# ETH3D/badslam

Hardware: NVIDIA H100
Metric: surfel_keyframe_residuals_per_second_per_BA_iteration (higher is better)
Workload: dtype f32

## Files before the change

badslam_b200/_lib.py:

```python
from __future__ import annotations

import ctypes as C
import os

HERE = os.path.dirname(os.path.abspath(__file__))
LIB_PATH = os.path.join(HERE, "libbadba_b200.so")

ABI_VERSION = 10

POSE_VARIANT_AUTO, POSE_VARIANT_256_PRE, POSE_VARIANT_512_PRE, POSE_VARIANT_256, POSE_VARIANT_512, POSE_VARIANT_1024 = range(6)

OK, ERR_INVALID_ARGUMENT, ERR_CUDA, ERR_STATE, ERR_UNSUPPORTED, ERR_NO_DEVICE = range(6)
STATUS_NAMES = {0: "BBA_OK", 1: "BBA_ERR_INVALID_ARGUMENT", 2: "BBA_ERR_CUDA", 3: "BBA_ERR_STATE",
                4: "BBA_ERR_UNSUPPORTED", 5: "BBA_ERR_NO_DEVICE"}


class Config(C.Structure):
    _fields_ = [("depth_width", C.c_int), ("depth_height", C.c_int), ("color_width", C.c_int), ("color_height", C.c_int),
                ("depth_intrinsics", C.c_float * 4), ("color_intrinsics", C.c_float * 4),
                ("raw_to_float_depth", C.c_float), ("baseline_fx", C.c_float),
                ("sparse_surfel_cell_size", C.c_int), ("max_surfel_count", C.c_uint32), ("max_keyframes", C.c_int),
                ("use_depth_residuals", C.c_int), ("use_descriptor_residuals", C.c_int),
                ("device", C.c_int), ("rank", C.c_int), ("world_size", C.c_int),
                ("min_observation_count_while_bootstrapping_1", C.c_int), ("min_observation_count_while_bootstrapping_2", C.c_int),
                ("min_observation_count", C.c_int), ("surfel_merge_dist_factor", C.c_float)]


PROGRESS_FN = C.CFUNCTYPE(C.c_int, C.c_void_p, C.c_int)


class BAOptions(C.Structure):
    _fields_ = [("optimize_depth_intrinsics", C.c_int), ("optimize_color_intrinsics", C.c_int),
                ("do_surfel_updates", C.c_int), ("optimize_poses", C.c_int), ("optimize_geometry", C.c_int),
                ("min_iterations", C.c_int), ("max_iterations", C.c_int), ("use_pcg", C.c_int),
                ("active_keyframe_window_start", C.c_int), ("active_keyframe_window_end", C.c_int),
                ("increase_ba_iteration_count", C.c_int), ("time_limit_seconds", C.c_double),
                ("pcg_max_inner_iterations", C.c_int), ("pcg_max_keyframes", C.c_int), ("pcg_gauge_keyframe", C.c_int),
                ("progress_function", PROGRESS_FN), ("progress_user", C.c_void_p)]


class PcgProbe(C.Structure):
    _fields_ = [("r", C.c_void_p), ("M", C.c_void_p), ("p", C.c_void_p), ("g", C.c_void_p), ("delta", C.c_void_p),
                ("alpha_n", C.c_double), ("alpha_d", C.c_double),
                ("r_step2", C.c_void_p), ("delta_step2", C.c_void_p), ("z", C.c_void_p), ("beta_n", C.c_double),
                ("p_step3", C.c_void_p), ("g_step3", C.c_void_p), ("alpha_d_step3", C.c_double)]


class BAResult(C.Structure):
    _fields_ = [("iterations_done", C.c_int), ("converged", C.c_int),
                ("depth_residual_count", C.c_uint64), ("descriptor_residual_count", C.c_uint64), ("cost", C.c_double),
                ("pose_iterations_total", C.c_int),
                ("ms_surfel_activation", C.c_float), ("ms_geometry_optimization", C.c_float),
                ("ms_pose_optimization", C.c_float), ("ms_intrinsics_optimization", C.c_float),
                ("kernel_launches", C.c_uint64),
                ("pcg_inner_iterations_total", C.c_int), ("pcg_last_r_norm", C.c_float), ("ms_pcg", C.c_float),
                ("surfels_deleted", C.c_uint32), ("surfels_size", C.c_uint32),
                ("surfels_created", C.c_uint32), ("surfels_merged", C.c_uint32)]


class PreprocessOptions(C.Structure):
    _fields_ = [("bilateral_filter_sigma_xy", C.c_float), ("bilateral_filter_sigma_inv_depth", C.c_float),
                ("bilateral_filter_radius_factor", C.c_float), ("max_depth", C.c_float)]


class RawFrameOptions(C.Structure):
    _fields_ = [("base", PreprocessOptions), ("median_filter_and_densify_iterations", C.c_int),
                ("pyramid_level_for_depth", C.c_int), ("pyramid_level_for_color", C.c_int)]


class OdometryOptions(C.Structure):
    _fields_ = [("num_scales", C.c_int), ("use_pyramid_level_0", C.c_int), ("use_gradmag", C.c_int),
                ("test_different_initial_estimates", C.c_int), ("max_iterations_per_scale", C.c_int)]


class OdometryResult(C.Structure):
    _fields_ = [("iterations", C.c_int * 8), ("chose_initial", C.c_int * 8), ("residual_count", C.c_uint32),
                ("residual_sum", C.c_float), ("passes", C.c_uint32), ("kernel_launches", C.c_uint32)]


class MotionModelRecord(C.Structure):
    _fields_ = [("count", C.c_int), ("base_kf_tr_frame", (C.c_float * 7) * 3), ("frame_tr_base_kf", (C.c_float * 7) * 3)]


class PoseConstraint(C.Structure):
    _fields_ = [("keyframe_a", C.c_int), ("keyframe_b", C.c_int), ("a_T_b", C.c_float * 7), ("information", C.c_float * 21)]


class PoseGraphOptions(C.Structure):
    _fields_ = [("gauge_keyframe", C.c_int), ("max_iterations", C.c_int), ("use_odometry_chain", C.c_int),
                ("odometry_information", C.c_float * 21)]


class PoseGraphResult(C.Structure):
    _fields_ = [("iterations", C.c_int), ("converged", C.c_int), ("linear_iterations", C.c_int), ("held_keyframes", C.c_int),
                ("initial_cost", C.c_double), ("final_cost", C.c_double)]


class PeerHandle(C.Structure):
    _fields_ = [("surfels_ipc", C.c_ubyte * 64), ("surfels_offset", C.c_uint64), ("active_ipc", C.c_ubyte * 64),
                ("active_offset", C.c_uint64), ("pitch_bytes", C.c_uint64), ("surfels_size", C.c_uint32), ("rank", C.c_int32)]


class PoseCoeffs(C.Structure):
    _fields_ = [("H", C.c_float * 21), ("b", C.c_float * 6),
                ("n_pair", C.c_uint64), ("n_inimg", C.c_uint64), ("n_depthok", C.c_uint64),
                ("n_assoc", C.c_uint64), ("n_photo", C.c_uint64),
                ("cost_depth", C.c_double), ("cost_desc1", C.c_double), ("cost_desc2", C.c_double)]


class FrameBuffers(C.Structure):
    _fields_ = [("depth", C.c_void_p), ("depth_pitch", C.c_size_t), ("normals", C.c_void_p), ("normals_pitch", C.c_size_t),
                ("color_rgba", C.c_void_p), ("color_pitch", C.c_size_t)]


class OdometryEntry(C.Structure):
    _fields_ = [("base_keyframe_id", C.c_int), ("base_frame", C.c_int), ("tracked_frame", C.c_int),
                ("base_T_frame_initial_1", C.c_float * 7), ("base_T_frame_initial_2", C.c_float * 7)]


ODOMETRY_CHUNK_ENTRIES = 64


class Profile(C.Structure):
    _fields_ = [("pose_launches", C.c_uint64), ("pose_ms", C.c_double), ("kf_evals", C.c_uint64),
                ("n_pair", C.c_uint64), ("n_inimg", C.c_uint64), ("n_depthok", C.c_uint64),
                ("n_assoc", C.c_uint64), ("n_photo", C.c_uint64),
                ("geometry_launches", C.c_uint64), ("activation_normals_ms", C.c_double),
                ("position_descriptor_ms", C.c_double)]


COLLECTIVE_FN = C.CFUNCTYPE(None, C.c_void_p, C.c_int, C.c_void_p, C.c_size_t, C.c_void_p)
COLLECTIVE_ALLGATHER, COLLECTIVE_ALLREDUCE_SUM = 0, 1

_P = C.c_void_p
_F7 = C.POINTER(C.c_float)
SYMBOLS = {
    "bba_abi_version": (C.c_int, []),
    "bba_create": (C.c_int, [C.POINTER(Config), C.POINTER(_P)]),
    "bba_destroy": (None, [_P]),
    "bba_last_error": (C.c_char_p, [_P]),
    "bba_set_surfels": (C.c_int, [_P, _P, C.c_size_t, C.c_uint32]),
    "bba_set_active_flags": (C.c_int, [_P, _P]),
    "bba_set_surfels_host": (C.c_int, [_P, _P, C.c_size_t, C.c_uint32, _P]),
    "bba_get_surfels_host": (C.c_int, [_P, _P, C.c_size_t, C.c_int, _P]),
    "bba_get_active_flags_host": (C.c_int, [_P, _P, _P]),
    "bba_get_surfels_device": (C.c_int, [_P, C.POINTER(_P), C.POINTER(C.c_size_t), C.POINTER(C.c_uint32)]),
    "bba_add_keyframe": (C.c_int, [_P, _P, C.c_size_t, _P, C.c_size_t, _P, C.c_size_t, _P, C.c_size_t, _F7,
                                   C.c_float, C.c_float, _P, C.POINTER(C.c_int)]),
    "bba_add_keyframe_host": (C.c_int, [_P, _P, _P, _P, _P, _F7, C.c_float, C.c_float, _P, C.POINTER(C.c_int)]),
    "bba_keyframe_count": (C.c_int, [_P]),
    "bba_set_keyframe_pose": (C.c_int, [_P, C.c_int, _F7]),
    "bba_get_keyframe_pose": (C.c_int, [_P, C.c_int, _F7]),
    "bba_set_keyframe_activation": (C.c_int, [_P, C.c_int, C.c_int]),
    "bba_get_keyframe_activation": (C.c_int, [_P, C.c_int, C.POINTER(C.c_int)]),
    "bba_set_keyframe_states": (C.c_int, [_P, C.c_int, _P, _P]),
    "bba_get_keyframe_states": (C.c_int, [_P, C.c_int, _P, _P]),
    "bba_get_covisibility": (C.c_int, [_P, C.c_int, _P]),
    "bba_set_keyframe_pose_priors": (C.c_int, [_P, C.c_int, _P, _P, _P]),
    "bba_clear_keyframe_pose_priors": (C.c_int, [_P, C.c_int, _P]),
    "bba_get_keyframe_pose_prior": (C.c_int, [_P, C.c_int, _P, _P, C.POINTER(C.c_int)]),
    "bba_add_keyframe_pose_constraints": (C.c_int, [_P, C.c_int, _P, _P]),
    "bba_remove_keyframe_pose_constraints": (C.c_int, [_P, C.c_int, _P]),
    "bba_get_keyframe_pose_constraints": (C.c_int, [_P, C.c_int, _P, _P, C.POINTER(C.c_int)]),
    "bba_set_intrinsics": (C.c_int, [_P, _F7, _F7, C.c_float]),
    "bba_get_intrinsics": (C.c_int, [_P, _F7, _F7, C.POINTER(C.c_float)]),
    "bba_host_se3_exp": (None, [_P, _P]),
    "bba_host_se3_log": (None, [_P, _P]),
    "bba_host_se3_compose": (None, [_P, _P, _P]),
    "bba_host_se3_inverse": (None, [_P, _P]),
    "bba_host_pose_update_converged": (C.c_int, [_P]),
    "bba_host_solve_ldlt": (C.c_int, [C.c_int, _P, _P, _P]),
    "bba_host_pose_prior_terms": (None, [_P, _P, _P, _P, _P, C.POINTER(C.c_double)]),
    "bba_host_pose_constraint_terms": (None, [_P, _P, _P, _P, _P, _P, C.POINTER(C.c_double)]),
    "bba_host_frusta_intersect": (C.c_int, [_P, C.c_int, C.c_int, _P, C.c_float, C.c_float, _P, C.c_float, C.c_float]),
    "bba_host_motion_model_clear": (None, [C.POINTER(MotionModelRecord), _P, _P]),
    "bba_host_motion_model_predict": (C.c_int, [C.POINTER(MotionModelRecord), C.c_int, _P, _P]),
    "bba_host_motion_model_push": (None, [C.POINTER(MotionModelRecord), _P]),
    "bba_host_motion_model_rebase": (None, [C.POINTER(MotionModelRecord)]),
    "bba_host_deform_trajectory": (C.c_int, [C.c_int, _P, _P, _P, C.c_int, C.c_int, _P]),
    "bba_set_residual_types": (C.c_int, [_P, C.c_int, C.c_int]),
    "bba_get_residual_types": (C.c_int, [_P, C.POINTER(C.c_int), C.POINTER(C.c_int)]),
    "bba_set_cfactor_host": (C.c_int, [_P, _P, _P]),
    "bba_get_cfactor_host": (C.c_int, [_P, _P, _P]),
    "bba_cfactor_size": (C.c_int, [_P, C.POINTER(C.c_int), C.POINTER(C.c_int)]),
    "bba_accumulate_pose_coeffs": (C.c_int, [_P, C.c_int, _F7, C.POINTER(PoseCoeffs), _P]),
    "bba_debug_pose_coeffs_batch": (C.c_int, [_P, C.c_int, _P, _P, C.c_int, C.c_int, _P, _P, _P, _P, _P]),
    "bba_debug_set_pose_group": (C.c_int, [_P, C.c_int]),
    "bba_estimate_frame_pose": (C.c_int, [_P, C.c_int, _F7, _F7, C.POINTER(C.c_int), C.POINTER(C.c_int), _P]),
    "bba_estimate_frame_pose_for_frame": (C.c_int, [_P, _P, C.c_size_t, _P, C.c_size_t, _P, C.c_size_t, _F7, _F7,
                                                    C.POINTER(C.c_int), C.POINTER(C.c_int), _P]),
    "bba_estimate_frame_poses_for_frames": (C.c_int, [_P, C.c_int, C.POINTER(FrameBuffers), C.c_int, _P, _P, _P, _P, _P,
                                                      C.POINTER(PoseCoeffs), _P]),
    "bba_track_frame_pairwise": (C.c_int, [_P, C.POINTER(OdometryOptions), C.c_int, _P, C.c_size_t, _P, C.c_size_t, _P, C.c_size_t,
                                           _F7, _F7, _F7, C.POINTER(OdometryResult), _P]),
    "bba_track_frames_pairwise": (C.c_int, [_P, C.POINTER(OdometryOptions), C.c_int, C.POINTER(FrameBuffers), C.c_int,
                                            C.POINTER(OdometryEntry), _P, C.POINTER(OdometryResult), C.POINTER(C.c_uint32), _P]),
    "bba_track_frame_pairwise_to_frame": (C.c_int, [_P, C.POINTER(OdometryOptions), _P, C.c_size_t, _P, C.c_size_t, _P, C.c_size_t,
                                                    _P, C.c_size_t, _P, C.c_size_t, _P, C.c_size_t, _F7, _F7, _F7,
                                                    C.POINTER(OdometryResult), _P]),
    "bba_odometry_get_level": (C.c_int, [_P, C.c_int, C.c_int, _P, _P, _P, C.POINTER(C.c_int), C.POINTER(C.c_int), _P]),
    "bba_odometry_debug_coeffs": (C.c_int, [_P, C.c_int, C.c_int, _F7, _F7, _P, _P, C.POINTER(C.c_uint32), C.POINTER(C.c_float),
                                            _P, _P, _P]),
    "bba_update_surfel_activation": (C.c_int, [_P, _P]),
    "bba_optimize_geometry_iteration": (C.c_int, [_P, _P]),
    "bba_deform_surfels": (C.c_int, [_P, C.c_int, _P, C.POINTER(C.c_uint32), C.POINTER(C.c_uint32), _P]),
    "bba_optimize_pose_graph": (C.c_int, [_P, C.POINTER(PoseGraphOptions), C.POINTER(PoseGraphResult), _P]),
    "bba_optimize_intrinsics": (C.c_int, [_P, C.c_int, C.c_int, _P]),
    "bba_debug_intrinsics_coeffs": (C.c_int, [_P, C.c_int, C.c_int, _P, _P, _P]),
    "bba_perform_end_tasks": (C.c_int, [_P, C.c_int, C.POINTER(C.c_uint32), C.POINTER(C.c_uint32), _P]),
    "bba_surfels_size": (C.c_uint32, [_P]),
    "bba_get_ba_iteration_counts": (C.c_int, [_P, C.POINTER(C.c_int), C.POINTER(C.c_int)]),
    "bba_set_ba_iteration_counts": (C.c_int, [_P, C.c_int, C.c_int]),
    "bba_create_surfels_for_keyframe": (C.c_int, [_P, C.c_int, C.c_int, C.POINTER(C.c_uint32), _P]),
    "bba_merge_surfels_for_keyframe": (C.c_int, [_P, C.c_int, C.POINTER(C.c_uint32), _P]),
    "bba_compact_surfels": (C.c_int, [_P, C.c_uint32, C.c_int, C.POINTER(C.c_uint32), _P]),
    "bba_preprocess_frame": (C.c_int, [_P, C.POINTER(PreprocessOptions), _P, C.c_size_t, _P, C.c_size_t, _P, C.c_size_t,
                                       _P, C.c_size_t, _P, C.c_size_t, _P, C.c_size_t, C.POINTER(C.c_float), C.POINTER(C.c_float), _P]),
    "bba_preprocess_raw_frame": (C.c_int, [_P, C.POINTER(RawFrameOptions), _P, C.c_size_t, C.c_int, C.c_int, _P, C.c_size_t, C.c_int,
                                           C.c_int, _P, C.c_size_t, _P, C.c_size_t, _P, C.c_size_t, _P, C.c_size_t,
                                           C.POINTER(C.c_float), C.POINTER(C.c_float), _P]),
    "bba_pcg_debug": (C.c_int, [_P, C.POINTER(BAOptions), C.c_int, C.c_int, C.POINTER(C.c_uint32), C.POINTER(PcgProbe), _P]),
    "bba_bundle_adjust": (C.c_int, [_P, C.POINTER(BAOptions), C.POINTER(BAResult), _P]),
    "bba_peer_export": (C.c_int, [_P, _P]),
    "bba_peer_import": (C.c_int, [_P, _P, C.c_int]),
    "bba_peer_count": (C.c_int, [_P]),
    "bba_peer_unmap": (C.c_int, [_P]),
    "bba_mark_replica_rewritten": (C.c_int, [_P]),
    "bba_set_collective": (C.c_int, [_P, COLLECTIVE_FN, _P]),
    "bba_local_group_create": (C.c_int, [C.POINTER(_P), C.c_int, C.c_int, C.POINTER(_P)]),
    "bba_local_group_reset": (C.c_int, [_P]),
    "bba_local_group_poison": (C.c_int, [_P]),
    "bba_local_group_destroy": (None, [_P]),
    "bba_debug_collective": (C.c_int, [_P, C.c_int, _P, C.c_size_t, _P]),
    "bba_shard_surfel_owner": (C.c_int, [C.c_uint32, C.c_int]),
    "bba_shard_surfel_local_index": (C.c_uint32, [C.c_uint32, C.c_int]),
    "bba_shard_slice_length": (C.c_uint32, [C.c_uint32, C.c_int]),
    "bba_shard_keyframe_owner": (C.c_int, [C.c_int, C.c_int]),
    "bba_balance_keyframes": (None, [_P, C.c_int, C.c_int, _P]),
    "bba_kernel_launch_count": (C.c_uint64, [_P]),
    "bba_update_keyframe_host": (C.c_int, [_P, C.c_int, _P, _P, _P, _P, _P]),
    "bba_set_deterministic": (C.c_int, [_P, C.c_int]),
    "bba_get_deterministic": (C.c_int, [_P, C.POINTER(C.c_int)]),
    "bba_debug_exact_sum": (C.c_int, [_P, _P, C.c_uint64, C.POINTER(C.c_double), _P]),
    "bba_host_exact_sum": (None, [_P, C.c_size_t, C.POINTER(C.c_double)]),
    "bba_set_profiling": (C.c_int, [_P, C.c_int]),
    "bba_get_profile": (C.c_int, [_P, C.POINTER(Profile), C.c_int]),
}

_lib = None


def load():
    global _lib
    if _lib is not None:
        return _lib
    if not os.path.exists(LIB_PATH):
        raise ImportError(f"{LIB_PATH} is missing: build it with `python -m badslam_b200.build` "
                          "(there is no CPU / eager fallback)")
    lib = C.CDLL(LIB_PATH)
    for name, (restype, argtypes) in SYMBOLS.items():
        fn = getattr(lib, name)
        fn.restype = restype
        fn.argtypes = argtypes
    if lib.bba_abi_version() != ABI_VERSION:
        raise ImportError(f"libbadba_b200.so ABI version {lib.bba_abi_version()}, this binding expects {ABI_VERSION}")
    _lib = lib
    return lib


class BadBAError(RuntimeError):
    def __init__(self, status, message):
        super().__init__(f"{STATUS_NAMES.get(status, status)}: {message}")
        self.status = status
```

badslam_b200/csrc/bundle_adjust.cu:

```cuda
#include <chrono>
#include <cmath>
#include <cstring>
#include <limits>

#include "handle.hpp"

namespace bba {
namespace {

void DetermineCovisibleActiveKeyframes(bba_handle h) {
  for (Keyframe& kf : h->keyframes) {
    if (kf.activation != BBA_KF_ACTIVE) continue;
    for (int o : kf.covis) {
      Keyframe& other = h->keyframes[o];
      if (other.activation == BBA_KF_INACTIVE) other.activation = BBA_KF_COVISIBLE_ACTIVE;
    }
  }
}

bba_status ReserveTileEpochs(bba_handle h) {
  const uint32_t need = (h->surfels_size + 31u) / 32u;
  BBA_CUDA(h, h->geo.d_tile_epoch.Reserve(need, std::max<uint32_t>((h->cfg.max_surfel_count + 31u) / 32u, need) + 1));
  return BBA_OK;
}
// ... 556 lines not shown
             h->pcg.d_vec[4], h->pcg.d_scalars, an, bn, h->sm_count, s);
  return BBA_OK;
}

bba_status PcgStep3(bba_handle h, const PcgLayout& L, int an, int bn, cudaStream_t s) {
  BBA_CUDA(h, cudaMemsetAsync(h->pcg.d_scalars + 1, 0, sizeof(double), s));
  BBA_LAUNCH(h, h->launches, LaunchPcgStep3, L.unknown_count, L.a_index, static_cast<int>(h->keyframes.size()), h->pcg.d_vec[3],
             h->pcg.d_vec[4], h->pcg.d_scalars, an, bn, h->sm_count, s);
  return BBA_OK;
}

bba_status PcgApplyDelta(bba_handle h, const PcgLayout& L, int gauge, cudaStream_t s, int* num_converged) {
  const int K = static_cast<int>(h->keyframes.size());
  const uint32_t N = h->surfels_size, P = static_cast<uint32_t>(h->cf_w) * h->cf_h;
  const float* pcg_delta = h->pcg.d_vec[2];
  size_t n_host = 0;
  const size_t pose_floats = L.opt_poses ? 6 * static_cast<size_t>(K - 1) : 0;
  if (pose_floats) BBA_CUDA(h, cudaMemcpyAsync(h->pcg.h_delta, pcg_delta, sizeof(float) * pose_floats, cudaMemcpyDeviceToHost, s));
  n_host = pose_floats;
  float* h_di = h->pcg.h_delta + n_host;
  if (L.opt_depth_intr) {
    BBA_CUDA(h, cudaMemcpyAsync(h_di, pcg_delta + L.depth_start, sizeof(float) * 5, cudaMemcpyDeviceToHost, s));
    n_host += 5;
  }
  float* h_ci = h->pcg.h_delta + n_host;
  if (L.opt_color_intr) BBA_CUDA(h, cudaMemcpyAsync(h_ci, pcg_delta + L.color_start, sizeof(float) * 4, cudaMemcpyDeviceToHost, s));
  if (L.opt_geometry && N > 0) {
    BBA_LAUNCH(h, h->launches, LaunchPcgUpdateSurfels, h->surfels, SurfelPitch(h), N, L.use_desc, L.surfel_start, pcg_delta, s);
    h->xchg.replicated_pass_pending = true;
  }
  if (L.opt_depth_intr) BBA_LAUNCH(h, h->launches, LaunchPcgUpdateCfactor, h->d_cfactor, P, pcg_delta + L.depth_start + 5, s);
  BBA_CUDA(h, cudaStreamSynchronize(s));
  if (L.opt_poses) {
    for (int k = 0; k < K; ++k) {
      if (k == gauge) {
        ++*num_converged;
        continue;
      }
      const float* d6 = h->pcg.h_delta + 6 * static_cast<size_t>(k < gauge ? k : k - 1);
      const Pose delta = bba::Exp(d6);
      h->keyframes[k].pose = bba::Compose(h->keyframes[k].pose, delta);
      float lg[6];
      bba::Log(delta, lg);
      if (bba::IsScale1PoseEstimationConverged(lg)) ++*num_converged;
    }
  }
  if (L.opt_depth_intr) {
    const double old_fx_inv = 1. / h->depth_K[0], old_fy_inv = 1. / h->depth_K[1];
    const double old_cx_inv = -(h->depth_K[2] - 0.5) * old_fx_inv, old_cy_inv = -(h->depth_K[3] - 0.5) * old_fy_inv;
    const double new_fx = 1. / (old_fx_inv + h_di[0]);
    const double new_fy = 1. / (old_fy_inv + h_di[1]);
    const double new_cx = -(new_fx * (old_cx_inv + h_di[2])) + 0.5;
    const double new_cy = -(new_fy * (old_cy_inv + h_di[3])) + 0.5;
    h->depth_K[0] = static_cast<float>(new_fx);
    h->depth_K[1] = static_cast<float>(new_fy);
    h->depth_K[2] = static_cast<float>(new_cx);
    h->depth_K[3] = static_cast<float>(new_cy);
    h->depth_a += h_di[4];
  }
  if (L.opt_color_intr)
    for (int c = 0; c < 4; ++c) h->color_K[c] = static_cast<float>(h->color_K[c] + h_ci[c]);
  return Publish(h, s, L.opt_depth_intr);
}

bba_status BundleAdjustPCG(bba_handle h, const bba_ba_options* o, bba_ba_result* res, cudaStream_t s) {
  const int K = static_cast<int>(h->keyframes.size());
  const int world = h->cfg.world_size;
  if (bba_status st = CheckCollective(h)) return st;
  if (world > 1 && o->pcg_gauge_keyframe < 0)
    return Fail(h, BBA_ERR_INVALID_ARGUMENT, "use_pcg with more than one rank needs pcg_gauge_keyframe >= 0 (the reference draws rand() % K)");
  if (K == 0) return Fail(h, BBA_ERR_STATE, "use_pcg: no keyframes");
  const int max_inner = o->pcg_max_inner_iterations > 0 ? o->pcg_max_inner_iterations : 30;
  const int max_keyframes = o->pcg_max_keyframes > 0 ? o->pcg_max_keyframes : 2500;
  if (K > max_keyframes) return Fail(h, BBA_ERR_INVALID_ARGUMENT, "use_pcg: more keyframes than pcg_max_keyframes");
  if (o->pcg_gauge_keyframe >= K) return Fail(h, BBA_ERR_INVALID_ARGUMENT, "pcg_gauge_keyframe out of range");
  PcgLayout L;
  if (bba_status st = MakePcgLayout(h, o, &L)) return st;
  const bool opt_poses = L.opt_poses, opt_geometry = L.opt_geometry;
  const uint64_t launches_before = h->launches;
  const auto t_start = std::chrono::steady_clock::now();
  if (bba_status st = BeginBundleAdjust(h, o, res, s)) return st;
  std::vector<int> keyframes_with_new_surfels;

  for (int iteration = 0; iteration < o->max_iterations; ++iteration) {
    if (o->progress_function && !o->progress_function(o->progress_user, iteration)) break;
    ++res->iterations_done;
    if (bba_status st = CreateInLoopSurfels(h, o, h->ba_iteration_count, s, res, &keyframes_with_new_surfels)) return st;
    const uint32_t N = h->surfels_size;
    if (N > 0) BBA_CUDA(h, cudaMemsetAsync(h->active, bba::kSurfelActiveFlag, N, s));
    if (bba_status st = UploadKeyframes(h, s)) return st;
    BBA_CUDA(h, cudaEventRecord(h->ev[0], s));
    if (opt_geometry && N > 0) {
      bba::GeometryArgs g;
      if (bba_status st = BuildGeometryArgs(h, &g, s, GeoOrder::kCaller)) return st;
      BBA_LAUNCH(h, h->launches, LaunchActivationAndNormals, g, h->sm_count, false, true, s);
      if (bba_status st = ExchangeGeometry(h, s)) return st;
    }
    BBA_CUDA(h, cudaEventRecord(h->ev[1], s));

    if (bba_status st = MakePcgLayout(h, o, &L)) return st;
    const uint32_t unknown_count = L.unknown_count;
    const int gauge = o->pcg_gauge_keyframe >= 0 ? o->pcg_gauge_keyframe : (rand() % K);

    int num_converged = 0;
    if (unknown_count > 0) {
      const bba::PcgArgs a = MakePcgArgs(h, L, gauge);
      int an = 0, bn = 2;
      if (bba_status st = PcgInit(h, L, a, an, s)) return st;
      float prev_r_norm = std::numeric_limits<float>::infinity();
      int without_improvement = 0;
      for (int step = 0; step < max_inner; ++step) {
        if (step > 0) std::swap(an, bn);
        if (bba_status st = PcgStep1(h, L, a, s)) return st;
        if (bba_status st = PcgStep2(h, L, an, bn, s)) return st;
        BBA_CUDA(h, cudaMemcpyAsync(h->pcg.h_scalars, h->pcg.d_scalars, sizeof(double) * 4, cudaMemcpyDeviceToHost, s));
        BBA_CUDA(h, cudaStreamSynchronize(s));
        ++res->pcg_inner_iterations_total;
        const float r_norm = std::sqrt(static_cast<float>(h->pcg.h_scalars[bn]));
        res->pcg_last_r_norm = r_norm;
        if (static_cast<double>(r_norm) < static_cast<double>(prev_r_norm) - 1e-3) {
          without_improvement = 0;
        } else if (++without_improvement >= 3) {
          break;
        }
        prev_r_norm = r_norm;
        if (step < max_inner - 1) {
          if (bba_status st = PcgStep3(h, L, an, bn, s)) return st;
        }
      }
      BBA_CUDA(h, cudaEventRecord(h->ev[2], s));
      if (bba_status st = PcgApplyDelta(h, L, gauge, s, &num_converged)) return st;
      if (o->do_surfel_updates && !keyframes_with_new_surfels.empty()) {
        uint32_t merged = 0;
        if (bba_status st = MergeAndCompact(h, keyframes_with_new_surfels, s, &merged)) return st;
        res->surfels_merged += merged;
      }
    } else {
      BBA_CUDA(h, cudaEventRecord(h->ev[2], s));
      BBA_CUDA(h, cudaStreamSynchronize(s));
      num_converged = opt_poses ? 1 : 0;
    }
    cudaEventElapsedTime(&res->ms_geometry_optimization, h->ev[0], h->ev[1]);
    cudaEventElapsedTime(&res->ms_pcg, h->ev[1], h->ev[2]);
    if (StopIterating(o, iteration, num_converged, K, t_start, res)) break;
  }
  if (!o->increase_ba_iteration_count && o->do_surfel_updates && !keyframes_with_new_surfels.empty()) {
    uint32_t merged = 0;
    if (bba_status st = MergeAndCompact(h, keyframes_with_new_surfels, s, &merged)) return st;
    res->surfels_merged += merged;
  }
  return EndBundleAdjust(h, o, launches_before, res, s);
}

bba_status GeometryPass(bba_handle h, bool activation, cudaStream_t s) {
  if (!h) return BBA_ERR_INVALID_ARGUMENT;
  if (bba_status st = CheckSurfels(h)) return st;
  if (h->surfels_size == 0) return BBA_OK;
  if (bba_status st = UploadKeyframes(h, s)) return st;
  bba::GeometryArgs g;
  if (bba_status st = BuildGeometryArgs(h, &g, s, GeoOrder::kSpatial)) return st;
  if (bba_status st = CheckCollective(h)) return st;
  BBA_LAUNCH(h, h->launches, LaunchActivationAndNormals, g, h->sm_count, activation, !activation, s);
  if (!activation) BBA_LAUNCH(h, h->launches, LaunchPositionAndDescriptor, g, h->sm_count, s);
  if (bba_status st = ExchangeGeometry(h, s)) return st;
  return MarkStaging(h, s);
}

void QuatToMatrix64(const float q[4], double R[9]) {
  const double n = std::sqrt(static_cast<double>(q[0]) * q[0] + static_cast<double>(q[1]) * q[1] + static_cast<double>(q[2]) * q[2] +
                             static_cast<double>(q[3]) * q[3]);
  const double x = q[0] / n, y = q[1] / n, z = q[2] / n, w = q[3] / n;
  R[0] = 1 - 2 * (y * y + z * z); R[1] = 2 * (x * y - z * w); R[2] = 2 * (x * z + y * w);
  R[3] = 2 * (x * y + z * w); R[4] = 1 - 2 * (x * x + z * z); R[5] = 2 * (y * z - x * w);
  R[6] = 2 * (x * z - y * w); R[7] = 2 * (y * z + x * w); R[8] = 1 - 2 * (x * x + y * y);
}

KfChange KeyframeChange(const Pose& global_T_frame, const float original[7]) {
  KfChange c{};
  float inv[7];
  PoseToArray(Inverse(global_T_frame), inv);
  c.unmoved = std::memcmp(inv, original, sizeof(inv)) == 0;
  double Rc[9], Ro[9];
  QuatToMatrix64(global_T_frame.q, Rc);
  QuatToMatrix64(original, Ro);
  for (int r = 0; r < 3; ++r) {
    for (int col = 0; col < 3; ++col)
      c.D[4 * r + col] = static_cast<float>(Rc[3 * r] * Ro[col] + Rc[3 * r + 1] * Ro[3 + col] + Rc[3 * r + 2] * Ro[6 + col]);
    c.D[4 * r + 3] = static_cast<float>(Rc[3 * r] * original[4] + Rc[3 * r + 1] * original[5] + Rc[3 * r + 2] * original[6] +
                                        global_T_frame.t[r]);
    c.centre[r] = static_cast<float>(-(Ro[r] * original[4] + Ro[3 + r] * original[5] + Ro[6 + r] * original[6]));
  }
  if (c.unmoved)
    for (int i = 0; i < 12; ++i) c.D[i] = (i % 5 == 0) ? 1.f : 0.f;
  return c;
}

bba_status DeformSurfels(bba_handle h, int count, const float* original, uint32_t* moved, uint32_t* unobserved, cudaStream_t s) {
  if (!h) return BBA_ERR_INVALID_ARGUMENT;
  const std::string fn = "bba_deform_surfels: ";
  if (count < 0 || count > static_cast<int>(h->keyframes.size())) return Fail(h, BBA_ERR_INVALID_ARGUMENT, fn + "bad count");
  if (count > 0 && !original) return Fail(h, BBA_ERR_INVALID_ARGUMENT, fn + "null argument");
  for (int k = 0; k < count; ++k) {
    const float* p = original + 7 * static_cast<size_t>(k);
    for (int j = 0; j < 7; ++j)
      if (!std::isfinite(p[j])) return Fail(h, BBA_ERR_INVALID_ARGUMENT, fn + "non-finite pose");
    if (p[0] * p[0] + p[1] * p[1] + p[2] * p[2] + p[3] * p[3] < 1e-12f) return Fail(h, BBA_ERR_INVALID_ARGUMENT, fn + "zero quaternion");
  }
  if (moved) *moved = 0;
  if (unobserved) *unobserved = 0;
  if (count == 0 || h->surfels_size == 0) return BBA_OK;
  if (bba_status st = CheckSurfels(h)) return st;
  if (bba_status st = CheckCollective(h)) return st;
  auto& d = h->deform;
  BBA_CUDA(h, d.h_kfs.Reserve(count, h->cfg.max_keyframes));
  BBA_CUDA(h, d.d_kfs.Reserve(count, h->cfg.max_keyframes));
  BBA_CUDA(h, d.h_changes.Reserve(count, h->cfg.max_keyframes));
  BBA_CUDA(h, d.d_changes.Reserve(count, h->cfg.max_keyframes));
  BBA_CUDA(h, d.d_counts.Reserve(2));
  BBA_CUDA(h, d.h_counts.Reserve(2));
  if (bba_status st = MakeAllKeyframeList(h)) return st;
  if (bba_status st = WaitStaging(h)) return st;
  for (int k = 0; k < count; ++k) {
    const Keyframe& kf = h->keyframes[k];
    const float* p = original + 7 * static_cast<size_t>(k);
    FillKfDevice(kf, kf.pose, d.h_kfs + k);
    ToMatrix3x4(PoseFromArray(p), d.h_kfs[k].T);
    d.h_changes[k] = KeyframeChange(kf.pose, p);
  }
  BBA_CUDA(h, cudaMemcpyAsync(d.d_kfs, d.h_kfs, sizeof(KfDevice) * count, cudaMemcpyHostToDevice, s));
  BBA_CUDA(h, cudaMemcpyAsync(d.d_changes, d.h_changes, sizeof(KfChange) * count, cudaMemcpyHostToDevice, s));
  if (bba_status st = MarkStaging(h, s)) return st;
  BBA_CUDA(h, cudaMemsetAsync(d.d_counts, 0, sizeof(unsigned int) * 2, s));
  bba::DeformArgs a;
  if (bba_status st = BuildGeometryArgs(h, &a.geo, s, GeoOrder::kSpatial)) return st;
  a.geo.kfs = d.d_kfs;
  a.geo.kf_list = h->geo.d_all_list;
  a.geo.kf_count = count;
  a.changes = d.d_changes;
  a.counts = d.d_counts;
  BBA_LAUNCH(h, h->launches, LaunchDeformSurfels, a, h->sm_count, s);
  if (bba_status st = ExchangeGeometry(h, s)) return st;
  h->pose.order_stale = true;
  if (!moved && !unobserved) return BBA_OK;
  BBA_CUDA(h, cudaMemcpyAsync(d.h_counts, d.d_counts, sizeof(unsigned int) * 2, cudaMemcpyDeviceToHost, s));
  BBA_CUDA(h, cudaStreamSynchronize(s));
  uint32_t counts[2] = {d.h_counts[0], d.h_counts[1]};
  if (h->cfg.world_size > 1)
    for (uint32_t& c : counts)
      if (bba_status st = SumOverRanks(h, c, s, &c)) return st;
  if (moved) *moved = counts[0];
  if (unobserved) *unobserved = counts[1];
  return BBA_OK;
}

struct PoseGraphSizes {
  size_t terms, ints, doubles;
};
PoseGraphSizes PoseGraphCapacity(size_t K, size_t C) {
  const size_t terms = 2 * K + C, entries = 3 * K + 2 * C, nnz = 3 * K + 2 * C;
  const size_t block_doubles = sizeof(PoseGraphTermBlocks) / sizeof(double);
  return {terms, K + 2 * (K + 1) + 2 * entries + nnz, terms * block_doubles + 36 * nnz + 42 * K + PoseGraphWorkDoubles(K)};
}

bba_status ReservePoseGraph(bba_handle h, size_t constraints) {
  const size_t M = static_cast<size_t>(h->cfg.max_keyframes);
  const PoseGraphSizes need = PoseGraphCapacity(M, constraints), alloc = PoseGraphCapacity(M, 2 * constraints);
  auto& g = h->graph;
  BBA_CUDA(h, g.h_terms.Reserve(need.terms, alloc.terms));
  BBA_CUDA(h, g.d_terms.Reserve(need.terms, alloc.terms));
  BBA_CUDA(h, g.h_ints.Reserve(need.ints, alloc.ints));
  BBA_CUDA(h, g.d_ints.Reserve(need.ints, alloc.ints));
  BBA_CUDA(h, g.d_doubles.Reserve(need.doubles, alloc.doubles));
  BBA_CUDA(h, g.h_poses.Reserve(7 * M));
  BBA_CUDA(h, g.d_poses.Reserve(14 * M));
  BBA_CUDA(h, g.d_state.Reserve(1));
  BBA_CUDA(h, g.h_state.Reserve(1));
  return BBA_OK;
}

int FindRoot(std::vector<int>& parent, int k) {
  while (parent[k] != k) k = parent[k] = parent[parent[k]];
  return k;
}

bba_status OptimizePoseGraph(bba_handle h, const bba_pose_graph_options* o, bba_pose_graph_result* result, cudaStream_t s) {
  if (!h) return BBA_ERR_INVALID_ARGUMENT;
  const std::string fn = "bba_optimize_pose_graph: ";
  if (!o) return Fail(h, BBA_ERR_INVALID_ARGUMENT, fn + "null options");
  const int K = static_cast<int>(h->keyframes.size());
  const int gauge = o->gauge_keyframe;
  if (gauge < -1 || gauge >= K) return Fail(h, BBA_ERR_INVALID_ARGUMENT, fn + "gauge_keyframe out of range");
  if (o->use_odometry_chain) {
    for (int j = 0; j < 21; ++j)
      if (!std::isfinite(o->odometry_information[j])) return Fail(h, BBA_ERR_INVALID_ARGUMENT, fn + "non-finite odometry_information");
    if (!InformationPsd(o->odometry_information))
      return Fail(h, BBA_ERR_INVALID_ARGUMENT, fn + "odometry_information is not positive semi-definite");
  }
  bba_pose_graph_result r{};
  if (result) *result = r;
  if (K < 2 && h->pose_prior_count == 0) return BBA_OK;
  const std::vector<PoseConstraint>& cons = h->pose_constraints;
  if (bba_status st = ReservePoseGraph(h, cons.size())) return st;
  auto& g = h->graph;
  const bool chain = o->use_odometry_chain != 0;
  const int max_iterations = o->max_iterations > 0 ? o->max_iterations : 20;

  float* poses = g.h_poses;
  for (int k = 0; k < K; ++k) PoseToArray(h->keyframes[k].pose, poses + 7 * k);
  std::vector<int> prior_term(K, -1);
  int T = 0;
  auto add = [&](int a, int b, const float* z, const float* info) {
    PoseGraphTerm& t = g.h_terms[T++];
    t.a = a;
    t.b = b;
    std::memcpy(t.z, z, sizeof(t.z));
    std::memcpy(t.info, info, sizeof(t.info));
// ... 7 lines not shown
  const int first_constraint = T;
  for (const PoseConstraint& c : cons) add(c.c.keyframe_a, c.c.keyframe_b, c.c.a_T_b, c.c.information);
  const int first_chain = T;
  if (chain)
    for (int k = 0; k + 1 < K; ++k) {
      double qa[4], ta[3], qb[4], tb[3], q[4], t[3];
      LoadPoseD(poses + 7 * k, qa, ta);
      LoadPoseD(poses + 7 * (k + 1), qb, tb);
      Se3BetweenD(qa, ta, qb, tb, q, t);
      float z[7];
      for (int j = 0; j < 4; ++j) z[j] = static_cast<float>(q[j]);
      for (int j = 0; j < 3; ++j) z[4 + j] = static_cast<float>(t[j]);
      add(k, k + 1, z, o->odometry_information);
    }

  std::vector<int> parent(K), lowest(K, -1);
  std::vector<char> touched(K, 0), anchored(K, 0);
  for (int k = 0; k < K; ++k) parent[k] = k;
  for (int i = first_constraint; i < T; ++i) {
    const PoseGraphTerm& t = g.h_terms[i];
    touched[t.a] = touched[t.b] = 1;
    const int ra = FindRoot(parent, t.a), rb = FindRoot(parent, t.b);
    if (ra != rb) parent[std::max(ra, rb)] = std::min(ra, rb);
  }
  for (int k = 0; k < K; ++k) {
    const int root = FindRoot(parent, k);
    if (lowest[root] < 0) lowest[root] = k;
    if (prior_term[k] >= 0) touched[k] = 1;
    if (prior_term[k] >= 0 || k == gauge) anchored[root] = 1;
  }
  int* held = g.h_ints;
  int held_count = 0;
  for (int k = 0; k < K; ++k) {
    const int root = FindRoot(parent, k);
    held[k] = (k == gauge || !touched[k] || (!anchored[root] && lowest[root] == k)) ? 1 : 0;
    held_count += held[k];
  }

  std::vector<int> off, adj;
  ConstraintAdjacency(h, K, &off, &adj);
  int* row_off = held + K;
  int entries = 0, nnz = 0;
  for (int k = 0; k < K; ++k) {
    row_off[k] = entries;
    const int binary = (off[k + 1] - off[k]) + (chain ? (k > 0) + (k + 1 < K) : 0);
    entries += (prior_term[k] >= 0) + binary;
    nnz += 1 + binary;
  }
  row_off[K] = entries;
  int* row_terms = row_off + K + 1;
  int* csr_off = row_terms + 2 * entries;
  int* csr_col = csr_off + K + 1;
  int e = 0, c = 0;
  auto entry = [&](int term, int side, int col) {
    row_terms[2 * e] = term;
    row_terms[2 * e + 1] = side;
    ++e;
    if (col >= 0) csr_col[c++] = col;
  };
  for (int k = 0; k < K; ++k) {
    csr_off[k] = c;
    csr_col[c++] = k;
    if (prior_term[k] >= 0) entry(prior_term[k], 0, -1);
    for (int j = off[k]; j < off[k + 1]; ++j) {
      const bba_pose_constraint& pc = cons[adj[j]].c;
      const bool is_a = pc.keyframe_a == k;
      entry(first_constraint + adj[j], is_a ? 0 : 1, is_a ? pc.keyframe_b : pc.keyframe_a);
    }
    if (chain && k > 0) entry(first_chain + k - 1, 1, k - 1);
    if (chain && k + 1 < K) entry(first_chain + k, 0, k + 1);
  }
  csr_off[K] = c;
  const size_t ints = static_cast<size_t>(csr_col + nnz - held);

  const size_t M = static_cast<size_t>(h->cfg.max_keyframes);
  if (T) BBA_CUDA(h, cudaMemcpyAsync(g.d_terms, g.h_terms, sizeof(PoseGraphTerm) * T, cudaMemcpyHostToDevice, s));
  BBA_CUDA(h, cudaMemcpyAsync(g.d_ints, g.h_ints, sizeof(int) * ints, cudaMemcpyHostToDevice, s));
  BBA_CUDA(h, cudaMemcpyAsync(g.d_poses, poses, sizeof(float) * 7 * K, cudaMemcpyHostToDevice, s));
  BBA_CUDA(h, cudaMemcpyAsync(g.d_poses + 7 * M, poses, sizeof(float) * 7 * K, cudaMemcpyHostToDevice, s));
  BBA_CUDA(h, cudaMemsetAsync(g.d_state, 0, sizeof(PoseGraphState), s));
  PoseGraphArgs a{};
  a.K = K;
  a.term_count = T;
  a.terms = g.d_terms;
  a.blocks = reinterpret_cast<PoseGraphTermBlocks*>(g.d_doubles.get());
  a.poses = g.d_poses;
  a.prev = g.d_poses + 7 * M;
  const int* d_ints = g.d_ints;
  a.held = d_ints;
  a.row_off = d_ints + (row_off - held);
  a.row_terms = d_ints + (row_terms - held);
  a.csr_off = d_ints + (csr_off - held);
  a.csr_col = d_ints + (csr_col - held);
  double* d = g.d_doubles.get() + static_cast<size_t>(T) * (sizeof(PoseGraphTermBlocks) / sizeof(double));
  a.csr_val = d;
  a.rhs = a.csr_val + 36 * static_cast<size_t>(nnz);
  a.tri = a.rhs + 6 * static_cast<size_t>(K);
  a.work = a.tri + 36 * static_cast<size_t>(K);
  a.state = g.d_state;
  a.max_iterations = max_iterations;
  a.max_linear = 6 * (K - held_count);
  for (int round = 0; round <= max_iterations; ++round) {
    a.round = round;
    BBA_LAUNCH(h, h->launches, LaunchPoseGraphRound, a, s);
  }
  BBA_CUDA(h, cudaMemcpyAsync(g.h_state, g.d_state, sizeof(PoseGraphState), cudaMemcpyDeviceToHost, s));
  BBA_CUDA(h, cudaMemcpyAsync(poses, g.d_poses, sizeof(float) * 7 * K, cudaMemcpyDeviceToHost, s));
  BBA_CUDA(h, cudaStreamSynchronize(s));
  for (int k = 0; k < K; ++k)
    if (!held[k]) h->keyframes[k].pose = PoseFromArray(poses + 7 * k);
  const PoseGraphState& st = *g.h_state.get();
  r.iterations = st.iterations;
  r.converged = st.converged;
  r.linear_iterations = st.linear_iterations;
  r.held_keyframes = held_count;
  r.initial_cost = st.initial_cost;
  r.final_cost = st.cost;
  if (result) *result = r;
  return Publish(h, s, false);
}

}
}

using namespace bba;

extern "C" {

bba_status bba_update_surfel_activation(bba_handle h, void* stream) {
  return GeometryPass(h, true, static_cast<cudaStream_t>(stream));
}

bba_status bba_optimize_geometry_iteration(bba_handle h, void* stream) {
  return GeometryPass(h, false, static_cast<cudaStream_t>(stream));
}

bba_status bba_deform_surfels(bba_handle h, int count, const float* original_keyframe_T_global, uint32_t* moved, uint32_t* unobserved,
                              void* stream) {
  return DeformSurfels(h, count, original_keyframe_T_global, moved, unobserved, static_cast<cudaStream_t>(stream));
}

bba_status bba_optimize_pose_graph(bba_handle h, const bba_pose_graph_options* options, bba_pose_graph_result* result, void* stream) {
  return OptimizePoseGraph(h, options, result, static_cast<cudaStream_t>(stream));
}

bba_status bba_optimize_intrinsics(bba_handle h, int optimize_depth, int optimize_color, void* stream) {
  if (!h) return BBA_ERR_INVALID_ARGUMENT;
  if (!optimize_depth && !optimize_color) return Fail(h, BBA_ERR_INVALID_ARGUMENT, "nothing to optimise");
  if (bba_status st = CheckSurfels(h)) return st;
  if (bba_status st = CheckCollective(h)) return st;
  return OptimizeIntrinsics(h, optimize_depth != 0, optimize_color != 0, static_cast<cudaStream_t>(stream));
}

bba_status bba_debug_intrinsics_coeffs(bba_handle h, int optimize_depth, int optimize_color, double* sums, float* cells, void* stream) {
  if (!h) return BBA_ERR_INVALID_ARGUMENT;
  if (!sums || !cells) return Fail(h, BBA_ERR_INVALID_ARGUMENT, "bba_debug_intrinsics_coeffs: null argument");
  if (!optimize_depth && !optimize_color) return Fail(h, BBA_ERR_INVALID_ARGUMENT, "nothing to optimise");
  if (bba_status st = CheckSurfels(h)) return st;
  if (bba_status st = CheckCollective(h)) return st;
  const size_t P = static_cast<size_t>(h->cf_w) * h->cf_h;
  std::memset(sums, 0, sizeof(double) * bba::kIntrinsicsSums);
  std::memset(cells, 0, sizeof(float) * 8 * P);
  if (h->surfels_size == 0 || h->keyframes.empty()) return BBA_OK;
  cudaStream_t s = static_cast<cudaStream_t>(stream);
  IntrinsicsEquations eq;
  if (bba_status st = AccumulateIntrinsics(h, optimize_depth != 0, optimize_color != 0, s, &eq)) return st;
  BBA_CUDA(h, cudaMemcpyAsync(sums, h->geo.d_intr_sums, sizeof(double) * bba::kIntrinsicsSums, cudaMemcpyDeviceToHost, s));
  BBA_CUDA(h, cudaMemcpyAsync(cells, eq.cell_B, sizeof(float) * 8 * P, cudaMemcpyDeviceToHost, s));
  BBA_CUDA(h, cudaStreamSynchronize(s));
  return BBA_OK;
}

}

namespace bba {
namespace {

bba_status BundleAdjust(bba_handle h, const bba_ba_options* o, bba_ba_result* res, void* stream) {
  std::memset(res, 0, sizeof(*res));
  if (bba_status st = CheckSurfels(h)) return st;
  if (o->use_pcg && h->deterministic)
    return Fail(h, BBA_ERR_UNSUPPORTED, "bba_bundle_adjust: use_pcg is not available in the deterministic mode (bba_set_deterministic)");
  if (o->use_pcg) return BundleAdjustPCG(h, o, res, static_cast<cudaStream_t>(stream));
  const bool opt_depth_intr = o->optimize_depth_intrinsics && h->cfg.use_depth_residuals;
  const bool opt_color_intr = o->optimize_color_intrinsics && h->cfg.use_descriptor_residuals;
  if (bba_status st = CheckCollective(h)) return st;
  cudaStream_t s = static_cast<cudaStream_t>(stream);
  const int K = static_cast<int>(h->keyframes.size());
  const uint64_t launches_before = h->launches;
  const auto t_start = std::chrono::steady_clock::now();

  h->pose.order_stale = true;
  const int fixed_ba_iteration_count = h->ba_iteration_count;
  if (bba_status st = BeginBundleAdjust(h, o, res, s)) return st;
  std::vector<int> keyframes_with_new_surfels;

  const bool fixed_window = o->active_keyframe_window_start > 0 || o->active_keyframe_window_end > 0;
  const bool whole_window = !(o->active_keyframe_window_start != 0 || o->active_keyframe_window_end != K - 1);

  BBA_CUDA(h, cudaMemsetAsync(h->active, 0, h->surfels_size, s));

  for (int iteration = 0; iteration < o->max_iterations; ++iteration) {
    if (o->progress_function && !o->progress_function(o->progress_user, iteration)) break;
    ++res->iterations_done;
    if (fixed_window) {
      for (int k = 0; k < K; ++k)
        h->keyframes[k].activation =
            (k >= o->active_keyframe_window_start && k <= o->active_keyframe_window_end) ? BBA_KF_ACTIVE : BBA_KF_INACTIVE;
      DetermineCovisibleActiveKeyframes(h);
    }

    BBA_TRACE("iteration start");
    const uint32_t old_surfels_size = h->surfels_size;
    if (bba_status st = CreateInLoopSurfels(h, o, fixed_ba_iteration_count, s, res, &keyframes_with_new_surfels)) return st;
    if (!keyframes_with_new_surfels.empty()) h->pose.order_stale = true;

    BBA_TRACE("creation done");
    if (bba_status st = UploadKeyframes(h, s)) return st;
    BBA_TRACE("keyframes uploaded");
    const bool has_new = o->optimize_geometry && h->surfels_size > old_surfels_size;
    bba::GeometryArgs g;
    if (bba_status st = BuildGeometryArgs(h, &g, s, has_new ? GeoOrder::kCaller : GeoOrder::kByPairs)) return st;

    BBA_TRACE("after creation + upload");
    BBA_CUDA(h, cudaEventRecord(h->ev[0], s));
    if (has_new)
      BBA_CUDA(h, cudaMemsetAsync(h->active + old_surfels_size, bba::kSurfelActiveFlag, h->surfels_size - old_surfels_size, s));
    if (!whole_window) BBA_CUDA(h, cudaMemsetAsync(h->active, bba::kSurfelActiveFlag, old_surfels_size, s));
    if (h->surfels_size > 0) {
      if (whole_window && has_new) {
        bba::GeometryArgs g_old = g, g_new = g;
        g_old.end = LocalCountBelow(old_surfels_size, h->cfg.rank, h->cfg.world_size);
        g_new.begin = g_old.end;
        BBA_LAUNCH(h, h->launches, LaunchActivationAndNormals, g_old, h->sm_count, true, true, s);
        BBA_LAUNCH(h, h->launches, LaunchActivationAndNormals, g_new, h->sm_count, false, true, s);
      } else if (whole_window) {
        BBA_LAUNCH(h, h->launches, LaunchActivationAndNormals, g, h->sm_count, true, o->optimize_geometry != 0, s);
      } else if (o->optimize_geometry) {
        BBA_LAUNCH(h, h->launches, LaunchActivationAndNormals, g, h->sm_count, false, true, s);
      }
    }
    BBA_CUDA(h, cudaEventRecord(h->ev[1], s));
    if (o->optimize_geometry && h->surfels_size > 0) BBA_LAUNCH(h, h->launches, LaunchPositionAndDescriptor, g, h->sm_count, s);
    if (bba_status st = ExchangeGeometry(h, s)) return st;
    BBA_CUDA(h, cudaEventRecord(h->ev[2], s));
    if (bba_status st = MarkStaging(h, s)) return st;

    BBA_TRACE("after geometry");
    if (o->do_surfel_updates && !keyframes_with_new_surfels.empty()) {
      uint32_t merged = 0;
      if (bba_status st = MergeAndCompact(h, keyframes_with_new_surfels, s, &merged)) return st;
      res->surfels_merged += merged;
      h->pose.order_stale = true;
    }

    BBA_TRACE("before pose step");
    int num_converged = 0;
    if (o->optimize_poses) {
      std::vector<int> ids;
      std::vector<Pose> init;
      for (int k = 0; k < K; ++k) {
        if (h->keyframes[k].activation == BBA_KF_INACTIVE) {
          ++num_converged;
          continue;
        }
        ids.push_back(k);
        init.push_back(h->keyframes[k].pose);
      }
      if (bba_status st = RunPoseStep(h, ids, init, 30, s)) return st;
      res->depth_residual_count = 0;
      res->descriptor_residual_count = 0;
      res->cost = 0;
      for (int k : ids) {
        Keyframe& kf = h->keyframes[k];
        const Pose est = PoseFromArray(h->pose.h_pose_est + 7 * k);
        float lg[6];
        bba::Log(bba::Compose(bba::Inverse(kf.pose), est), lg);
        const bool moved = !bba::IsScale1PoseEstimationConverged(lg);
        kf.pose = est;
        if (moved) {
          kf.activation = BBA_KF_ACTIVE;
        } else {
          kf.activation = BBA_KF_INACTIVE;
          ++num_converged;
        }
        res->pose_iterations_total += h->pose.h_iterations[k];
        const double* fs = h->pose.h_first_stats + 8 * k;
        res->depth_residual_count += static_cast<uint64_t>(fs[0] + 0.5);
        res->descriptor_residual_count += 2 * static_cast<uint64_t>(fs[1] + 0.5);
        res->cost += fs[2] + fs[3];
      }
    } else {
      BBA_CUDA(h, cudaStreamSynchronize(s));
    }
    if (bba_status st = Publish(h, s, false)) return st;
    BBA_CUDA(h, cudaEventRecord(h->ev[3], s));
    if (opt_depth_intr || opt_color_intr) {
      if (bba_status st = OptimizeIntrinsics(h, opt_depth_intr, opt_color_intr, s)) return st;
      BBA_CUDA(h, cudaEventRecord(h->ev[4], s));
      BBA_CUDA(h, cudaEventSynchronize(h->ev[4]));
      cudaEventElapsedTime(&res->ms_intrinsics_optimization, h->ev[3], h->ev[4]);
    }
    BBA_CUDA(h, cudaEventSynchronize(h->ev[3]));
    cudaEventElapsedTime(&res->ms_surfel_activation, h->ev[0], h->ev[1]);
    cudaEventElapsedTime(&res->ms_geometry_optimization, h->ev[1], h->ev[2]);
    cudaEventElapsedTime(&res->ms_pose_optimization, h->ev[2], h->ev[3]);
    if (h->profiling) {
      h->profile.activation_normals_ms += res->ms_surfel_activation;
      h->profile.position_descriptor_ms += res->ms_geometry_optimization;
      h->profile.geometry_launches += (o->optimize_geometry ? 2 : 1);
    }

    if (StopIterating(o, iteration, num_converged, K, t_start, res)) break;
    DetermineCovisibleActiveKeyframes(h);
    if (bba_status st = Publish(h, s, false)) return st;
  }
  BBA_TRACE("iterations done");
  return EndBundleAdjust(h, o, launches_before, res, s);
}

}
}

extern "C" bba_status bba_bundle_adjust(bba_handle h, const bba_ba_options* o, bba_ba_result* res, void* stream) {
  if (!h || !o || !res) return BBA_ERR_INVALID_ARGUMENT;
  const bba_status st = bba::BundleAdjust(h, o, res, static_cast<cudaStream_t>(stream));
  bba::Publish(h, static_cast<cudaStream_t>(stream), false);
  return st;
}

extern "C" {

bba_status bba_perform_end_tasks(bba_handle h, int do_surfel_updates, uint32_t* deleted, uint32_t* surfels_size, void* stream) {
  if (!h) return BBA_ERR_INVALID_ARGUMENT;
  if (bba_status st = CheckSurfels(h)) return st;
  uint32_t d = 0;
  if (bba_status st = PerformEndTasks(h, static_cast<cudaStream_t>(stream), &d, do_surfel_updates != 0)) return st;
  if (deleted) *deleted = d;
  if (surfels_size) *surfels_size = h->surfels_size;
  return BBA_OK;
}

bba_status bba_create_surfels_for_keyframe(bba_handle h, int id, int filter_new_surfels, uint32_t* created, void* stream) {
  CHECK_KF(h, id);
  if (bba_status st = CheckSurfels(h)) return st;
  uint32_t c = 0;
  if (bba_status st = CreateSurfelsForKeyframe(h, id, filter_new_surfels != 0, static_cast<cudaStream_t>(stream), &c)) return st;
  if (created) *created = c;
  return BBA_OK;
}

bba_status bba_merge_surfels_for_keyframe(bba_handle h, int id, uint32_t* deleted, void* stream) {
  CHECK_KF(h, id);
  if (bba_status st = CheckSurfels(h)) return st;
  uint32_t d = 0;
  if (bba_status st = MergeSurfelsForKeyframe(h, id, static_cast<cudaStream_t>(stream), &d)) return st;
  if (deleted) *deleted = d;
  return BBA_OK;
}

bba_status bba_compact_surfels(bba_handle h, uint32_t free_count, int with_active_flags, uint32_t* surfels_size, void* stream) {
  if (!h) return BBA_ERR_INVALID_ARGUMENT;
  if (bba_status st = CheckSurfels(h)) return st;
  if (free_count > h->surfels_size) return Fail(h, BBA_ERR_INVALID_ARGUMENT, "free_count exceeds surfels_size");
  if (bba_status st = CompactSurfels(h, free_count, with_active_flags != 0, static_cast<cudaStream_t>(stream))) return st;
  if (surfels_size) *surfels_size = h->surfels_size;
  return BBA_OK;
}

bba_status bba_pcg_debug(bba_handle h, const bba_ba_options* o, int step, int apply, uint32_t* unknown_count, bba_pcg_probe* out,
                         void* stream) {
  if (!h || !o || !unknown_count || step < 0) return BBA_ERR_INVALID_ARGUMENT;
  if (bba_status st = CheckSurfels(h)) return st;
  const int K = static_cast<int>(h->keyframes.size());
  if (K == 0) return Fail(h, BBA_ERR_STATE, "no keyframes");
  if (o->pcg_gauge_keyframe < 0 || o->pcg_gauge_keyframe >= K) return Fail(h, BBA_ERR_INVALID_ARGUMENT, "pcg_gauge_keyframe out of range");
  if (h->cfg.world_size > 1) return Fail(h, BBA_ERR_UNSUPPORTED, "bba_pcg_debug runs on one rank");
  if (h->deterministic) return Fail(h, BBA_ERR_UNSUPPORTED, "bba_pcg_debug: the PCG solver is not available in the deterministic mode");
  cudaStream_t s = static_cast<cudaStream_t>(stream);
  PcgLayout L;
  if (bba_status st = MakePcgLayout(h, o, &L)) return st;
  *unknown_count = L.unknown_count;
  if (!out || L.unknown_count == 0) return BBA_OK;
  const uint32_t U = L.unknown_count;
  auto copy = [&](float* dst, const float* src) -> bba_status {
    if (dst) BBA_CUDA(h, cudaMemcpyAsync(dst, src, sizeof(float) * U, cudaMemcpyDeviceToHost, s));
    return BBA_OK;
  };
  auto scalars = [&](int slot, double* dst) -> bba_status {
    BBA_CUDA(h, cudaMemcpyAsync(h->pcg.h_scalars, h->pcg.d_scalars, sizeof(double) * 4, cudaMemcpyDeviceToHost, s));
    BBA_CUDA(h, cudaStreamSynchronize(s));
    *dst = h->pcg.h_scalars[slot];
    return BBA_OK;
  };
  if (bba_status st = UploadKeyframes(h, s)) return st;
  const bba::PcgArgs a = MakePcgArgs(h, L, o->pcg_gauge_keyframe);
  int an = 0, bn = 2;
  if (bba_status st = PcgInit(h, L, a, an, s)) return st;
  for (int k = 0;; ++k) {
    if (k > 0) std::swap(an, bn);
    if (bba_status st = PcgStep1(h, L, a, s)) return st;
    if (k == step) break;
    if (bba_status st = PcgStep2(h, L, an, bn, s)) return st;
    if (bba_status st = PcgStep3(h, L, an, bn, s)) return st;
  }
  float *r = h->pcg.d_vec[0], *M = h->pcg.d_vec[1], *delta = h->pcg.d_vec[2], *g = h->pcg.d_vec[3], *p = h->pcg.d_vec[4];
  bba_status st = BBA_OK;
  if ((st = copy(out->r, r)) || (st = copy(out->M, M)) || (st = copy(out->p, p)) || (st = copy(out->g, g)) || (st = copy(out->delta, delta)) ||
      (st = scalars(an, &out->alpha_n)) || (st = scalars(1, &out->alpha_d)))
    return st;
  if ((st = PcgStep2(h, L, an, bn, s)) || (st = copy(out->r_step2, r)) || (st = copy(out->delta_step2, delta)) || (st = copy(out->z, g)) ||
      (st = scalars(bn, &out->beta_n)))
    return st;
  if ((st = PcgStep3(h, L, an, bn, s)) || (st = copy(out->p_step3, p)) || (st = copy(out->g_step3, g)) || (st = scalars(1, &out->alpha_d_step3)))
    return st;
  if (apply) {
    int num_converged = 0;
    if ((st = PcgApplyDelta(h, L, o->pcg_gauge_keyframe, s, &num_converged))) return st;
  }
  BBA_CUDA(h, cudaStreamSynchronize(s));
  return MarkStaging(h, s);
}

}
```

badslam_b200/csrc/handle.hpp:

```cpp
#pragma once

#include <cuda_runtime.h>

#include <algorithm>
#include <atomic>
#include <condition_variable>
#include <cstdio>
#include <cstdlib>
#include <map>
#include <memory>
#include <mutex>
#include <string>
#include <thread>
#include <vector>

#include "../../include/badba.h"
#include "host_math.hpp"
#include "kernels.cuh"
#include "odometry.cuh"

namespace bba {

template <class R, auto Free>
struct Owned {
// ... 50 lines not shown
    p_.r = p;
    pitch_ = pitch;
    return cudaSuccess;
  }
  template <class T = uint8_t> T* get() const { return static_cast<T*>(p_.r); }
  size_t pitch() const { return pitch_; }
  explicit operator bool() const { return p_.r != nullptr; }

 private:
  Owned<void*, cudaFree> p_;
  size_t pitch_ = 0;
};

using Event = Owned<cudaEvent_t, cudaEventDestroy>;

struct Texture {
  Owned<cudaArray_t, cudaFreeArray> array;
  Owned<cudaTextureObject_t, cudaDestroyTextureObject> tex;
};

struct Keyframe {
  const uint16_t* depth = nullptr;
  const uint16_t* normals = nullptr;
  const uint16_t* radius = nullptr;
  size_t depth_pitch = 0, normals_pitch = 0, radius_pitch = 0;
  cudaTextureObject_t tex = 0;
  const uint8_t* rgba = nullptr;
  size_t rgba_pitch = 0;
  PitchedBuffer owned[3];
  PitchedBuffer owned_rgba;
  Texture luma;
  int last_active_in_ba_iteration = -1;
  int last_covis_in_ba_iteration = -1;
  Pose pose;
  int activation = BBA_KF_ACTIVE;
  float min_depth = 0.f, max_depth = 0.f;
  Frustum frustum;
  std::vector<int> covis;
};

struct KeyframeView {
  const uint16_t* depth = nullptr;
  const uint16_t* normals = nullptr;
  size_t depth_pitch = 0, normals_pitch = 0;
  cudaTextureObject_t tex = 0;
  Pose pose;
  float min_depth = 0.f, max_depth = 0.f;
  int activation = BBA_KF_ACTIVE;
  PosePrior prior{};
};

struct PoseConstraint {
  int id;
  bba_pose_constraint c;
  float info_a[21];
};

struct CameraView {
  float depth_K[4] = {}, color_K[4] = {};
  float depth_a = 0.f;
  int use_depth = 1, use_desc = 1;
  int deterministic = 0;
};

struct LumaStaging {
  PitchedBuffer plane;
  int planes = 0;
  PinnedBuffer<LumaSource> table_upload;
  DeviceBuffer<LumaSource> table;
  Event free;
};

}

struct bba_context {
  bba_config cfg;
  float depth_K[4], color_K[4];
  float depth_a = 0.f;
  int cf_w = 0, cf_h = 0;
  int sm_count = 132;
  std::mutex error_mu;
  std::map<std::thread::id, std::string> errors;

  float* surfels = nullptr;
  size_t surfel_pitch_bytes = 0;
  uint32_t surfels_size = 0;
  uint8_t* active = nullptr;
  bba::DeviceBuffer<float> owned_surfels;
  size_t owned_surfel_pitch = 0;
  bba::DeviceBuffer<uint8_t> owned_active;

  bba::DeviceBuffer<float> d_cfactor;
  std::vector<bba::Keyframe> keyframes;
  bba::DeviceBuffer<bba::KfDevice> d_kfs;
  std::vector<bba::PosePrior> pose_priors;
  int pose_prior_count = 0;
  std::vector<bba::PoseConstraint> pose_constraints;
  int next_pose_constraint_id = 0;

  struct Staging {
    bba::PinnedBuffer<bba::KfDevice> h_kfs;
    bba::Event event;
    bool pending = false;
    bba::LumaStaging luma;
    bba::PitchedBuffer color;
  } staging;

  std::vector<bba::Texture> frame_luma;

  struct PoseStep {
    bba::DeviceBuffer<bba::KfDevice> d_work_records;
    bba::DeviceBuffer<float> d_pose_est;
    bba::DeviceBuffer<double> d_acc;
    bba::DeviceBuffer<bba::ExactSum> d_exact;
    bba::DeviceBuffer<unsigned long long> d_stage_counts;
    bba::DeviceBuffer<int> d_work[2];
    bba::DeviceBuffer<int> d_count;
    bba::DeviceBuffer<int> d_iterations;
    bba::DeviceBuffer<int> d_converged;
    bba::DeviceBuffer<double> d_first_stats;
    bba::DeviceBuffer<unsigned long long> d_totals;
    bba::DeviceBuffer<unsigned int> d_queue;
    bba::MappedBuffer<int> flag;
    volatile int* h_flag = nullptr;
    int* d_flag = nullptr;
    bba::PinnedBuffer<float> h_pose_est;
    bba::PinnedBuffer<int> h_work;
    bba::PinnedBuffer<int> h_iterations;
    bba::PinnedBuffer<int> h_converged;
    bba::PinnedBuffer<double> h_first_stats;
    bba::PinnedBuffer<unsigned long long> h_totals;
    bba::PinnedBuffer<int> h_term_offsets;
    bba::DeviceBuffer<int> d_term_offsets;
    bba::PinnedBuffer<bba::PoseTerm> h_terms;
    bba::DeviceBuffer<bba::PoseTerm> d_terms;
    struct Order {
      bba::DeviceBuffer<uint32_t> words;
      bba::DeviceBuffer<unsigned char> temp;
      bba::DeviceBuffer<float> stream;
      bba::DeviceBuffer<float> boxes;
      bba::SpatialOrderBuffers view{};
      uint32_t capacity = 0;
    } order;
    uint32_t order_n = 0;
    bool order_stale = true;
    int group = 0;
  } pose;

  struct Geometry {
    bba::DeviceBuffer<int> d_list;
    bba::PinnedBuffer<int> h_list;
    bba::DeviceBuffer<unsigned int> d_queue;
    bba::DeviceBuffer<unsigned int> d_tile_epoch;
    const uint32_t* perm = nullptr;
    bba::DeviceBuffer<float> d_intr;
    bba::DeviceBuffer<double> d_intr_sums;
    bba::DeviceBuffer<bba::ExactSum> d_intr_exact;
    bba::DeviceBuffer<int> d_all_list;
    bba::PinnedBuffer<double> h_intr_sums;
    bba::PinnedBuffer<float> h_intr_x1;
  } geo;

  struct Deform {
    bba::PinnedBuffer<bba::KfDevice> h_kfs;
    bba::DeviceBuffer<bba::KfDevice> d_kfs;
    bba::PinnedBuffer<bba::KfChange> h_changes;
    bba::DeviceBuffer<bba::KfChange> d_changes;
    bba::DeviceBuffer<unsigned int> d_counts;
    bba::PinnedBuffer<unsigned int> h_counts;
  } deform;

  struct PoseGraph {
    bba::PinnedBuffer<bba::PoseGraphTerm> h_terms;
    bba::DeviceBuffer<bba::PoseGraphTerm> d_terms;
    bba::PinnedBuffer<int> h_ints;
    bba::DeviceBuffer<int> d_ints;
    bba::PinnedBuffer<float> h_poses;
    bba::DeviceBuffer<float> d_poses;
    bba::DeviceBuffer<double> d_doubles;
    bba::DeviceBuffer<bba::PoseGraphState> d_state;
    bba::PinnedBuffer<bba::PoseGraphState> h_state;
  } graph;

  struct Lifecycle {
    bba::DeviceBuffer<unsigned int> d_sup;
    bba::DeviceBuffer<unsigned int> d_cell_bits;
    bba::DeviceBuffer<unsigned int> d_flags;
    bba::DeviceBuffer<unsigned int> d_scan_out;
    bba::DeviceBuffer<unsigned int> d_scan_sums;
    bba::DeviceBuffer<bba::CovisEntry> d_covis;
    bba::PinnedBuffer<bba::CovisEntry> h_covis;
    bba::DeviceBuffer<bba::KfRadius> d_kf_radius;
    bba::PinnedBuffer<bba::KfRadius> h_kf_radius;
    bba::DeviceBuffer<unsigned int> d_deleted_count;
    bba::PinnedBuffer<unsigned int> h_count;
  } life;
  int last_ba_iteration_count = -1;

  struct Pcg {
    bba::DeviceBuffer<float> d_vec[5];
    bba::DeviceBuffer<double> d_scalars;
    bba::PinnedBuffer<double> h_scalars;
    bba::PinnedBuffer<float> h_delta;
    bba::PinnedBuffer<bba::PcgPoseBlock> h_pose_blocks;
    bba::DeviceBuffer<bba::PcgPoseBlock> d_pose_blocks;
    bba::PinnedBuffer<bba::PcgPoseTerm> h_pose_terms;
    bba::DeviceBuffer<bba::PcgPoseTerm> d_pose_terms;
    int pose_blocks = 0;
  } pcg;

  struct Exchange {
    bba_collective_fn collective = nullptr;
    void* collective_user = nullptr;
    bba_local_group group = nullptr;
    std::string exchange_error;
    bba::DeviceBuffer<float> d_exchange;
    bba::DeviceBuffer<float> d_pose_pack;
    bba::PinnedBuffer<float> h_pose_pack;
    bba::DeviceBuffer<int> d_local_ids;
    bba::DeviceBuffer<float> d_count_xchg;
    bba::PinnedBuffer<float> h_count_xchg;
    bba::DeviceBuffer<float> d_barrier;
    bba::PeerSet peers{};
    void* peer_bases[2 * bba::kMaxPeers] = {};
    int peer_base_count = 0;
    bool replicated_pass_pending = false;
  } xchg;

  struct Pyramid {
    bba::PitchedBuffer gradmag;
    bba::Texture gradmag_tex;
    bba::PitchedBuffer depth[bba::odom::kMaxScales], normals[bba::odom::kMaxScales], color[bba::odom::kMaxScales];
    bba::Texture color_tex[bba::odom::kMaxScales];
    bba::odom::Image image[bba::odom::kMaxScales] = {};
  };
  struct Odometry {
    int num_scales = 0;
    int last_num_scales = 0;
    int last_first_scale = 0;
    std::vector<std::unique_ptr<Pyramid>> pool;
    int w[bba::odom::kMaxScales] = {}, h[bba::odom::kMaxScales] = {};
    bba::odom::LevelCamera cam[bba::odom::kMaxScales] = {};
    bba::odom::Image last_level[2][bba::odom::kMaxScales] = {};
    bba::odom::TrackEntry last_entry{};
    bba::PinnedBuffer<bba::odom::PyramidImage> h_images;
    bba::DeviceBuffer<bba::odom::PyramidImage> d_images;
    bba::PinnedBuffer<bba::odom::TrackEntry> h_entries;
    bba::DeviceBuffer<bba::odom::TrackEntry> d_entries;
    bba::DeviceBuffer<double> d_acc;
    bba::DeviceBuffer<double> d_partials;
    bba::DeviceBuffer<unsigned int> d_control;
    bba::DeviceBuffer<bba::odom::TrackResult> d_result;
    bba::PinnedBuffer<bba::odom::TrackResult> h_result;
  } odo;

  struct Preprocess {
    bba::DeviceBuffer<float> d_min_max;
    bba::PinnedBuffer<float> h_min_max;
  } pre;

  struct FrontEnd {
    std::mutex mu;
    std::condition_variable slot_free;
    bba::CameraView cams;
    std::vector<bba::KeyframeView> kfs;
    std::vector<bba::PoseConstraint> constraints;
    bba::DeviceBuffer<float> cfactor[2];
    bba::Event published[2];
    bba::Event readers_done[2];
    int current = 0;
    int readers[2] = {0, 0};
    std::mutex call;
    bba::LumaStaging luma;
    std::vector<bba::Texture> frames;
  } fe;

  std::atomic<uint64_t> launches{0};
  std::atomic<uint64_t> front_end_launches{0};
  int ba_iteration_count = 0;
  std::vector<float> kf_cost;

  bool deterministic = false;

  int profiling = 0;
  bba_profile profile;
  bba::Event prof_ev[64];
  bba::Event ev[6];
};

namespace bba {

bba_status Fail(bba_handle h, bba_status s, const std::string& msg);
void SetError(bba_handle h, const std::string& msg);

class FrontEndScope {
 public:
  FrontEndScope() { ++depth_; }
  ~FrontEndScope() { --depth_; }
  FrontEndScope(const FrontEndScope&) = delete;
  FrontEndScope& operator=(const FrontEndScope&) = delete;
  static bool active() { return depth_ > 0; }

 private:
  static thread_local int depth_;
};

// ... 98 lines not shown
```

badslam_b200/csrc/kernels.cu:

```cuda
#include "persistent.cuh"

#include <cuda.h>

#include <algorithm>

namespace bba {


__device__ __forceinline__ uint32_t SmemAddr(const void* p) { return static_cast<uint32_t>(__cvta_generic_to_shared(p)); }

__device__ __forceinline__ void MbarInit(uint64_t* bar, uint32_t count) {
  asm volatile("mbarrier.init.shared::cta.b64 [%0], %1;" ::"r"(SmemAddr(bar)), "r"(count));
}
__device__ __forceinline__ void FenceBarrierInit() { asm volatile("fence.mbarrier_init.release.cluster;" ::: "memory"); }
__device__ __forceinline__ void MbarArriveExpectTx(uint64_t* bar, uint32_t bytes) {
  asm volatile("mbarrier.arrive.expect_tx.shared::cta.b64 _, [%0], %1;" ::"r"(SmemAddr(bar)), "r"(bytes) : "memory");
}
__device__ __forceinline__ void MbarArrive(uint32_t bar) {
  asm volatile("mbarrier.arrive.shared::cta.b64 _, [%0];" ::"r"(bar) : "memory");
}
__device__ __forceinline__ void MbarWait(uint32_t bar, uint32_t parity) {
  asm volatile(
      "{\n"
      ".reg .pred p;\n"
// ... 396 lines not shown
      }
    }
  }
  if (PRE) {
    acquire_slot(batch_seq);
    if (lane == 0) batch_hdr[warp][batch_seq & 1] = make_int4(0, 0, 0, -1);
    commit_slot(batch_seq);
  }
}

__global__ void __launch_bounds__(128) PackWorkRecordsKernel(const KfDevice* __restrict__ kfs, const int* __restrict__ work_list,
                                                             const int* __restrict__ work_count, KfDevice* __restrict__ records) {
  const int n = __ldg(work_count);
  constexpr int kWords = sizeof(KfDevice) / 16;
  for (int i = blockIdx.x * blockDim.x + threadIdx.x; i < n * kWords; i += gridDim.x * blockDim.x) {
    const int rec = i / kWords, w = i - rec * kWords;
    const int kf = __ldg(work_list + rec);
    uint4 v = __ldg(reinterpret_cast<const uint4*>(kfs + kf) + w);
    if (w == kWords - 1) v.y = static_cast<unsigned int>(kf);
    reinterpret_cast<uint4*>(records + rec)[w] = v;
  }
}

static constexpr size_t PoseSmemBytes(int tile, bool pre, int group) {
  return static_cast<size_t>(2) * (pre ? kPoseStagedRowsPre : kPoseStagedRows) * tile * sizeof(float) + (pre ? kPoseRingBytes : 0) +
         static_cast<size_t>(2) * group * sizeof(KfDevice);
}

template <int TILE, bool PRE>
static cudaError_t SetPoseSmemLimit() {
  const int smem = static_cast<int>(PoseSmemBytes(TILE, PRE, kPoseMaxGroup));
  for (const void* k : {reinterpret_cast<const void*>(PoseAccumulateKernel<TILE, false, PRE, false>),
                        reinterpret_cast<const void*>(PoseAccumulateKernel<TILE, true, PRE, false>),
                        reinterpret_cast<const void*>(PoseAccumulateKernel<TILE, false, PRE, true>),
                        reinterpret_cast<const void*>(PoseAccumulateKernel<TILE, true, PRE, true>)})
    if (const cudaError_t e = cudaFuncSetAttribute(k, cudaFuncAttributeMaxDynamicSharedMemorySize, smem)) return e;
  return cudaSuccess;
}

cudaError_t SetPoseAccumulateSmemLimits() {
  for (cudaError_t e : {SetPoseSmemLimit<256, true>(), SetPoseSmemLimit<512, true>(), SetPoseSmemLimit<256, false>(),
                        SetPoseSmemLimit<512, false>(), SetPoseSmemLimit<1024, false>()})
    if (e != cudaSuccess) return e;
  return cudaSuccess;
}

template <int TILE, bool STATS, bool PRE>
static void LaunchPoseAccumulateT(const PoseAccumulateArgs& args, int sm_count, cudaStream_t stream) {
  const size_t smem = PoseSmemBytes(TILE, PRE, args.group);
  const dim3 grid(kPoseMinCtas * sm_count), block(PRE ? kPoseWsThreads : kPoseThreads);
  if (args.exact) PoseAccumulateKernel<TILE, STATS, PRE, true><<<grid, block, smem, stream>>>(args);
  else PoseAccumulateKernel<TILE, STATS, PRE, false><<<grid, block, smem, stream>>>(args);
}

template <bool STATS>
static void LaunchPoseAccumulateS(const PoseAccumulateArgs& args, int sm_count, int variant, cudaStream_t stream) {
  if (variant == kPoseVariantAuto) {
    const uint64_t slots = static_cast<uint64_t>(kPoseMinCtas * sm_count) * 4;
    if (args.stream != nullptr) variant = args.n >= slots * 512 ? kPoseVariant512Pre : kPoseVariant256Pre;
    else variant = args.n >= slots * 1024 ? kPoseVariant1024 : args.n >= slots * 512 ? kPoseVariant512 : kPoseVariant256;
  }
  switch (variant) {
    case kPoseVariant256Pre: LaunchPoseAccumulateT<256, STATS, true>(args, sm_count, stream); break;
    case kPoseVariant512Pre: LaunchPoseAccumulateT<512, STATS, true>(args, sm_count, stream); break;
    case kPoseVariant256: LaunchPoseAccumulateT<256, STATS, false>(args, sm_count, stream); break;
    case kPoseVariant512: LaunchPoseAccumulateT<512, STATS, false>(args, sm_count, stream); break;
    case kPoseVariant1024: LaunchPoseAccumulateT<1024, STATS, false>(args, sm_count, stream); break;
  }
}

LaunchResult LaunchPoseAccumulate(const PoseAccumulateArgs& args, int sm_count, bool with_stats, int max_work, cudaStream_t stream,
                                  int variant) {
  if (args.n == 0 || max_work <= 0) return {};
  PackWorkRecordsKernel<<<(max_work * 6 + 127) / 128, 128, 0, stream>>>(args.kfs, args.work_list, args.work_count, args.work_records);
  PoseAccumulateArgs a = args;
  if (a.group == 0) a.group = a.stream && a.stream_sorted ? 32 : 8;
  if (with_stats) LaunchPoseAccumulateS<true>(a, sm_count, variant, stream);
  else LaunchPoseAccumulateS<false>(a, sm_count, variant, stream);
  return {2};
}


constexpr int kGeoThreads = 256;
constexpr int kGeoGroup = 32;

__device__ __forceinline__ void StageGroupRecords(const KfDevice* __restrict__ kfs, const int* __restrict__ kf_list, int count,
                                                  KfDevice* dst, int lane) {
  constexpr int kWords = sizeof(KfDevice) / 16;
  __syncwarp();
  const int my_kf = lane < count ? __ldg(kf_list + lane) : 0;
#pragma unroll
  for (int w = 0; w < (kGeoGroup * kWords + 31) / 32; ++w) {
    const int idx = w * 32 + lane, rec = idx / kWords, part = idx - rec * kWords;
    const int kf = __shfl_sync(0xffffffffu, my_kf, rec & 31);
    if (rec < count) {
      uint4 v = __ldg(reinterpret_cast<const uint4*>(kfs + kf) + part);
      reinterpret_cast<uint4*>(dst + rec)[part] = v;
    }
  }
  __syncwarp();
}

__device__ __forceinline__ void WarpBox(const Vec3& p, bool in, float (&lo)[3], float (&hi)[3]) {
  const float c[3] = {p.x, p.y, p.z};
#pragma unroll
  for (int ax = 0; ax < 3; ++ax) {
    const bool f = in && isfinite(c[ax]);
    lo[ax] = FromOrderedBits(__reduce_min_sync(0xffffffffu, f ? OrderedBits(c[ax]) : 0xffffffffu));
    hi[ax] = FromOrderedBits(__reduce_max_sync(0xffffffffu, f ? OrderedBits(c[ax]) : 0u));
  }
}

static_assert(kGeoGroup <= 32, "one lane per keyframe of a group");
template <bool ACTIVE_ONLY>
__device__ __forceinline__ unsigned VisibleKeyframes(const CameraParams& cam, const KfDevice* recs, int n_kf, const float (&lo)[3],
                                                     const float (&hi)[3], int lane) {
  bool visible = false;
  if (lane < n_kf) {
    KfRegs K;
    LoadKfShared(recs + lane, &K);
    visible = (!ACTIVE_ONLY || K.activation == 0) && !BoxOutsideViewLane(cam, K.T, lo, hi);
  }
  return __ballot_sync(0xffffffffu, visible);
}

__device__ __forceinline__ int PopLowest(unsigned* m) {
  if (*m == 0u) return -1;
  const int j = __ffs(*m) - 1;
  *m &= *m - 1u;
  return j;
}

__device__ __forceinline__ void StoreSurfelRow(const GeometryArgs& a, int row, uint32_t i, float v) {
  StoreReplicas(a.surfels, a.peers.surfels, a.peers.count, static_cast<size_t>(row) * a.pitch + i, v);
}

__device__ __forceinline__ bool GeoStreamPosition(const GeometryArgs& a, uint32_t tile, uint32_t sub, int lane, uint32_t* s) {
  const uint32_t li = a.begin + (tile << a.tile_shift) + sub * 32 + lane;
  *s = SurfelShardToGlobal(li, a.shard_rank, a.shard_world);
  return li < a.end && *s < a.n;
}
__device__ __forceinline__ uint32_t GeoResultIndex(const GeometryArgs& a, uint32_t s) { return a.perm ? __ldg(a.perm + s) : s; }
template <int N>
__device__ __forceinline__ void LoadParkedSums(const GeometryArgs& a, uint32_t s, float (&v)[N]) {
#pragma unroll
  for (int r = 0; r < N; ++r) v[r] = __ldcg(a.surfels + (kRowAccum0 + r) * static_cast<size_t>(a.pitch) + s);
}
template <int N>
__device__ __forceinline__ void StoreParkedSums(const GeometryArgs& a, uint32_t s, const float (&v)[N]) {
#pragma unroll
  for (int r = 0; r < N; ++r) __stcg(a.surfels + (kRowAccum0 + r) * static_cast<size_t>(a.pitch) + s, v[r]);
}

template <bool DETERMINE, bool NORMALS>
__global__ void __launch_bounds__(kGeoThreads) ActivationNormalsKernel(const __grid_constant__ GeometryArgs a) {
  extern __shared__ __align__(16) unsigned char geo_smem[];
  KfDevice* s_kfs = reinterpret_cast<KfDevice*>(geo_smem);
  const uint32_t tile_len = 1u << a.tile_shift;
  const uint32_t n_tiles = (a.end - a.begin + tile_len - 1) >> a.tile_shift;
  const uint32_t n_groups = (a.kf_count + kGeoGroup - 1) / kGeoGroup;
  const uint32_t n_items = n_groups * n_tiles;
  const size_t P = a.pitch, F = a.stream_pitch;
  const int lane = threadIdx.x & 31;
  uint32_t group, tile;
  while (ClaimItem(a.queue, n_tiles, n_items, a.tile_epoch, &group, &tile)) {
    const bool first = group == 0, last = group + 1 == n_groups;
    const int j_begin = group * kGeoGroup, j_end = min(a.kf_count, static_cast<int>(group + 1) * kGeoGroup);
    const int n_kf = j_end - j_begin;
    KfDevice* recs = s_kfs + (threadIdx.x >> 5) * kGeoGroup;
    StageGroupRecords(a.kfs, a.kf_list + j_begin, n_kf, recs, lane);
    for (uint32_t sub = 0; sub < tile_len / 32; ++sub) {
      uint32_t s;
      const bool in_range = GeoStreamPosition(a, tile, sub, lane, &s);
      const uint32_t flags = in_range ? __float_as_uint(a.stream[(kGeoStreamRows - 1) * F + s]) : 0u;
      const bool live = in_range && (DETERMINE || (flags & kSurfelActiveFlag));
      if (__ballot_sync(0xffffffffu, live) == 0) continue;
      bool act = !DETERMINE;
      float s0 = 0.f, s1 = 0.f, s2 = 0.f, s3 = 0.f;
      if (!first && live) {
        if (NORMALS) {
          s0 = __ldcg(a.surfels + (kRowAccum0 + 0) * P + s);
          s1 = __ldcg(a.surfels + (kRowAccum0 + 1) * P + s);
          s2 = __ldcg(a.surfels + (kRowAccum0 + 2) * P + s);
          s3 = __ldcg(a.surfels + (kRowAccum0 + 3) * P + s);
        }
        if (DETERMINE) act = __ldcg(a.surfels + (kRowAccum0 + 4) * P + s) != 0.f;
      }
      const bool walk = live && (NORMALS || !act);
      if (__ballot_sync(0xffffffffu, walk) != 0) {
        Vec3 gp = V3(0.f, 0.f, 0.f), nrm = V3(0.f, 0.f, 1.f);
        if (walk) {
          gp = V3(a.stream[0 * F + s], a.stream[1 * F + s], a.stream[2 * F + s]);
          nrm = UnpackNormal(__float_as_uint(a.stream[3 * F + s]));
        }
        float lo[3], hi[3];
        WarpBox(gp, walk, lo, hi);
        unsigned vis = VisibleKeyframes<!NORMALS>(a.cam, recs, n_kf, lo, hi, lane);
        auto accumulate = [&](const KfRegs& K, const PixelLoads& l, Assoc& r) {
          if (Associate(a.cam, K.T, nrm, l, &r) != 3) return;
          if (K.activation == 0) act = true;
          if (NORMALS) {
            const Vec3 ln = U16ToImageSpaceNormal(r.kf_normal);
            s0 += K.T[0] * ln.x + K.T[4] * ln.y + K.T[8] * ln.z;
            s1 += K.T[1] * ln.x + K.T[5] * ln.y + K.T[9] * ln.z;
            s2 += K.T[2] * ln.x + K.T[6] * ln.y + K.T[10] * ln.z;
            s3 += 1.f;
          }
        };
        for (int j = PopLowest(&vis); j >= 0; j = PopLowest(&vis)) {
          KfRegs K;
          LoadKfShared(recs + j, &K);
          Assoc r;
          if (walk && (NORMALS || !act) && ProjectIntoImage(a.cam, K.T, gp, &r))
            accumulate(K, LoadPixel(a.cam, K.depth, K.depth_pitch, K.normals, K.normals_pitch, r), r);
          if (!NORMALS && __all_sync(0xffffffffu, !walk || act)) break;
        }
      }
      if (!live) continue;
      if (!last) {
        if (NORMALS) {
          __stcg(a.surfels + (kRowAccum0 + 0) * P + s, s0);
          __stcg(a.surfels + (kRowAccum0 + 1) * P + s, s1);
          __stcg(a.surfels + (kRowAccum0 + 2) * P + s, s2);
          __stcg(a.surfels + (kRowAccum0 + 3) * P + s, s3);
        }
        if (DETERMINE) __stcg(a.surfels + (kRowAccum0 + 4) * P + s, act ? 1.f : 0.f);
      } else {
        const uint32_t i = GeoResultIndex(a, s);
        if (DETERMINE) StoreReplicas(a.active, a.peers.active, a.peers.count, i, act ? kSurfelActiveFlag : static_cast<uint8_t>(flags & ~kSurfelActiveFlag));
        if (NORMALS && act && s3 >= 1.f) {
          const float inv = 1.f / s3;
          StoreSurfelRow(a, kRowNormal, i, __uint_as_float(PackNormal(V3(inv * s0, inv * s1, inv * s2))));
        }
      }
    }
    RetireItem(a.tile_epoch, group, tile);
  }
}

template <bool USE_DEPTH, bool USE_DESC>
__global__ void __launch_bounds__(kGeoThreads, 3) PositionDescriptorKernel(const __grid_constant__ GeometryArgs a) {
  extern __shared__ __align__(16) unsigned char geo_smem[];
  KfDevice* s_kfs = reinterpret_cast<KfDevice*>(geo_smem);
  const uint32_t tile_len = 1u << a.tile_shift;
  const uint32_t n_tiles = (a.end - a.begin + tile_len - 1) >> a.tile_shift;
  const uint32_t n_groups = (a.kf_count + kGeoGroup - 1) / kGeoGroup;
  const uint32_t n_items = n_groups * n_tiles;
  const size_t P = a.pitch, F = a.stream_pitch;
  const int lane = threadIdx.x & 31;
  uint32_t group, tile;
  while (ClaimItem(a.queue, n_tiles, n_items, a.tile_epoch, &group, &tile)) {
    const bool first = group == 0, last = group + 1 == n_groups;
    const int j_begin = group * kGeoGroup, j_end = min(a.kf_count, static_cast<int>(group + 1) * kGeoGroup);
    KfDevice* recs = s_kfs + (threadIdx.x >> 5) * kGeoGroup;
    StageGroupRecords(a.kfs, a.kf_list + j_begin, j_end - j_begin, recs, lane);
    for (uint32_t sub = 0; sub < tile_len / 32; ++sub) {
      const uint32_t li = a.begin + (tile << a.tile_shift) + sub * 32 + lane;
      const uint32_t s = SurfelShardToGlobal(li, a.shard_rank, a.shard_world);
      const bool live = li < a.end && s < a.n && (__float_as_uint(a.stream[(kGeoStreamRows - 1) * F + s]) & kSurfelActiveFlag);
      if (__ballot_sync(0xffffffffu, live) == 0) continue;
      Vec3 gp = V3(0.f, 0.f, 0.f), nrm = V3(0.f, 0.f, 1.f);
      float radius_sq = 0.f, d1 = 0.f, d2 = 0.f;
      if (live) {
        gp = V3(a.stream[0 * F + s], a.stream[1 * F + s], a.stream[2 * F + s]);
        nrm = UnpackNormal(__float_as_uint(a.stream[3 * F + s]));
        if (USE_DESC) {
          radius_sq = a.stream[4 * F + s];
          d1 = a.stream[5 * F + s];
          d2 = a.stream[6 * F + s];
        }
      }
      float H00 = 0.f, H01 = 0.f, H02 = 0.f, H11 = 0.f, H22 = 0.f, b0 = 0.f, b1 = 0.f, b2 = 0.f;
      const float H12 = 0.f;
      if (!first && live) {
        H00 = __ldcg(a.surfels + (kRowAccum0 + 0) * P + s);
        b0 = __ldcg(a.surfels + (kRowAccum0 + 6) * P + s);
        if (USE_DESC) {
          H01 = __ldcg(a.surfels + (kRowAccum0 + 1) * P + s);
          H02 = __ldcg(a.surfels + (kRowAccum0 + 2) * P + s);
          H11 = __ldcg(a.surfels + (kRowAccum0 + 3) * P + s);
          H22 = __ldcg(a.surfels + (kRowAccum0 + 5) * P + s);
          b1 = __ldcg(a.surfels + (kRowAccum0 + 7) * P + s);
          b2 = __ldcg(a.surfels + (kRowAccum0 + 8) * P + s);
        }
      }
      float lo[3], hi[3];
      WarpBox(gp, live, lo, hi);
      unsigned vis = VisibleKeyframes<false>(a.cam, recs, j_end - j_begin, lo, hi, lane);
      auto accumulate = [&](const Assoc& r, const DescEval& e, bool photo) {
        if (USE_DEPTH) {
          float inv_stddev;
          Vec3 up;
          const float raw = DepthResidual(a.cam, r, &inv_stddev, &up);
          const float jac = -inv_stddev;
          const float w = DepthWeight(raw);
          if (USE_DESC) {
            H00 += w * jac * jac;
            b0 += w * raw * jac;
          } else {
            const float wj = w * jac;
            H00 += wj * jac;
            b0 += wj * raw;
          }
        }
        if (USE_DESC && photo) {
          const float term1 = -a.cam.cfx * (r.ln.x * r.lp.z - r.ln.z * r.lp.x);
          const float term2 = -a.cam.cfy * (r.ln.y * r.lp.z - r.ln.z * r.lp.y);
          const float term3 = 1.f / (r.lp.z * r.lp.z);
          const float j1 = -(e.gx1 * term1 + e.gy1 * term2) * term3;
          const float j2 = -(e.gx2 * term1 + e.gy2 * term2) * term3;
          constexpr float jd = -1.f;
          const float w1 = DescWeight(e.r1), wr1 = w1 * e.r1;
          const float w2 = DescWeight(e.r2), wr2 = w2 * e.r2;
          H00 += w1 * j1 * j1 + w2 * j2 * j2;
          H01 += w1 * j1 * jd;
          H11 += w1 * jd * jd;
          b0 += wr1 * j1 + wr2 * j2;
          b1 += wr1 * jd;
          H02 += w2 * j2 * jd;
          H22 += w2 * jd * jd;
          b2 += wr2 * jd;
        }
      };
      for (int j = PopLowest(&vis); j >= 0; j = PopLowest(&vis)) {
        KfRegs K;
        LoadKfShared(recs + j, &K);
        K.tex = UniformTexture(K.tex);
        Assoc r;
        if (!live || !ProjectIntoImage(a.cam, K.T, gp, &r)) continue;
        PixelLoads l;
        DescEval e;
        bool photo = false;
        if (EvalPair(a.cam, K, gp, nrm, radius_sq, d1, d2, USE_DESC, &r, &l, &e, &photo) == 3) accumulate(r, e, photo);
      }

      if (!live) continue;
      if (!last) {
        __stcg(a.surfels + (kRowAccum0 + 0) * P + s, H00);
        __stcg(a.surfels + (kRowAccum0 + 6) * P + s, b0);
        if (USE_DESC) {
          __stcg(a.surfels + (kRowAccum0 + 1) * P + s, H01);
          __stcg(a.surfels + (kRowAccum0 + 2) * P + s, H02);
          __stcg(a.surfels + (kRowAccum0 + 3) * P + s, H11);
          __stcg(a.surfels + (kRowAccum0 + 5) * P + s, H22);
          __stcg(a.surfels + (kRowAccum0 + 7) * P + s, b1);
          __stcg(a.surfels + (kRowAccum0 + 8) * P + s, b2);
        }
        continue;
      }
      const uint32_t i = a.perm ? __ldg(a.perm + s) : s;
      if (!USE_DESC) {
        if (H00 > 1e-6f) {
          const float t = -1.f * b0 / H00;
          StoreSurfelRow(a, kRowX, i, gp.x + t * nrm.x);
          StoreSurfelRow(a, kRowY, i, gp.y + t * nrm.y);
          StoreSurfelRow(a, kRowZ, i, gp.z + t * nrm.z);
        }
      } else {
        constexpr float kEpsilon = 1e-6f;
        const float L00 = sqrtf(H00 + kEpsilon);
        const float L01 = H01 / L00;
        const float L11 = sqrtf((H11 + kEpsilon) - L01 * L01);
        const float L02 = H02 / L00;
        const float L12 = (H12 - L02 * L01) / L11;
        const float L22 = sqrtf((H22 + kEpsilon) - L02 * L02 - L12 * L12);
        const float y0 = b0 / L00;
        const float y1 = (b1 - L01 * y0) / L11;
        const float y2 = (b2 - L02 * y0 - L12 * y1) / L22;
        const float x2 = y2 / L22;
        const float x1 = (y1 - L12 * x2) / L11;
        const float x0 = (y0 - L02 * x2 - L01 * x1) / L00;
        if (x0 != 0) {
          StoreSurfelRow(a, kRowX, i, gp.x - x0 * nrm.x);
          StoreSurfelRow(a, kRowY, i, gp.y - x0 * nrm.y);
          StoreSurfelRow(a, kRowZ, i, gp.z - x0 * nrm.z);
        }
        if (x1 != 0) StoreSurfelRow(a, kRowD1, i, fmaxf(-180.f, fminf(180.f, d1 - x1)));
        if (x2 != 0) StoreSurfelRow(a, kRowD2, i, fmaxf(-180.f, fminf(180.f, d2 - x2)));
      }
    }
    RetireItem(a.tile_epoch, group, tile);
  }
}

constexpr int kDeformSums = 8;
__global__ void __launch_bounds__(kGeoThreads) DeformSurfelsKernel(const __grid_constant__ DeformArgs d) {
  extern __shared__ __align__(16) unsigned char geo_smem[];
  const GeometryArgs& a = d.geo;
  KfDevice* s_kfs = reinterpret_cast<KfDevice*>(geo_smem);
  const uint32_t tile_len = 1u << a.tile_shift;
  const uint32_t n_tiles = (a.end - a.begin + tile_len - 1) >> a.tile_shift;
  const uint32_t n_groups = (a.kf_count + kGeoGroup - 1) / kGeoGroup;
  const uint32_t n_items = n_groups * n_tiles;
  const size_t F = a.stream_pitch;
  const int lane = threadIdx.x & 31;
  auto vote = [&](const KfChange* __restrict__ c, const Vec3& p, const Vec3& n, float (&v)[kDeformSums]) {
    const float* D = c->D;
    const Vec3 q = Transform(D, p);
    v[0] += q.x - p.x;
    v[1] += q.y - p.y;
    v[2] += q.z - p.z;
    const Vec3 rn = Rotate(D, n);
    v[3] += rn.x;
    v[4] += rn.y;
    v[5] += rn.z;
    v[6] += 1.f;
    if (!__ldg(&c->unmoved)) v[7] += 1.f;
  };
  uint32_t group, tile;
  while (ClaimItem(a.queue, n_tiles, n_items, a.tile_epoch, &group, &tile)) {
    const bool first = group == 0, last = group + 1 == n_groups;
    const int j_begin = group * kGeoGroup, j_end = min(a.kf_count, static_cast<int>(group + 1) * kGeoGroup);
    const int n_kf = j_end - j_begin;
    KfDevice* recs = s_kfs + (threadIdx.x >> 5) * kGeoGroup;
    StageGroupRecords(a.kfs, a.kf_list + j_begin, n_kf, recs, lane);
    for (uint32_t sub = 0; sub < tile_len / 32; ++sub) {
      uint32_t s;
      const bool in_range = GeoStreamPosition(a, tile, sub, lane, &s);
      Vec3 gp = V3(0.f, 0.f, 0.f), nrm = V3(0.f, 0.f, 1.f);
      if (in_range) gp = V3(a.stream[0 * F + s], a.stream[1 * F + s], a.stream[2 * F + s]);
      const bool live = in_range && !isnan(gp.x);
      if (__ballot_sync(0xffffffffu, live) == 0) continue;
      if (live) nrm = UnpackNormal(__float_as_uint(a.stream[3 * F + s]));
      float v[kDeformSums] = {};
      if (!first && live) LoadParkedSums(a, s, v);
      float lo[3], hi[3];
      WarpBox(gp, live, lo, hi);
      unsigned vis = VisibleKeyframes<false>(a.cam, recs, n_kf, lo, hi, lane);
      for (int j = PopLowest(&vis); j >= 0; j = PopLowest(&vis)) {
        KfRegs K;
        LoadKfShared(recs + j, &K);
        Assoc r;
        if (live && ProjectIntoImage(a.cam, K.T, gp, &r) &&
            Associate(a.cam, K.T, nrm, LoadPixel(a.cam, K.depth, K.depth_pitch, K.normals, K.normals_pitch, r), &r) == 3)
          vote(d.changes + j_begin + j, gp, nrm, v);
      }
      if (live && !last) StoreParkedSums(a, s, v);
      bool unobserved = false, moved = false;
      if (live && last) {
        unobserved = v[6] == 0.f;
        if (unobserved) {
          int best = 0;
          float best_d = INFINITY;
          for (int k = 0; k < a.kf_count; ++k) {
            const Vec3 e = gp - V3(__ldg(&d.changes[k].centre[0]), __ldg(&d.changes[k].centre[1]), __ldg(&d.changes[k].centre[2]));
            const float dist = Dot(e, e);
            if (dist < best_d) {
              best_d = dist;
              best = k;
            }
          }
          vote(d.changes + best, gp, nrm, v);
        }
        moved = v[7] != 0.f;
        if (moved) {
          const uint32_t i = GeoResultIndex(a, s);
          StoreSurfelRow(a, kRowX, i, gp.x + __fdiv_rn(v[0], v[6]));
          StoreSurfelRow(a, kRowY, i, gp.y + __fdiv_rn(v[1], v[6]));
          StoreSurfelRow(a, kRowZ, i, gp.z + __fdiv_rn(v[2], v[6]));
          const float len = __fsqrt_rn(v[3] * v[3] + v[4] * v[4] + v[5] * v[5]);
          if (len > 0.f)
            StoreSurfelRow(a, kRowNormal, i, __uint_as_float(PackNormal(V3(__fdiv_rn(v[3], len), __fdiv_rn(v[4], len), __fdiv_rn(v[5], len)))));
        }
      }
      if (last) {
        const unsigned moved_lanes = __ballot_sync(0xffffffffu, moved), unobserved_lanes = __ballot_sync(0xffffffffu, unobserved);
        if (lane == 0 && moved_lanes) atomicAdd(d.counts, __popc(moved_lanes));
        if (lane == 0 && unobserved_lanes) atomicAdd(d.counts + 1, __popc(unobserved_lanes));
      }
    }
    RetireItem(a.tile_epoch, group, tile);
  }
}

constexpr size_t kGeoSmemBytes = sizeof(KfDevice) * (kGeoThreads / 32) * kGeoGroup;

template <typename Kernel>
static LaunchResult PrepareGeo(Kernel kernel, GeometryArgs* a, int sm_count, bool desc_rows, cudaStream_t stream, uint32_t* grid) {
  int per_sm = 0;
  LaunchResult r{1, cudaOccupancyMaxActiveBlocksPerMultiprocessor(&per_sm, kernel, kGeoThreads, kGeoSmemBytes)};
  *grid = EpochOrderedGrid(per_sm, sm_count, kGeoThreads, a->end - a->begin, (a->kf_count + kGeoGroup - 1) / kGeoGroup, &a->tile_shift);
  const uint32_t n_tiles = (a->end - a->begin + (1u << a->tile_shift) - 1) >> a->tile_shift;
  r += cudaMemsetAsync(a->queue, 0, sizeof(unsigned int), stream);
  r += cudaMemsetAsync(a->tile_epoch, 0, sizeof(unsigned int) * n_tiles, stream);
  r += LaunchGeometryStream(*a, desc_rows, stream);
  return r;
}

template <typename Kernel>
static LaunchResult LaunchGeo(Kernel kernel, GeometryArgs a, int sm_count, bool desc_rows, cudaStream_t stream) {
  uint32_t grid;
  const LaunchResult r = PrepareGeo(kernel, &a, sm_count, desc_rows, stream, &grid);
  kernel<<<grid, kGeoThreads, kGeoSmemBytes, stream>>>(a);
  return r;
}

LaunchResult LaunchDeformSurfels(const DeformArgs& args, int sm_count, cudaStream_t stream) {
  if (args.geo.end <= args.geo.begin || args.geo.kf_count <= 0) return {};
  DeformArgs a = args;
  uint32_t grid;
  const LaunchResult r = PrepareGeo(DeformSurfelsKernel, &a.geo, sm_count, false, stream, &grid);
  DeformSurfelsKernel<<<grid, kGeoThreads, kGeoSmemBytes, stream>>>(a);
  return r;
}

LaunchResult LaunchActivationAndNormals(const GeometryArgs& a, int sm_count, bool determine_activation, bool update_normals,
                                        cudaStream_t stream) {
  if (a.end <= a.begin || (!determine_activation && !update_normals)) return {};
  if (a.kf_count <= 0) {
    if (determine_activation) return {0, cudaMemsetAsync(a.active, 0, a.n, stream)};
    return {};
  }
  if (determine_activation && update_normals) return LaunchGeo(ActivationNormalsKernel<true, true>, a, sm_count, false, stream);
  if (determine_activation) return LaunchGeo(ActivationNormalsKernel<true, false>, a, sm_count, false, stream);
  return LaunchGeo(ActivationNormalsKernel<false, true>, a, sm_count, false, stream);
}

LaunchResult LaunchPositionAndDescriptor(const GeometryArgs& a, int sm_count, cudaStream_t stream) {
  if (a.end <= a.begin || a.kf_count <= 0) return {};
  if (a.cam.use_desc) {
    if (a.cam.use_depth) return LaunchGeo(PositionDescriptorKernel<true, true>, a, sm_count, true, stream);
    return LaunchGeo(PositionDescriptorKernel<false, true>, a, sm_count, true, stream);
  }
  return LaunchGeo(PositionDescriptorKernel<true, false>, a, sm_count, false, stream);
}


__global__ void __launch_bounds__(256) PackShardKernel(const float* __restrict__ surfels, uint32_t pitch,
                                                       const uint8_t* __restrict__ active, uint32_t n, ShardRows rows,
                                                       const uint32_t* __restrict__ perm, uint32_t rank, uint32_t world, uint32_t shard_len,
                                                       float* __restrict__ slice) {
  const uint32_t c = blockIdx.x * blockDim.x + threadIdx.x;
  if (c >= shard_len) return;
  const uint32_t s = SurfelShardToGlobal(c, rank, world);
  const bool in = s < n;
  const uint32_t i = in && perm ? __ldg(perm + s) : s;
  float v[kShardRows];
#pragma unroll
  for (int r = 0; r < kShardRows - 1; ++r) v[r] = in && r < rows.count ? surfels[static_cast<size_t>(rows.ids[r]) * pitch + i] : 0.f;
  v[kShardRows - 1] = in && rows.active ? static_cast<float>(active[i]) : 0.f;
#pragma unroll
  for (int r = 0; r < kShardRows - 1; ++r)
    if (r < rows.count) slice[static_cast<size_t>(r) * shard_len + c] = v[r];
  if (rows.active) slice[static_cast<size_t>(rows.count) * shard_len + c] = v[kShardRows - 1];
}

__global__ void __launch_bounds__(256) UnpackShardsKernel(float* __restrict__ surfels, uint32_t pitch, uint8_t* __restrict__ active,
                                                          uint32_t n, ShardRows rows, const uint32_t* __restrict__ perm, uint32_t shard_len,
                                                          uint32_t world, int skip_rank, const float* __restrict__ buffer) {
  const uint32_t s = blockIdx.x * blockDim.x + threadIdx.x;
  if (s >= n) return;
  const uint32_t granule = s >> kShardGranuleShift;
  const uint32_t rank = granule % world;
  if (static_cast<int>(rank) == skip_rank) return;
  const uint32_t c = ((granule / world) << kShardGranuleShift) | (s & ((1u << kShardGranuleShift) - 1u));
  const uint32_t i = perm ? __ldg(perm + s) : s;
  const float* slice = buffer + static_cast<size_t>(rank) * (rows.count + rows.active) * shard_len;
  float v[kShardRows];
#pragma unroll
  for (int r = 0; r < kShardRows - 1; ++r) v[r] = r < rows.count ? slice[static_cast<size_t>(r) * shard_len + c] : 0.f;
  v[kShardRows - 1] = rows.active ? slice[static_cast<size_t>(rows.count) * shard_len + c] : 0.f;
#pragma unroll
  for (int r = 0; r < kShardRows - 1; ++r)
    if (r < rows.count) surfels[static_cast<size_t>(rows.ids[r]) * pitch + i] = v[r];
  if (rows.active) active[i] = static_cast<uint8_t>(v[kShardRows - 1]);
}

LaunchResult LaunchPackShard(const float* surfels, uint32_t pitch, const uint8_t* active, uint32_t n, ShardRows rows, const uint32_t* perm,
                             uint32_t rank, uint32_t world, uint32_t shard_len, float* slice, cudaStream_t stream) {
  if (shard_len == 0) return {};
  PackShardKernel<<<(shard_len + 255) / 256, 256, 0, stream>>>(surfels, pitch, active, n, rows, perm, rank, world, shard_len, slice);
  return {1};
}

LaunchResult LaunchUnpackShards(float* surfels, uint32_t pitch, uint8_t* active, uint32_t n, ShardRows rows, const uint32_t* perm,
                                uint32_t shard_len, int world, int skip_rank, const float* buffer, cudaStream_t stream) {
  if (n == 0) return {};
  UnpackShardsKernel<<<(n + 255) / 256, 256, 0, stream>>>(surfels, pitch, active, n, rows, perm, shard_len, static_cast<uint32_t>(world),
                                                          skip_rank, buffer);
  return {1};
}

__global__ void PackPoseResultsKernel(const int* __restrict__ ids, int n, const float* __restrict__ pose_est,
                                      const int* __restrict__ iterations, const int* __restrict__ converged,
                                      const double* __restrict__ first_stats, float* __restrict__ out) {
  const int i = blockIdx.x * blockDim.x + threadIdx.x;
  if (i >= n) return;
  const int kf = ids[i];
  float* o = out + static_cast<size_t>(kf) * kPoseSlot;
  for (int j = 0; j < 7; ++j) o[j] = pose_est[kf * 7 + j];
  o[7] = static_cast<float>(iterations[kf]);
  o[8] = static_cast<float>(converged[kf]);
  for (int j = 0; j < 8; ++j) o[9 + j] = static_cast<float>(first_stats[kf * 8 + j]);
}

LaunchResult LaunchPackPoseResults(const int* ids, int n, const float* pose_est, const int* iterations, const int* converged,
                                   const double* first_stats, float* out, cudaStream_t stream) {
  if (n <= 0) return {};
  PackPoseResultsKernel<<<(n + 127) / 128, 128, 0, stream>>>(ids, n, pose_est, iterations, converged, first_stats, out);
  return {1};
}


__global__ void __launch_bounds__(256) ExtractLumaKernel(LumaSource first, const LumaSource* __restrict__ rest,
                                                         uint8_t* __restrict__ luma, size_t luma_pitch, int w, int h) {
  const int x4 = (blockIdx.x * blockDim.x + threadIdx.x) * 4;
  const int y = blockIdx.y;
  if (x4 >= w || y >= h) return;
  const LumaSource f = blockIdx.z == 0 ? first : rest[blockIdx.z - 1];
  const uint8_t* src = f.rgba + static_cast<size_t>(y) * f.pitch + static_cast<size_t>(x4) * 4;
  uint8_t* dst = luma + (static_cast<size_t>(blockIdx.z) * h + y) * luma_pitch + x4;
  if (x4 + 3 < w && (reinterpret_cast<uintptr_t>(src) & 15) == 0 && (reinterpret_cast<uintptr_t>(dst) & 3) == 0) {
    const uint4 v = __ldg(reinterpret_cast<const uint4*>(src));
    const uint32_t packed = (v.x >> 24) | ((v.y >> 24) << 8) | ((v.z >> 24) << 16) | ((v.w >> 24) << 24);
    *reinterpret_cast<uint32_t*>(dst) = packed;
  } else {
    for (int k = 0; k < 4 && x4 + k < w; ++k) dst[k] = src[4 * k + 3];
  }
}

LaunchResult LaunchExtractLuma(LumaSource first, const LumaSource* rest, int images, uint8_t* luma, size_t luma_pitch, int w, int h,
                               cudaStream_t stream) {
  if (images <= 0) return {};
  if (images > 65535) return {0, cudaErrorInvalidValue};
  dim3 block(256);
  dim3 grid((w / 4 + 255) / 256 + 1, h, images);
  ExtractLumaKernel<<<grid, block, 0, stream>>>(first, rest, luma, luma_pitch, w, h);
  return {1};
}

}
```

badslam_b200/csrc/kernels.cuh:

```cuda
#pragma once

#include <cuda_runtime.h>
#include <stdint.h>

#include "device_math.cuh"
#include "exact_sum.cuh"
#include "launch.hpp"

namespace bba {

struct PoseTerm {
  float pose[7];
  float info[21];
};

constexpr int kPoseAccSize = 32;

struct PoseAccumulateArgs {
  CameraParams cam;
  const float* surfels;
  uint32_t pitch;
  uint32_t n;
  const KfDevice* kfs;
  const int* work_list;
  const int* work_count;
  const float* stream;
  uint32_t stream_pitch;
  const float* boxes;
  bool stream_sorted;
  KfDevice* work_records;
  int group;
  double* acc;
  ExactSum* exact;
  unsigned long long* stage_counts;
  unsigned int* queue;
};

constexpr int kPoseMaxGroup = 64;

constexpr int kSpatialChunk = 256;
struct SpatialOrderBuffers {
  uint32_t* keys_in;
  uint32_t* keys_out;
  uint32_t* index_in;
  uint32_t* perm;
  unsigned int* bounds;
  void* temp;
  size_t temp_bytes;
};
size_t SpatialOrderTempBytes(uint32_t capacity);
LaunchResult LaunchSpatialOrder(const float* surfels, uint32_t pitch, uint32_t n, const SpatialOrderBuffers& b, cudaStream_t stream);
constexpr int kPoseStreamRows = 14;
LaunchResult LaunchPoseStream(const float* surfels, uint32_t pitch, uint32_t n, const uint32_t* perm, float* stream, uint32_t stream_pitch,
                              float* boxes, cudaStream_t cuda_stream);
enum PoseVariant { kPoseVariantAuto = 0, kPoseVariant256Pre = 1, kPoseVariant512Pre = 2, kPoseVariant256 = 3, kPoseVariant512 = 4,
                   kPoseVariant1024 = 5 };
inline bool PoseVariantValid(int v) { return v >= kPoseVariantAuto && v <= kPoseVariant1024; }
inline bool PoseVariantPre(int v) { return v == kPoseVariant256Pre || v == kPoseVariant512Pre; }
LaunchResult LaunchPoseAccumulate(const PoseAccumulateArgs& args, int sm_count, bool with_stats, int max_work, cudaStream_t stream,
                                  int variant = kPoseVariantAuto);
cudaError_t SetPoseAccumulateSmemLimits();

struct PoseSolveArgs {
  KfDevice* kfs;
  float* pose_est;
  double* acc;
  ExactSum* exact;
  unsigned long long* stage_counts;
  const int* work_in;
  const int* count_in;
  int* work_out;
  int* count_out;
  int* iterations;
  int* converged;
  double* first_stats;
  unsigned long long* totals;
  volatile int* host_flag;
  unsigned int* queue;
  int iteration;
  int max_iterations;
  const int* term_offsets;
  const PoseTerm* terms;
};
LaunchResult LaunchPoseSolve(const PoseSolveArgs& args, cudaStream_t stream);

struct PoseGraphTerm {
  int a, b;
  float z[7];
  float info[21];
};
struct PoseGraphTermBlocks {
  double H[78];
  double b[12];
  double cost;
};
struct PoseGraphState {
  double initial_cost;
  double cost;
  int done;
  int iterations;
  int converged;
  int linear_iterations;
};
struct PoseGraphArgs {
  int K;
  int term_count;
  const PoseGraphTerm* terms;
  PoseGraphTermBlocks* blocks;
  float* poses;
  float* prev;
  const int* held;
  const int* row_off;
  const int* row_terms;
  const int* csr_off;
  const int* csr_col;
  double* csr_val;
  double* rhs;
  double* tri;
  double* work;
  PoseGraphState* state;
  int max_iterations;
  int max_linear;
  int round;
};
inline size_t PoseGraphWorkDoubles(size_t K) { return (2 * K + 32) * (6 * 36 + 3 * 6) + 5 * 6 * K; }
LaunchResult LaunchPoseGraphRound(const PoseGraphArgs& a, cudaStream_t stream);

constexpr int kMaxPeers = 7;
struct PeerSet {
  int count;
  float* surfels[kMaxPeers];
  uint8_t* active[kMaxPeers];
};

struct GeometryArgs {
  CameraParams cam;
  float* surfels;
  uint32_t pitch;
  uint32_t n;
  uint32_t begin, end;
  uint32_t shard_rank, shard_world;
  const uint32_t* perm;
  float* stream;
  uint32_t stream_pitch;
  uint8_t* active;
  const KfDevice* kfs;
  const int* kf_list;
  int kf_count;
  unsigned int* queue;
  unsigned int* tile_epoch;
  int tile_shift;
  PeerSet peers;
};
constexpr int kGeoStreamRows = 8;
static_assert(kGeoStreamRows <= kPoseStreamRows, "the geometry stream lives in the pose stream's buffer");
LaunchResult LaunchGeometryStream(const GeometryArgs& args, bool desc_rows, cudaStream_t stream);
LaunchResult LaunchActivationAndNormals(const GeometryArgs& args, int sm_count, bool determine_activation, bool update_normals,
                                        cudaStream_t stream);
LaunchResult LaunchPositionAndDescriptor(const GeometryArgs& args, int sm_count, cudaStream_t stream);

struct KfChange {
  float D[12];
  float centre[3];
  int unmoved;
};
struct DeformArgs {
  GeometryArgs geo;
  const KfChange* changes;
  unsigned int* counts;
};
LaunchResult LaunchDeformSurfels(const DeformArgs& a, int sm_count, cudaStream_t stream);

constexpr uint32_t kShardGranuleShift = 8;
__host__ __device__ inline uint32_t SurfelShardToGlobal(uint32_t local, uint32_t rank, uint32_t world) {
  return world <= 1 ? local : ((((local >> kShardGranuleShift) * world + rank) << kShardGranuleShift) | (local & ((1u << kShardGranuleShift) - 1u)));
}
constexpr int kShardRows = 7;
struct ShardRows {
  int ids[kShardRows - 1];
  int count;
  int active;
};
LaunchResult LaunchPackShard(const float* surfels, uint32_t pitch, const uint8_t* active, uint32_t n, ShardRows rows, const uint32_t* perm,
                             uint32_t rank, uint32_t world, uint32_t shard_len, float* slice, cudaStream_t stream);
LaunchResult LaunchUnpackShards(float* surfels, uint32_t pitch, uint8_t* active, uint32_t n, ShardRows rows, const uint32_t* perm,
                                uint32_t shard_len, int world, int skip_rank, const float* buffer, cudaStream_t stream);
constexpr int kPoseSlot = 17;
LaunchResult LaunchPackPoseResults(const int* ids, int n, const float* pose_est, const int* iterations, const int* converged,
                                   const double* first_stats, float* out, cudaStream_t stream);

constexpr int kIntrinsicsSums = 34;
struct IntrinsicsArgs {
  CameraParams cam;
  const float* surfels;
  uint32_t pitch;
  uint32_t n;
  uint32_t begin, end;
  uint32_t shard_rank, shard_world;
  const KfDevice* kfs;
  const int* kf_list;
  int kf_count;
  unsigned int* queue;
  double* sums;
  float* cell_B;
  float* cell_D;
  float* cell_b2;
  float* cell_obs;
  uint32_t cell_count;
  ExactSum* exact_cells;
  ExactSum* exact_sums;
};
LaunchResult LaunchIntrinsicsAccumulate(const IntrinsicsArgs& a, int sm_count, bool optimize_color, bool optimize_depth, cudaStream_t stream);
LaunchResult LaunchIntrinsicsFinalize(uint32_t cell_count, const ExactSum* exact_cells, float* cell_B, const ExactSum* exact_sums, double* sums,
                                      cudaStream_t stream);
LaunchResult LaunchIntrinsicsSchur(uint32_t cell_count, float* B, float* D, const float* b2, double* sums, cudaStream_t stream);
LaunchResult LaunchIntrinsicsConvertSums(double* sums, float* head, bool to_float, cudaStream_t stream);
LaunchResult LaunchIntrinsicsCellUpdate(uint32_t cell_count, const float* obs, const float* B, const float* D, const float* x1,
                                        float* cfactor, cudaStream_t stream);

struct PcgArgs {
  CameraParams cam;
  const float* surfels;
  uint32_t pitch;
  uint32_t begin, end;
  uint32_t n;
  uint32_t shard_rank, shard_world;
  int alpha_d_slot;
  const KfDevice* kfs;
  int kf_count;
  int gauge_kf;
  int opt_poses, opt_geometry, opt_depth_intr, opt_color_intr;
  uint32_t surfel_start, surfel_stride;
  uint32_t depth_intr_start, color_intr_start;
  float* r;
  float* M;
  const float* p;
  float* g;
  double* scalars;
  unsigned int* queue;
};
constexpr int kPcgPartialsA = 8, kPcgPartialsB = 8 + 2048, kPcgCounters = 8 + 4096, kPcgScalarDoubles = 8 + 4096 + 2;
LaunchResult LaunchPcgAccumulate(const PcgArgs& a, int sm_count, bool init, cudaStream_t stream);
LaunchResult LaunchPcgPackAlphaD(const double* scalars, float* tail, cudaStream_t stream);
LaunchResult LaunchPcgUnpackAlphaD(double* scalars, const float* tail, cudaStream_t stream);
LaunchResult LaunchPcgInit2(uint32_t n, uint32_t a_index, float a, int kf_count, const float* r, const float* M, float* delta, float* g, float* p,
                            double* scalars, int slot_alpha_n, int sm_count, cudaStream_t stream);
LaunchResult LaunchPcgStep2(uint32_t n, uint32_t a_index, float* r, const float* M, float* delta, float* g, const float* p, double* scalars,
                            int slot_alpha_n, int slot_beta_n, int sm_count, cudaStream_t stream);
LaunchResult LaunchPcgStep3(uint32_t n, uint32_t a_index, int kf_count, float* g, float* p, double* scalars, int slot_alpha_n, int slot_beta_n,
                            int sm_count, cudaStream_t stream);
LaunchResult LaunchPcgUpdateSurfels(float* surfels, uint32_t pitch, uint32_t n, bool use_desc, uint32_t surfel_start, const float* delta,
                                    cudaStream_t stream);
LaunchResult LaunchPcgUpdateCfactor(float* cfactor, uint32_t cells, const float* delta, cudaStream_t stream);
struct PcgPoseTerm {
  int other;
  float H[21];
  float b[6];
  float X[36];
};
struct PcgPoseBlock {
  uint32_t u;
  int begin, end;
};
LaunchResult LaunchPcgPoseTerms(const PcgPoseBlock* blocks, int block_count, const PcgPoseTerm* terms, bool init, float* r, float* M,
                                const float* p, float* g, double* alpha_d, cudaStream_t stream);

struct KfRadius {
  const uint16_t* ptr;
  uint32_t pitch;
  uint32_t pad;
};
struct SurfelStatsArgs {
  CameraParams cam;
  float* surfels;
  uint32_t pitch;
  uint32_t n;
  const KfDevice* kfs;
  const KfRadius* radius;
  int kf_count;
  int min_observation_count;
  unsigned int* queue;
  unsigned int* tile_epoch;
  int tile_shift;
  unsigned int* deleted_count;
  uint32_t local_count, shard_rank, shard_world;
  PeerSet peers;
};
LaunchResult LaunchObservationStats(SurfelStatsArgs a, int sm_count, cudaStream_t stream);
uint32_t ScanScratchWords(uint32_t n);
uint32_t ScanTotalIndex(uint32_t n);
LaunchResult LaunchCompactSurfels(float* surfels, uint32_t pitch, uint32_t n, uint32_t free_count, unsigned int* block_sums, uint8_t* active,
                                  cudaStream_t stream);

struct CovisEntry {
  float R[12];
  const uint16_t* depth;
  const uint16_t* normals;
  uint32_t depth_pitch, normals_pitch;
  uint32_t pad[2];
};
struct LifecycleArgs {
  CameraParams cam;
  float T[12];
  float G[12];
  const uint16_t* depth;
  const uint16_t* normals;
  const uint16_t* radius;
  uint32_t depth_pitch, normals_pitch, radius_pitch;
  cudaTextureObject_t tex;
  const uint8_t* rgba;
  uint32_t rgba_pitch;
  float* surfels;
// ... 28 lines not shown
```

badslam_b200/csrc/persistent.cuh:

```cuda
#pragma once

#include <algorithm>
#include <type_traits>

#include "kernels.cuh"

namespace bba {

__device__ __forceinline__ unsigned int LoadAcquire(const unsigned int* p) {
  unsigned int v;
  asm volatile("ld.acquire.gpu.global.u32 %0, [%1];" : "=r"(v) : "l"(p) : "memory");
  return v;
}
__device__ __forceinline__ void StoreRelease(unsigned int* p, unsigned int v) {
  asm volatile("st.release.gpu.global.u32 [%0], %1;" ::"l"(p), "r"(v) : "memory");
}

template <typename T>
__device__ __forceinline__ T WarpSum(T v) {
#pragma unroll
  for (int o = 16; o >= 1; o >>= 1) v += __shfl_xor_sync(0xffffffffu, v, o);
  return v;
}

template <typename T>
__device__ __forceinline__ T BlockSum(T v) {
  __shared__ T partial[32];
  const int lane = threadIdx.x & 31, warp = threadIdx.x >> 5;
  v = WarpSum(v);
  if (lane == 0) partial[warp] = v;
  __syncthreads();
  if (warp == 0) v = WarpSum(lane < static_cast<int>(blockDim.x >> 5) ? partial[lane] : T(0));
  return v;
}

__device__ __forceinline__ unsigned int BlockExclusiveScan(unsigned int v, unsigned int* total) {
  __shared__ unsigned int warp_offset[32];
  __shared__ unsigned int block_total;
  const int lane = threadIdx.x & 31, warp = threadIdx.x >> 5;
  unsigned int inc = v;
#pragma unroll
  for (int o = 1; o < 32; o <<= 1) {
    const unsigned int t = __shfl_up_sync(0xffffffffu, inc, o);
    if (lane >= o) inc += t;
  }
  if (lane == 31) warp_offset[warp] = inc;
  __syncthreads();
  if (warp == 0) {
    const unsigned int w = warp_offset[lane];
    unsigned int winc = w;
#pragma unroll
    for (int o = 1; o < 32; o <<= 1) {
      const unsigned int t = __shfl_up_sync(0xffffffffu, winc, o);
      if (lane >= o) winc += t;
    }
    warp_offset[lane] = winc - w;
    if (lane == 31) block_total = winc;
  }
  __syncthreads();
  *total = block_total;
  return warp_offset[warp] + inc - v;
}

template <int HALF, int N>
__device__ __forceinline__ void WarpTransposeStage(float (&v)[N], int lane) {
  const bool upper = (lane & HALF) != 0;
#pragma unroll
  for (int i = 0; i < HALF; ++i) {
    const float lo = v[i], hi = v[i + HALF];
    const float send = upper ? lo : hi;
    const float keep = upper ? hi : lo;
    v[i] = keep + __shfl_xor_sync(0xffffffffu, send, HALF);
  }
  if constexpr (HALF > 1) WarpTransposeStage<HALF / 2>(v, lane);
}
template <int N>
__device__ __forceinline__ float WarpTransposeReduce(float (&v)[N], int lane) {
  static_assert(N == 8 || N == 16 || N == 32, "WarpTransposeReduce: N = 8, 16 or 32");
  WarpTransposeStage<N / 2>(v, lane);
  float r = v[0];
#pragma unroll
  for (int o = N; o < 32; o <<= 1) r += __shfl_xor_sync(0xffffffffu, r, o);
  return r;
}

template <typename Epochs>
__device__ __forceinline__ bool ClaimItem(unsigned int* queue, uint32_t n_tiles, uint32_t n_items, Epochs tile_epoch, uint32_t* group,
                                          uint32_t* tile) {
  unsigned int item = 0;
  if ((threadIdx.x & 31) == 0) {
    item = atomicAdd(queue, 1u);
    if constexpr (!std::is_same<Epochs, decltype(nullptr)>::value) {
      if (item < n_items) {
        const uint32_t g = item / n_tiles, t = item - g * n_tiles;
        while (LoadAcquire(tile_epoch + t) < g) __nanosleep(64);
      }
    }
  }
  item = __shfl_sync(0xffffffffu, item, 0);
  if (item >= n_items) return false;
  *group = item / n_tiles;
  *tile = item - *group * n_tiles;
  return true;
}
__device__ __forceinline__ void RetireItem(unsigned int* tile_epoch, uint32_t group, uint32_t tile) {
  __syncwarp();
  if ((threadIdx.x & 31) == 0) {
    __threadfence();
    StoreRelease(tile_epoch + tile, group + 1);
  }
}

template <typename T>
__device__ __forceinline__ void StoreReplicas(T* local, T* const (&peers)[kMaxPeers], int peer_count, size_t o, T v) {
  local[o] = v;
#pragma unroll
  for (int p = 0; p < kMaxPeers; ++p)
    if (p < peer_count) peers[p][o] = v;
}

__device__ __forceinline__ int LoadKfShared(const KfDevice* rec, KfRegs* r) {
  const float4* p = reinterpret_cast<const float4*>(rec);
  const float4 a = p[0], b = p[1], c = p[2];
  r->T[0] = a.x; r->T[1] = a.y; r->T[2] = a.z; r->T[3] = a.w;
  r->T[4] = b.x; r->T[5] = b.y; r->T[6] = b.z; r->T[7] = b.w;
  r->T[8] = c.x; r->T[9] = c.y; r->T[10] = c.z; r->T[11] = c.w;
  const ulonglong2 q = *reinterpret_cast<const ulonglong2*>(p + 3);
  r->depth = reinterpret_cast<const uint16_t*>(q.x);
  r->normals = reinterpret_cast<const uint16_t*>(q.y);
  const ulonglong2 q2 = *reinterpret_cast<const ulonglong2*>(p + 4);
  r->tex = static_cast<cudaTextureObject_t>(q2.x);
  r->depth_pitch = static_cast<uint32_t>(q2.y & 0xffffffffu);
  r->normals_pitch = static_cast<uint32_t>(q2.y >> 32);
  const int2 tail = *reinterpret_cast<const int2*>(p + 5);
  r->activation = tail.x;
  return tail.y;
}

__device__ __forceinline__ void LoadKfGlobal(const KfDevice* __restrict__ kfs, int kf, KfRegs* r) {
  const KfDevice& k = kfs[kf];
#pragma unroll
  for (int i = 0; i < 12; ++i) r->T[i] = __ldg(&k.T[i]);
  r->depth = k.depth;
  r->normals = k.normals;
  r->tex = k.tex;
  r->depth_pitch = k.depth_pitch;
  r->normals_pitch = k.normals_pitch;
}

inline uint32_t EpochOrderedGrid(int per_sm, int sm_count, int threads, uint32_t n, uint32_t n_groups, int* tile_shift) {
  const uint64_t resident_ctas = static_cast<uint64_t>(std::max(per_sm, 1)) * sm_count;
  const uint64_t resident_warps = resident_ctas * (threads / 32);
  int shift = 8;
  while (shift > 5 && 2 * static_cast<uint64_t>((n + (1u << shift) - 1) >> shift) < 3 * resident_warps) --shift;
  *tile_shift = shift;
  const uint64_t n_items = static_cast<uint64_t>((n + (1u << shift) - 1) >> shift) * n_groups;
  return static_cast<uint32_t>(std::min<uint64_t>((n_items + threads / 32 - 1) / (threads / 32), resident_ctas));
}
inline uint32_t ItemGrid(int per_sm, int sm_count, uint64_t n_items) {
  return static_cast<uint32_t>(std::min<uint64_t>((n_items + 7) / 8, static_cast<uint64_t>(std::max(per_sm, 1)) * sm_count));
}

}
```

badslam_b200/direct_ba.py:

```python
from __future__ import annotations

import ctypes as C
from dataclasses import dataclass
from typing import List, Optional

import numpy as np
import torch

from . import _lib
from ._lib import BadBAError


@dataclass
class PinholeCamera4f:
    width: int
    height: int
    parameters: np.ndarray

    def __post_init__(self):
        self.parameters = np.asarray(self.parameters, dtype=np.float32).copy()

    def Scaled(self, factor: float) -> "PinholeCamera4f":
        factor = float(factor)
        return PinholeCamera4f(int(factor * self.width + 0.5), int(factor * self.height + 0.5),
# ... 419 lines not shown
        self._check(self._lib.bba_set_keyframe_states(self._h, K, None if p is None else p.ctypes.data,
                                                      None if a is None else a.ctypes.data))

    def GetKeyframeStates(self):
        K = len(self._keyframes)
        p = np.zeros((K, 7), np.float32)
        a = np.zeros(K, np.int32)
        self._check(self._lib.bba_get_keyframe_states(self._h, K, p.ctypes.data, a.ctypes.data))
        return p, a

    def SetKeyframePosePriors(self, ids, poses, information):
        ids = np.ascontiguousarray(np.atleast_1d(ids), np.int32)
        n = len(ids)
        p = np.ascontiguousarray(np.asarray(poses, np.float32).reshape(n, 7))
        L = np.asarray(information, np.float32)
        if L.shape[-2:] == (6, 6):
            L = np.broadcast_to(L, (n, 6, 6))[:, np.triu_indices(6)[0], np.triu_indices(6)[1]]
        L = np.ascontiguousarray(np.broadcast_to(L.reshape(-1, 21), (n, 21)), np.float32)
        self._check(self._lib.bba_set_keyframe_pose_priors(self._h, n, ids.ctypes.data, p.ctypes.data, L.ctypes.data))

    def ClearKeyframePosePriors(self, ids=None):
        if ids is None:
            self._check(self._lib.bba_clear_keyframe_pose_priors(self._h, -1, None))
            return
        ids = np.ascontiguousarray(np.atleast_1d(ids), np.int32)
        self._check(self._lib.bba_clear_keyframe_pose_priors(self._h, len(ids), ids.ctypes.data))

    def KeyframePosePrior(self, keyframe_id: int):
        p, L, has = np.zeros(7, np.float32), np.zeros(21, np.float32), C.c_int()
        self._check(self._lib.bba_get_keyframe_pose_prior(self._h, keyframe_id, p.ctypes.data, L.ctypes.data, C.byref(has)))
        return (p, L) if has.value else None

    def AddKeyframePoseConstraints(self, a_ids, b_ids, a_T_b, information) -> np.ndarray:
        a = np.atleast_1d(np.asarray(a_ids, np.int64))
        b = np.atleast_1d(np.asarray(b_ids, np.int64))
        n = len(a)
        if len(b) != n:
            raise ValueError("a_ids and b_ids differ in length")
        Z = np.asarray(a_T_b, np.float32).reshape(n, 7)
        L = np.asarray(information, np.float32)
        if L.shape[-2:] == (6, 6):
            L = np.broadcast_to(L, (n, 6, 6))[:, np.triu_indices(6)[0], np.triu_indices(6)[1]]
        L = np.broadcast_to(L.reshape(-1, 21), (n, 21))
        recs = (_lib.PoseConstraint * max(n, 1))()
        for i in range(n):
            recs[i].keyframe_a, recs[i].keyframe_b = int(a[i]), int(b[i])
            recs[i].a_T_b[:] = [float(v) for v in Z[i]]
            recs[i].information[:] = [float(v) for v in L[i]]
        ids = np.zeros(max(n, 1), np.int32)
        self._check(self._lib.bba_add_keyframe_pose_constraints(self._h, n, recs, ids.ctypes.data))
        return ids[:n]

    def RemoveKeyframePoseConstraints(self, ids=None):
        if ids is None:
            self._check(self._lib.bba_remove_keyframe_pose_constraints(self._h, -1, None))
            return
        ids = np.ascontiguousarray(np.atleast_1d(ids), np.int32)
        self._check(self._lib.bba_remove_keyframe_pose_constraints(self._h, len(ids), ids.ctypes.data))

    def KeyframePoseConstraints(self):
        count = C.c_int()
        self._check(self._lib.bba_get_keyframe_pose_constraints(self._h, 0, None, None, C.byref(count)))
        n = count.value
        ids = np.zeros(max(n, 1), np.int32)
        recs = (_lib.PoseConstraint * max(n, 1))()
        self._check(self._lib.bba_get_keyframe_pose_constraints(self._h, n, ids.ctypes.data, recs, C.byref(count)))
        n = min(n, count.value)
        a = np.array([recs[i].keyframe_a for i in range(n)], np.int32)
        b = np.array([recs[i].keyframe_b for i in range(n)], np.int32)
        Z = np.array([list(recs[i].a_T_b) for i in range(n)], np.float32).reshape(n, 7)
        L = np.array([list(recs[i].information) for i in range(n)], np.float32).reshape(n, 21)
        return ids[:n], a, b, Z, L

    def OptimizePoseGraph(self, add_current_state_odometry_constraints=True, gauge_keyframe=0, max_iterations=20,
                          odometry_information=None, stream=None) -> dict:
        o = _lib.PoseGraphOptions()
        o.gauge_keyframe = int(gauge_keyframe)
        o.max_iterations = int(max_iterations)
        o.use_odometry_chain = int(bool(add_current_state_odometry_constraints))
        L = np.eye(6, dtype=np.float32) if odometry_information is None else np.asarray(odometry_information, np.float32)
        if L.shape == (6, 6):
            L = L[np.triu_indices(6)]
        o.odometry_information[:] = [float(v) for v in L.reshape(21)]
        r = _lib.PoseGraphResult()
        self._check(self._lib.bba_optimize_pose_graph(self._h, C.byref(o), C.byref(r), self._stream_ptr(stream)))
        return {name: getattr(r, name) for name, _ in _lib.PoseGraphResult._fields_}

    def RememberKeyframePoses(self) -> np.ndarray:
        K = self._lib.bba_keyframe_count(self._h)
        p = np.zeros((K, 7), np.float32)
        self._check(self._lib.bba_get_keyframe_states(self._h, K, p.ctypes.data, None))
        out = np.empty_like(p)
        for k in range(K):
            self._lib.bba_host_se3_inverse(p[k].ctypes.data, out[k].ctypes.data)
        return out

    def ExtrapolateAndInterpolateKeyframePoseChanges(self, start_frame: int, end_frame: int, original_keyframe_T_global,
                                                     keyframe_frame_indices, frame_poses: np.ndarray) -> np.ndarray:
        K = len(original_keyframe_T_global)
        current = np.zeros((K, 7), np.float32)
        self._check(self._lib.bba_get_keyframe_states(self._h, K, current.ctypes.data, None))
        return deform_trajectory(start_frame, end_frame, keyframe_frame_indices, original_keyframe_T_global, current, frame_poses)

    def DeformSurfelsWithKeyframePoseChanges(self, original_keyframe_T_global, stream=None):
        original = np.ascontiguousarray(original_keyframe_T_global, np.float32).reshape(-1, 7)
        moved, unobserved = C.c_uint32(), C.c_uint32()
        self._check(self._lib.bba_deform_surfels(self._h, len(original), original.ctypes.data, C.byref(moved), C.byref(unobserved),
                                                 self._stream_ptr(stream)))
        return moved.value, unobserved.value

    def SurfelsDeviceView(self) -> torch.Tensor:
        if self._surfels is not None:
            return self._surfels
        ptr, pitch, n = C.c_void_p(), C.c_size_t(), C.c_uint32()
        self._check(self._lib.bba_get_surfels_device(self._h, C.byref(ptr), C.byref(pitch), C.byref(n)))

        class _Raw:
            pass
        raw = _Raw()
        raw.__cuda_array_interface__ = {"shape": (17, pitch.value // 4), "typestr": "<f4", "data": (ptr.value, False),
                                        "version": 2, "strides": None}
        self._raw_keepalive = raw
        return torch.as_tensor(raw, device=self.device)

    def covisibility(self) -> np.ndarray:
        K = len(self._keyframes)
        out = np.zeros((K, K), np.uint8)
        for k in range(K):
            self._check(self._lib.bba_get_covisibility(self._h, k, out[k].ctypes.data))
        return out

    def AccumulatePoseEstimationCoeffs(self, keyframe_id: int, global_T_frame_estimate, stream=None):
        p = np.ascontiguousarray(global_T_frame_estimate, np.float32)
        out = _lib.PoseCoeffs()
        self._check(self._lib.bba_accumulate_pose_coeffs(self._h, keyframe_id, p.ctypes.data_as(C.POINTER(C.c_float)),
                                                         C.byref(out), self._stream_ptr(stream)))
        return out

    def PoseCoeffsBatch(self, keyframe_ids, global_T_frame_estimates, variant: int = _lib.POSE_VARIANT_AUTO, with_stats: bool = True,
                        stream=None):
        ids = np.ascontiguousarray(keyframe_ids, np.int32)
        poses = np.ascontiguousarray(global_T_frame_estimates, np.float32).reshape(len(ids), 7)
        K = len(self._keyframes)
        H, b, costs = np.zeros((K, 21)), np.zeros((K, 6)), np.zeros((K, 3))
        counts = np.zeros((K, 4), np.uint64)
        self._check(self._lib.bba_debug_pose_coeffs_batch(self._h, len(ids), ids.ctypes.data, poses.ctypes.data, int(variant),
                                                          int(with_stats), H.ctypes.data, b.ctypes.data, counts.ctypes.data,
                                                          costs.ctypes.data, self._stream_ptr(stream)))
        return H, b, counts, costs

    def DebugSetPoseGroup(self, keyframes: int):
        self._check(self._lib.bba_debug_set_pose_group(self._h, int(keyframes)))

    def EstimateFramePose(self, stream, global_T_frame_initial_estimate, keyframe_id: int):
        p = np.ascontiguousarray(global_T_frame_initial_estimate, np.float32)
        out = np.zeros(7, np.float32)
        it, conv = C.c_int(), C.c_int()
        self._check(self._lib.bba_estimate_frame_pose(self._h, keyframe_id, p.ctypes.data_as(C.POINTER(C.c_float)),
                                                      out.ctypes.data_as(C.POINTER(C.c_float)), C.byref(it), C.byref(conv),
                                                      self._stream_ptr(stream)))
        return out, it.value, bool(conv.value)

    def EstimateFramePoseFromBuffers(self, stream, global_T_frame_initial_estimate, depth_buffer: torch.Tensor,
                                     normals_buffer: torch.Tensor, color_buffer: torch.Tensor):
        p = np.ascontiguousarray(global_T_frame_initial_estimate, np.float32)
        out = np.zeros(7, np.float32)
        it, conv = C.c_int(), C.c_int()
        self._check(self._lib.bba_estimate_frame_pose_for_frame(
            self._h, depth_buffer.data_ptr(), depth_buffer.stride(0) * 2, normals_buffer.data_ptr(), normals_buffer.stride(0) * 2,
            color_buffer.data_ptr(), color_buffer.stride(0), p.ctypes.data_as(C.POINTER(C.c_float)),
            out.ctypes.data_as(C.POINTER(C.c_float)), C.byref(it), C.byref(conv), self._stream_ptr(stream)))
        return out, it.value, bool(conv.value)

    def EstimateFramePosesFromBuffers(self, stream, frames, initial_poses, frame_of_entry=None, with_coeffs: bool = False):
        bufs = _frame_buffers(frames)
        init = np.ascontiguousarray(initial_poses, np.float32).reshape(-1, 7)
        count = len(init)
        fmap = None if frame_of_entry is None else np.ascontiguousarray(frame_of_entry, np.int32)
        out = np.zeros((count, 7), np.float32)
        it, conv = np.zeros(count, np.int32), np.zeros(count, np.int32)
        coeffs = (_lib.PoseCoeffs * count)() if with_coeffs else None
        self._check(self._lib.bba_estimate_frame_poses_for_frames(
            self._h, len(frames), bufs, count, None if fmap is None else fmap.ctypes.data, init.ctypes.data, out.ctypes.data,
            it.ctypes.data, conv.ctypes.data, coeffs, self._stream_ptr(stream)))
        if with_coeffs:
            return out, it, conv.astype(bool), list(coeffs)
        return out, it, conv.astype(bool)

    def TrackFramePairwise(self, stream, base_keyframe_id: int, depth_buffer: torch.Tensor, normals_buffer: torch.Tensor,
                           color_buffer: torch.Tensor, base_T_frame_initial_estimate_1, base_T_frame_initial_estimate_2=None,
                           num_scales: int = 5, use_pyramid_level_0: bool = True, use_gradmag: bool = False,
                           test_different_initial_estimates: bool = True, max_iterations_per_scale: int = 30):
        p1 = np.ascontiguousarray(base_T_frame_initial_estimate_1, np.float32)
        p2 = p1 if base_T_frame_initial_estimate_2 is None else np.ascontiguousarray(base_T_frame_initial_estimate_2, np.float32)
        out = np.zeros(7, np.float32)
        o = _odometry_options(num_scales, use_pyramid_level_0, use_gradmag, test_different_initial_estimates, max_iterations_per_scale)
        res = _lib.OdometryResult()
        F = C.POINTER(C.c_float)
        self._check(self._lib.bba_track_frame_pairwise(
            self._h, C.byref(o), int(base_keyframe_id), depth_buffer.data_ptr(), depth_buffer.stride(0) * 2, normals_buffer.data_ptr(),
            normals_buffer.stride(0) * 2, color_buffer.data_ptr(), color_buffer.stride(0), p1.ctypes.data_as(F), p2.ctypes.data_as(F),
            out.ctypes.data_as(F), C.byref(res), self._stream_ptr(stream)))
        return out, res

    def TrackFramePairwiseToFrame(self, stream, base_depth_buffer: torch.Tensor, base_normals_buffer: torch.Tensor,
                                  base_color_buffer: torch.Tensor, depth_buffer: torch.Tensor, normals_buffer: torch.Tensor,
                                  color_buffer: torch.Tensor, base_T_frame_initial_estimate_1, base_T_frame_initial_estimate_2=None,
                                  num_scales: int = 5, use_pyramid_level_0: bool = True, use_gradmag: bool = False,
                                  test_different_initial_estimates: bool = True, max_iterations_per_scale: int = 30):
        p1 = np.ascontiguousarray(base_T_frame_initial_estimate_1, np.float32)
        p2 = p1 if base_T_frame_initial_estimate_2 is None else np.ascontiguousarray(base_T_frame_initial_estimate_2, np.float32)
        out = np.zeros(7, np.float32)
        o = _odometry_options(num_scales, use_pyramid_level_0, use_gradmag, test_different_initial_estimates, max_iterations_per_scale)
        res = _lib.OdometryResult()
        F = C.POINTER(C.c_float)
        self._check(self._lib.bba_track_frame_pairwise_to_frame(
            self._h, C.byref(o), base_depth_buffer.data_ptr(), base_depth_buffer.stride(0) * 2, base_normals_buffer.data_ptr(),
            base_normals_buffer.stride(0) * 2, base_color_buffer.data_ptr(), base_color_buffer.stride(0),
            depth_buffer.data_ptr(), depth_buffer.stride(0) * 2, normals_buffer.data_ptr(), normals_buffer.stride(0) * 2,
            color_buffer.data_ptr(), color_buffer.stride(0), p1.ctypes.data_as(F), p2.ctypes.data_as(F), out.ctypes.data_as(F),
            C.byref(res), self._stream_ptr(stream)))
        return out, res

    def TrackFramesPairwise(self, stream, frames, entries, num_scales: int = 5, use_pyramid_level_0: bool = True,
                            use_gradmag: bool = False, test_different_initial_estimates: bool = True, max_iterations_per_scale: int = 30):
        bufs = _frame_buffers(frames)
        ents = (_lib.OdometryEntry * len(entries))()
        for e, spec in zip(ents, entries):
            e.base_keyframe_id, e.base_frame, e.tracked_frame = int(spec[0]), int(spec[1]), int(spec[2])
            p1 = np.ascontiguousarray(spec[3], np.float32).reshape(7)
            p2 = p1 if len(spec) < 5 or spec[4] is None else np.ascontiguousarray(spec[4], np.float32).reshape(7)
            e.base_T_frame_initial_1[:] = p1.tolist()
            e.base_T_frame_initial_2[:] = p2.tolist()
        count = len(entries)
        out = np.zeros((count, 7), np.float32)
        results = (_lib.OdometryResult * count)()
        launches = C.c_uint32()
        o = _odometry_options(num_scales, use_pyramid_level_0, use_gradmag, test_different_initial_estimates, max_iterations_per_scale)
        self._check(self._lib.bba_track_frames_pairwise(self._h, C.byref(o), len(frames), bufs, count, ents, out.ctypes.data, results,
                                                        C.byref(launches), self._stream_ptr(stream)))
        return out, list(results), launches.value

    def OdometryLevel(self, which: int, scale: int, stream=None):
        w, h = C.c_int(), C.c_int()
        self._check(self._lib.bba_odometry_get_level(self._h, which, scale, None, None, None, C.byref(w), C.byref(h), self._stream_ptr(stream)))
        d = np.zeros((h.value, w.value), np.float32)
        n = np.zeros((h.value, w.value), np.uint16)
        c = np.zeros((h.value, w.value), np.uint8)
        self._check(self._lib.bba_odometry_get_level(self._h, which, scale, d.ctypes.data, n.ctypes.data, c.ctypes.data, C.byref(w),
                                                     C.byref(h), self._stream_ptr(stream)))
        return d, n, c

    def OdometryCoeffs(self, scale: int, base_T_frame_a, base_T_frame_b=None, use_gradmag: bool = False, stream=None):
        pa = np.ascontiguousarray(base_T_frame_a, np.float32)
        pb = pa if base_T_frame_b is None else np.ascontiguousarray(base_T_frame_b, np.float32)
        H, b = np.zeros(21, np.float32), np.zeros(6, np.float32)
        cnt, rs = C.c_uint32(), C.c_float()
        counts, costs = np.zeros(2, np.uint32), np.zeros(2, np.float32)
        F = C.POINTER(C.c_float)
        self._check(self._lib.bba_odometry_debug_coeffs(self._h, scale, int(use_gradmag), pa.ctypes.data_as(F), pb.ctypes.data_as(F),
                                                        H.ctypes.data, b.ctypes.data, C.byref(cnt), C.byref(rs), counts.ctypes.data,
                                                        costs.ctypes.data, self._stream_ptr(stream)))
        return H, b, cnt.value, rs.value, counts, costs

    def UpdateSurfelActivation(self, stream=None):
        self._check(self._lib.bba_update_surfel_activation(self._h, self._stream_ptr(stream)))

    def OptimizeGeometryIteration(self, stream=None):
        self._check(self._lib.bba_optimize_geometry_iteration(self._h, self._stream_ptr(stream)))

    def OptimizeIntrinsics(self, optimize_depth_intrinsics: bool, optimize_color_intrinsics: bool, stream=None):
        self._check(self._lib.bba_optimize_intrinsics(self._h, int(optimize_depth_intrinsics),
                                                      int(optimize_color_intrinsics), self._stream_ptr(stream)))

    def IntrinsicsCoeffs(self, optimize_depth_intrinsics: bool, optimize_color_intrinsics: bool, stream=None):
        w, h = C.c_int(), C.c_int()
        self._check(self._lib.bba_cfactor_size(self._h, C.byref(w), C.byref(h)))
        sums, cells = np.zeros(34), np.zeros((8, w.value * h.value), np.float32)
        self._check(self._lib.bba_debug_intrinsics_coeffs(self._h, int(optimize_depth_intrinsics), int(optimize_color_intrinsics),
                                                          sums.ctypes.data, cells.ctypes.data, self._stream_ptr(stream)))
        return sums, cells

    def BundleAdjustment(self, stream, optimize_depth_intrinsics: bool, optimize_color_intrinsics: bool,
                         do_surfel_updates: bool, optimize_poses: bool, optimize_geometry: bool,
                         min_iterations: int, max_iterations: int, use_pcg: bool = False,
                         active_keyframe_window_start: int = 0, active_keyframe_window_end: int = -1,
                         increase_ba_iteration_count: bool = True, time_limit: float = 0.0,
                         pcg_max_inner_iterations: int = 30, pcg_max_keyframes: int = 2500,
                         pcg_gauge_keyframe: int = -1, progress_function=None) -> BAResult:
        if active_keyframe_window_end < 0:
            active_keyframe_window_end = len(self._keyframes) - 1
        o = _lib.BAOptions(int(optimize_depth_intrinsics), int(optimize_color_intrinsics), int(do_surfel_updates),
                           int(optimize_poses), int(optimize_geometry), int(min_iterations), int(max_iterations),
                           int(use_pcg), int(active_keyframe_window_start), int(active_keyframe_window_end),
                           int(increase_ba_iteration_count), float(time_limit), int(pcg_max_inner_iterations),
                           int(pcg_max_keyframes), int(pcg_gauge_keyframe))
        if progress_function is not None:
            cb = _lib.PROGRESS_FN(lambda _user, iteration: 1 if progress_function(int(iteration)) else 0)
            o.progress_function = cb
        r = _lib.BAResult()
        self._check(self._lib.bba_bundle_adjust(self._h, C.byref(o), C.byref(r), self._stream_ptr(stream)))
        return BAResult(r.iterations_done, bool(r.converged), r.depth_residual_count, r.descriptor_residual_count,
                        r.cost, r.pose_iterations_total, r.ms_surfel_activation, r.ms_geometry_optimization,
                        r.ms_pose_optimization, r.ms_intrinsics_optimization, r.kernel_launches,
                        r.pcg_inner_iterations_total, r.pcg_last_r_norm, r.ms_pcg, r.surfels_deleted, r.surfels_size,
                        r.surfels_created, r.surfels_merged)
# ... 267 lines not shown
```

include/badba.h:

```cpp
#ifndef BADBA_H
#define BADBA_H

#include <stddef.h>
#include <stdint.h>

#ifdef __cplusplus
extern "C" {
#endif

#define BBA_ABI_VERSION 10

typedef struct bba_context* bba_handle;

typedef enum {
  BBA_OK = 0,
  BBA_ERR_INVALID_ARGUMENT = 1,
  BBA_ERR_CUDA = 2,
  BBA_ERR_STATE = 3,
  BBA_ERR_UNSUPPORTED = 4,
  BBA_ERR_NO_DEVICE = 5
} bba_status;

typedef enum { BBA_KF_ACTIVE = 0, BBA_KF_COVISIBLE_ACTIVE = 1, BBA_KF_INACTIVE = 2 } bba_kf_activation;

typedef struct {
  int depth_width, depth_height;
  int color_width, color_height;
  float depth_intrinsics[4];
  float color_intrinsics[4];
  float raw_to_float_depth;
  float baseline_fx;
  int sparse_surfel_cell_size;
  uint32_t max_surfel_count;
  int max_keyframes;
  int use_depth_residuals;
  int use_descriptor_residuals;
  int device;
  int rank, world_size;
  int min_observation_count_while_bootstrapping_1;
  int min_observation_count_while_bootstrapping_2;
  int min_observation_count;
  float surfel_merge_dist_factor;
} bba_config;

typedef struct {
  int optimize_depth_intrinsics;
  int optimize_color_intrinsics;
  int do_surfel_updates;
  int optimize_poses;
  int optimize_geometry;
  int min_iterations;
  int max_iterations;
  int use_pcg;
  int active_keyframe_window_start;
  int active_keyframe_window_end;
  int increase_ba_iteration_count;
  double time_limit_seconds;
  int pcg_max_inner_iterations;
  int pcg_max_keyframes;
  int pcg_gauge_keyframe;
  int (*progress_function)(void* user, int iteration);
  void* progress_user;
} bba_ba_options;

typedef struct {
  int iterations_done;
  int converged;
  uint64_t depth_residual_count;
  uint64_t descriptor_residual_count;
  double cost;
  int pose_iterations_total;
  float ms_surfel_activation;
  float ms_geometry_optimization;
  float ms_pose_optimization;
  float ms_intrinsics_optimization;
  uint64_t kernel_launches;
  int pcg_inner_iterations_total;
  float pcg_last_r_norm;
  float ms_pcg;
  uint32_t surfels_deleted;
  uint32_t surfels_size;
  uint32_t surfels_created;
  uint32_t surfels_merged;
} bba_ba_result;

typedef struct {
  float H[21];
  float b[6];
  uint64_t n_pair, n_inimg, n_depthok, n_assoc, n_photo;
  double cost_depth, cost_desc1, cost_desc2;
} bba_pose_coeffs;

typedef enum { BBA_COLLECTIVE_ALLGATHER = 0, BBA_COLLECTIVE_ALLREDUCE_SUM = 1 } bba_collective_op;
typedef void (*bba_collective_fn)(void* user, int op, void* device_buffer, size_t count, void* stream);

int         bba_abi_version(void);
bba_status  bba_create(const bba_config* config, bba_handle* out);
void        bba_destroy(bba_handle h);
const char* bba_last_error(bba_handle h);

bba_status bba_set_surfels(bba_handle h, float* device_surfels, size_t pitch_bytes, uint32_t surfels_size);
bba_status bba_set_active_flags(bba_handle h, uint8_t* device_flags);
bba_status bba_set_surfels_host(bba_handle h, const float* host_surfels, size_t pitch_bytes, uint32_t surfels_size, void* stream);
bba_status bba_get_surfels_host(bba_handle h, float* host_surfels, size_t pitch_bytes, int rows, void* stream);
bba_status bba_get_active_flags_host(bba_handle h, uint8_t* host_flags, void* stream);
bba_status bba_get_surfels_device(bba_handle h, float** device_surfels, size_t* pitch_bytes, uint32_t* surfels_size);

bba_status bba_add_keyframe(bba_handle h,
                            const uint16_t* device_depth, size_t depth_pitch,
                            const uint16_t* device_normals, size_t normals_pitch,
                            const uint16_t* device_radius, size_t radius_pitch,
                            const uint8_t* device_color_rgba, size_t color_pitch,
                            const float global_T_frame[7], float min_depth, float max_depth,
                            void* stream, int* out_keyframe_id);
bba_status bba_add_keyframe_host(bba_handle h,
                                 const uint16_t* host_depth, const uint16_t* host_normals,
                                 const uint16_t* host_radius, const uint8_t* host_color_rgba,
                                 const float global_T_frame[7], float min_depth, float max_depth,
                                 void* stream, int* out_keyframe_id);
int        bba_keyframe_count(bba_handle h);
bba_status bba_set_keyframe_pose(bba_handle h, int keyframe_id, const float global_T_frame[7]);
bba_status bba_get_keyframe_pose(bba_handle h, int keyframe_id, float global_T_frame[7]);
bba_status bba_set_keyframe_activation(bba_handle h, int keyframe_id, int activation);
bba_status bba_get_keyframe_activation(bba_handle h, int keyframe_id, int* activation);
bba_status bba_set_keyframe_states(bba_handle h, int count, const float* global_T_frame, const int* activation);
bba_status bba_get_keyframe_states(bba_handle h, int count, float* global_T_frame, int* activation);
bba_status bba_get_covisibility(bba_handle h, int keyframe_id, uint8_t* out_row );
bba_status bba_set_keyframe_pose_priors(bba_handle h, int count, const int* keyframe_ids, const float* prior_global_T_frame,
                                        const float* information);
bba_status bba_clear_keyframe_pose_priors(bba_handle h, int count, const int* keyframe_ids);
bba_status bba_get_keyframe_pose_prior(bba_handle h, int keyframe_id, float prior_global_T_frame[7], float information[21],
                                       int* has_prior);
typedef struct {
  int keyframe_a, keyframe_b;
  float a_T_b[7];
  float information[21];
} bba_pose_constraint;
bba_status bba_add_keyframe_pose_constraints(bba_handle h, int count, const bba_pose_constraint* constraints, int* out_ids);
bba_status bba_remove_keyframe_pose_constraints(bba_handle h, int count, const int* ids);
bba_status bba_get_keyframe_pose_constraints(bba_handle h, int capacity, int* ids, bba_pose_constraint* out, int* count);

bba_status bba_set_intrinsics(bba_handle h, const float depth_intrinsics[4], const float color_intrinsics[4], float depth_a);
bba_status bba_get_intrinsics(bba_handle h, float depth_intrinsics[4], float color_intrinsics[4], float* depth_a);
bba_status bba_set_residual_types(bba_handle h, int use_depth_residuals, int use_descriptor_residuals);
bba_status bba_get_residual_types(bba_handle h, int* use_depth_residuals, int* use_descriptor_residuals);
bba_status bba_set_cfactor_host(bba_handle h, const float* host_cfactor , void* stream);
bba_status bba_get_cfactor_host(bba_handle h, float* host_cfactor, void* stream);
bba_status bba_cfactor_size(bba_handle h, int* cf_width, int* cf_height);

bba_status bba_accumulate_pose_coeffs(bba_handle h, int keyframe_id, const float global_T_frame_estimate[7],
                                      bba_pose_coeffs* out, void* stream);
typedef enum {
  BBA_POSE_VARIANT_AUTO = 0,
  BBA_POSE_VARIANT_256_PRE = 1,
  BBA_POSE_VARIANT_512_PRE = 2,
  BBA_POSE_VARIANT_256 = 3,
  BBA_POSE_VARIANT_512 = 4,
  BBA_POSE_VARIANT_1024 = 5
} bba_pose_variant;
bba_status bba_debug_pose_coeffs_batch(bba_handle h, int count, const int* keyframe_ids, const float* global_T_frame, int variant,
                                       int with_stats, double* H, double* b, uint64_t* counts, double* costs, void* stream);
bba_status bba_debug_set_pose_group(bba_handle h, int keyframes);
bba_status bba_estimate_frame_pose(bba_handle h, int keyframe_id, const float global_T_frame_initial[7],
                                   float global_T_frame_out[7], int* iterations, int* converged, void* stream);
bba_status bba_estimate_frame_pose_for_frame(bba_handle h, const uint16_t* device_depth, size_t depth_pitch,
                                             const uint16_t* device_normals, size_t normals_pitch,
                                             const uint8_t* device_color_rgba, size_t color_pitch,
                                             const float global_T_frame_initial[7], float global_T_frame_estimate[7],
                                             int* iterations, int* converged, void* stream);
typedef struct {
  const uint16_t* depth;      size_t depth_pitch;
  const uint16_t* normals;    size_t normals_pitch;
  const uint8_t*  color_rgba; size_t color_pitch;
} bba_frame_buffers;
bba_status bba_estimate_frame_poses_for_frames(bba_handle h, int frame_count, const bba_frame_buffers* frames, int count,
                                               const int* frame_of_entry, const float* global_T_frame_initial,
                                               float* global_T_frame_estimate, int* iterations, int* converged,
                                               bba_pose_coeffs* at_estimate, void* stream);
bba_status bba_update_surfel_activation(bba_handle h, void* stream);
bba_status bba_optimize_geometry_iteration(bba_handle h, void* stream);
bba_status bba_deform_surfels(bba_handle h, int count, const float* original_keyframe_T_global, uint32_t* moved, uint32_t* unobserved,
                              void* stream);
typedef struct {
  int gauge_keyframe;
  int max_iterations;
  int use_odometry_chain;
  float odometry_information[21];
} bba_pose_graph_options;
typedef struct {
  int iterations, converged, linear_iterations, held_keyframes;
  double initial_cost, final_cost;
} bba_pose_graph_result;
bba_status bba_optimize_pose_graph(bba_handle h, const bba_pose_graph_options* options, bba_pose_graph_result* result, void* stream);
bba_status bba_perform_end_tasks(bba_handle h, int do_surfel_updates, uint32_t* deleted, uint32_t* surfels_size, void* stream);
uint32_t bba_surfels_size(bba_handle h);
bba_status bba_get_ba_iteration_counts(bba_handle h, int* ba_iteration_count, int* last_ba_iteration_count);
bba_status bba_set_ba_iteration_counts(bba_handle h, int ba_iteration_count, int last_ba_iteration_count);

bba_status bba_create_surfels_for_keyframe(bba_handle h, int keyframe_id, int filter_new_surfels, uint32_t* created, void* stream);
bba_status bba_merge_surfels_for_keyframe(bba_handle h, int keyframe_id, uint32_t* deleted, void* stream);
bba_status bba_compact_surfels(bba_handle h, uint32_t free_count, int with_active_flags, uint32_t* surfels_size, void* stream);

typedef struct bba_pcg_probe {
  float* r;
  float* M;
  float* p;
  float* g;
  float* delta;
  double alpha_n;
  double alpha_d;
  float* r_step2;
  float* delta_step2;
  float* z;
  double beta_n;
  float* p_step3;
  float* g_step3;
  double alpha_d_step3;
} bba_pcg_probe;
bba_status bba_pcg_debug(bba_handle h, const bba_ba_options* o, int step, int apply, uint32_t* unknown_count, bba_pcg_probe* out,
                         void* stream);

bba_status bba_optimize_intrinsics(bba_handle h, int optimize_depth_intrinsics, int optimize_color_intrinsics, void* stream);
bba_status bba_debug_intrinsics_coeffs(bba_handle h, int optimize_depth_intrinsics, int optimize_color_intrinsics, double* sums,
                                       float* cells, void* stream);
bba_status bba_bundle_adjust(bba_handle h, const bba_ba_options* options, bba_ba_result* result, void* stream);

bba_status bba_set_collective(bba_handle h, bba_collective_fn fn, void* user);
typedef struct {
  unsigned char surfels_ipc[64];
  uint64_t surfels_offset;
  unsigned char active_ipc[64];
  uint64_t active_offset;
  uint64_t pitch_bytes;
  uint32_t surfels_size;
  int32_t rank;
} bba_peer_handle;
bba_status bba_peer_export(bba_handle h, bba_peer_handle* out);
bba_status bba_peer_import(bba_handle h, const bba_peer_handle* all_ranks, int count);
int bba_peer_count(bba_handle h);
bba_status bba_peer_unmap(bba_handle h);
bba_status bba_mark_replica_rewritten(bba_handle h);

int      bba_shard_surfel_owner(uint32_t surfel_index, int world_size);
uint32_t bba_shard_surfel_local_index(uint32_t surfel_index, int world_size);
uint32_t bba_shard_slice_length(uint32_t surfels_size, int world_size);
int  bba_shard_keyframe_owner(int list_index, int world_size);
void bba_balance_keyframes(const float* cost, int count, int world_size, int* owner);

typedef struct bba_local_group_s* bba_local_group;
bba_status bba_local_group_create(const bba_handle* ranks, int count, int peer_stores, bba_local_group* out);
bba_status bba_local_group_reset(bba_local_group g);
bba_status bba_local_group_poison(bba_local_group g);
void       bba_local_group_destroy(bba_local_group g);
bba_status bba_debug_collective(bba_handle h, int op, void* device_buffer, size_t count, void* stream);

bba_status bba_update_keyframe_host(bba_handle h, int keyframe_id,
                                    const uint16_t* host_depth, const uint16_t* host_normals,
                                    const uint16_t* host_radius, const uint8_t* host_color_rgba, void* stream);

typedef struct {
  float bilateral_filter_sigma_xy;
  float bilateral_filter_sigma_inv_depth;
  float bilateral_filter_radius_factor;
  float max_depth;
} bba_preprocess_options;
bba_status bba_preprocess_frame(bba_handle h, const bba_preprocess_options* options,
                                const uint16_t* device_raw_depth, size_t raw_depth_pitch,
                                const uint8_t* device_rgb, size_t rgb_pitch,
                                uint16_t* device_depth, size_t depth_pitch,
                                uint16_t* device_normals, size_t normals_pitch,
                                uint16_t* device_radius, size_t radius_pitch,
                                uint8_t* device_color_rgba, size_t color_pitch,
                                float* min_depth, float* max_depth, void* stream);

typedef struct {
  bba_preprocess_options base;
  int median_filter_and_densify_iterations;
  int pyramid_level_for_depth;
  int pyramid_level_for_color;
} bba_raw_frame_options;
bba_status bba_preprocess_raw_frame(bba_handle h, const bba_raw_frame_options* options,
                                    const uint16_t* device_raw_depth, size_t raw_depth_pitch,
                                    int raw_depth_width, int raw_depth_height,
                                    const uint8_t* device_rgb, size_t rgb_pitch, int rgb_width, int rgb_height,
                                    uint16_t* device_depth, size_t depth_pitch,
                                    uint16_t* device_normals, size_t normals_pitch,
                                    uint16_t* device_radius, size_t radius_pitch,
                                    uint8_t* device_color_rgba, size_t color_pitch,
                                    float* min_depth, float* max_depth, void* stream);

typedef struct {
  int num_scales;
  int use_pyramid_level_0;
  int use_gradmag;
  int test_different_initial_estimates;
  int max_iterations_per_scale;
} bba_odometry_options;
typedef struct {
  int iterations[8];
  int chose_initial[8];
  uint32_t residual_count;
  float residual_sum;
  uint32_t passes;
  uint32_t kernel_launches;
} bba_odometry_result;
bba_status bba_track_frame_pairwise(bba_handle h, const bba_odometry_options* options, int base_keyframe_id,
                                    const uint16_t* device_depth, size_t depth_pitch,
                                    const uint16_t* device_normals, size_t normals_pitch,
                                    const uint8_t* device_color_rgba, size_t color_pitch,
                                    const float base_T_frame_initial_1[7], const float base_T_frame_initial_2[7],
                                    float base_T_frame_estimate[7], bba_odometry_result* result, void* stream);
bba_status bba_track_frame_pairwise_to_frame(bba_handle h, const bba_odometry_options* options,
                                             const uint16_t* base_depth, size_t base_depth_pitch,
                                             const uint16_t* base_normals, size_t base_normals_pitch,
                                             const uint8_t* base_color_rgba, size_t base_color_pitch,
// ... 74 lines not shown
```

Before: 26.89 billion.

## Fuse activation/normal and position/descriptor geometry kernels into one tiled pass

Adds a single GeometryPassKernel that, for each surfel tile, computes keyframe visibility once, updates activation and normals, then accumulates and solves the position/descriptor update, all with keyframe records in shared memory (up to 512 keyframes). This replaces two separate kernels and the parked partial sums they write to and reload from global memory. It is the default when the keyframe count fits and no new surfels were added; otherwise the old split path runs. The fused kernel runs both walks over all keyframes in one block and uses more shared memory, which can lower occupancy.

```diff
diff --git a/badslam_b200/_lib.py b/badslam_b200/_lib.py
--- a/badslam_b200/_lib.py
+++ b/badslam_b200/_lib.py
@@ -9,6 +9,7 @@
 ABI_VERSION = 10
 
 POSE_VARIANT_AUTO, POSE_VARIANT_256_PRE, POSE_VARIANT_512_PRE, POSE_VARIANT_256, POSE_VARIANT_512, POSE_VARIANT_1024 = range(6)
+GEOMETRY_PASS_AUTO, GEOMETRY_PASS_SPLIT, GEOMETRY_PASS_ONE = range(3)
 
 OK, ERR_INVALID_ARGUMENT, ERR_CUDA, ERR_STATE, ERR_UNSUPPORTED, ERR_NO_DEVICE = range(6)
 STATUS_NAMES = {0: "BBA_OK", 1: "BBA_ERR_INVALID_ARGUMENT", 2: "BBA_ERR_CUDA", 3: "BBA_ERR_STATE",
@@ -186,6 +187,7 @@
     "bba_accumulate_pose_coeffs": (C.c_int, [_P, C.c_int, _F7, C.POINTER(PoseCoeffs), _P]),
     "bba_debug_pose_coeffs_batch": (C.c_int, [_P, C.c_int, _P, _P, C.c_int, C.c_int, _P, _P, _P, _P, _P]),
     "bba_debug_set_pose_group": (C.c_int, [_P, C.c_int]),
+    "bba_debug_set_geometry_pass": (C.c_int, [_P, C.c_int, C.c_int]),
     "bba_estimate_frame_pose": (C.c_int, [_P, C.c_int, _F7, _F7, C.POINTER(C.c_int), C.POINTER(C.c_int), _P]),
     "bba_estimate_frame_pose_for_frame": (C.c_int, [_P, _P, C.c_size_t, _P, C.c_size_t, _P, C.c_size_t, _F7, _F7,
                                                     C.POINTER(C.c_int), C.POINTER(C.c_int), _P]),
diff --git a/badslam_b200/csrc/bundle_adjust.cu b/badslam_b200/csrc/bundle_adjust.cu
--- a/badslam_b200/csrc/bundle_adjust.cu
+++ b/badslam_b200/csrc/bundle_adjust.cu
@@ -732,6 +732,10 @@
   return EndBundleAdjust(h, o, launches_before, res, s);
 }
 
+bool OneGeometryPass(bba_handle h, const bba::GeometryArgs& g) {
+  return h->geo.pass != BBA_GEOMETRY_PASS_SPLIT && bba::GeometryPassFits(g);
+}
+
 bba_status GeometryPass(bba_handle h, bool activation, cudaStream_t s) {
   if (!h) return BBA_ERR_INVALID_ARGUMENT;
   if (bba_status st = CheckSurfels(h)) return st;
@@ -740,8 +744,13 @@
   bba::GeometryArgs g;
   if (bba_status st = BuildGeometryArgs(h, &g, s, GeoOrder::kSpatial)) return st;
   if (bba_status st = CheckCollective(h)) return st;
-  BBA_LAUNCH(h, h->launches, LaunchActivationAndNormals, g, h->sm_count, activation, !activation, s);
-  if (!activation) BBA_LAUNCH(h, h->launches, LaunchPositionAndDescriptor, g, h->sm_count, s);
+  if (!activation && OneGeometryPass(h, g)) {
+    BBA_LAUNCH(h, h->launches, LaunchGeometryStream, g, g.cam.use_desc, s);
+    BBA_LAUNCH(h, h->launches, LaunchGeometryPass, g, h->sm_count, false, h->geo.pass_tile_shift, s);
+  } else {
+    BBA_LAUNCH(h, h->launches, LaunchActivationAndNormals, g, h->sm_count, activation, !activation, s);
+    if (!activation) BBA_LAUNCH(h, h->launches, LaunchPositionAndDescriptor, g, h->sm_count, s);
+  }
   if (bba_status st = ExchangeGeometry(h, s)) return st;
   return MarkStaging(h, s);
 }
@@ -1055,6 +1064,17 @@
   return OptimizeIntrinsics(h, optimize_depth != 0, optimize_color != 0, static_cast<cudaStream_t>(stream));
 }
 
+bba_status bba_debug_set_geometry_pass(bba_handle h, int pass, int tile_shift) {
+  if (!h) return BBA_ERR_INVALID_ARGUMENT;
+  if (pass < BBA_GEOMETRY_PASS_AUTO || pass > BBA_GEOMETRY_PASS_ONE)
+    return Fail(h, BBA_ERR_INVALID_ARGUMENT, "bba_debug_set_geometry_pass: unknown pass");
+  if (tile_shift != 0 && (tile_shift < 5 || tile_shift > 8))
+    return Fail(h, BBA_ERR_INVALID_ARGUMENT, "bba_debug_set_geometry_pass: tile_shift out of range (0, 5 .. 8)");
+  h->geo.pass = pass;
+  h->geo.pass_tile_shift = tile_shift;
+  return BBA_OK;
+}
+
 bba_status bba_debug_intrinsics_coeffs(bba_handle h, int optimize_depth, int optimize_color, double* sums, float* cells, void* stream) {
   if (!h) return BBA_ERR_INVALID_ARGUMENT;
   if (!sums || !cells) return Fail(h, BBA_ERR_INVALID_ARGUMENT, "bba_debug_intrinsics_coeffs: null argument");
@@ -1126,12 +1146,15 @@
     if (bba_status st = BuildGeometryArgs(h, &g, s, has_new ? GeoOrder::kCaller : GeoOrder::kByPairs)) return st;
 
     BBA_TRACE("after creation + upload");
+    const bool one_pass = o->optimize_geometry && !has_new && h->surfels_size > 0 && OneGeometryPass(h, g);
     BBA_CUDA(h, cudaEventRecord(h->ev[0], s));
     if (has_new)
       BBA_CUDA(h, cudaMemsetAsync(h->active + old_surfels_size, bba::kSurfelActiveFlag, h->surfels_size - old_surfels_size, s));
     if (!whole_window) BBA_CUDA(h, cudaMemsetAsync(h->active, bba::kSurfelActiveFlag, old_surfels_size, s));
     if (h->surfels_size > 0) {
-      if (whole_window && has_new) {
+      if (one_pass) {
+        BBA_LAUNCH(h, h->launches, LaunchGeometryStream, g, g.cam.use_desc, s);
+      } else if (whole_window && has_new) {
         bba::GeometryArgs g_old = g, g_new = g;
         g_old.end = LocalCountBelow(old_surfels_size, h->cfg.rank, h->cfg.world_size);
         g_new.begin = g_old.end;
@@ -1144,7 +1167,8 @@
       }
     }
     BBA_CUDA(h, cudaEventRecord(h->ev[1], s));
-    if (o->optimize_geometry && h->surfels_size > 0) BBA_LAUNCH(h, h->launches, LaunchPositionAndDescriptor, g, h->sm_count, s);
+    if (one_pass) BBA_LAUNCH(h, h->launches, LaunchGeometryPass, g, h->sm_count, whole_window, h->geo.pass_tile_shift, s);
+    else if (o->optimize_geometry && h->surfels_size > 0) BBA_LAUNCH(h, h->launches, LaunchPositionAndDescriptor, g, h->sm_count, s);
     if (bba_status st = ExchangeGeometry(h, s)) return st;
     BBA_CUDA(h, cudaEventRecord(h->ev[2], s));
     if (bba_status st = MarkStaging(h, s)) return st;
@@ -1211,7 +1235,7 @@
     if (h->profiling) {
       h->profile.activation_normals_ms += res->ms_surfel_activation;
       h->profile.position_descriptor_ms += res->ms_geometry_optimization;
-      h->profile.geometry_launches += (o->optimize_geometry ? 2 : 1);
+      h->profile.geometry_launches += one_pass ? 1 : (o->optimize_geometry ? 2 : 1);
     }
 
     if (StopIterating(o, iteration, num_converged, K, t_start, res)) break;
diff --git a/badslam_b200/csrc/handle.hpp b/badslam_b200/csrc/handle.hpp
--- a/badslam_b200/csrc/handle.hpp
+++ b/badslam_b200/csrc/handle.hpp
@@ -226,6 +226,8 @@
     bba::PinnedBuffer<int> h_list;
     bba::DeviceBuffer<unsigned int> d_queue;
     bba::DeviceBuffer<unsigned int> d_tile_epoch;
+    int pass = BBA_GEOMETRY_PASS_AUTO;
+    int pass_tile_shift = 0;
     const uint32_t* perm = nullptr;
     bba::DeviceBuffer<float> d_intr;
     bba::DeviceBuffer<double> d_intr_sums;
diff --git a/badslam_b200/csrc/kernels.cu b/badslam_b200/csrc/kernels.cu
--- a/badslam_b200/csrc/kernels.cu
+++ b/badslam_b200/csrc/kernels.cu
@@ -572,6 +572,92 @@
   for (int r = 0; r < N; ++r) __stcg(a.surfels + (kRowAccum0 + r) * static_cast<size_t>(a.pitch) + s, v[r]);
 }
 
+__device__ __forceinline__ void AddPairNormal(const float* __restrict__ T, const Assoc& r, float (&n)[4]) {
+  const Vec3 ln = U16ToImageSpaceNormal(r.kf_normal);
+  n[0] += T[0] * ln.x + T[4] * ln.y + T[8] * ln.z;
+  n[1] += T[1] * ln.x + T[5] * ln.y + T[9] * ln.z;
+  n[2] += T[2] * ln.x + T[6] * ln.y + T[10] * ln.z;
+  n[3] += 1.f;
+}
+__device__ __forceinline__ uint32_t PackedMeanNormal(const float (&n)[4]) {
+  const float inv = 1.f / n[3];
+  return PackNormal(V3(inv * n[0], inv * n[1], inv * n[2]));
+}
+
+struct PositionSums {
+  float H00 = 0.f, H01 = 0.f, H02 = 0.f, H11 = 0.f, H22 = 0.f, b0 = 0.f, b1 = 0.f, b2 = 0.f;
+};
+template <bool USE_DEPTH, bool USE_DESC>
+__device__ __forceinline__ void AccumulatePosition(const CameraParams& cam, const Assoc& r, const DescEval& e, bool photo, PositionSums& q) {
+  if (USE_DEPTH) {
+    float inv_stddev;
+    Vec3 up;
+    const float raw = DepthResidual(cam, r, &inv_stddev, &up);
+    const float jac = -inv_stddev;
+    const float w = DepthWeight(raw);
+    if (USE_DESC) {
+      q.H00 += w * jac * jac;
+      q.b0 += w * raw * jac;
+    } else {
+      const float wj = w * jac;
+      q.H00 += wj * jac;
+      q.b0 += wj * raw;
+    }
+  }
+  if (USE_DESC && photo) {
+    const float term1 = -cam.cfx * (r.ln.x * r.lp.z - r.ln.z * r.lp.x);
+    const float term2 = -cam.cfy * (r.ln.y * r.lp.z - r.ln.z * r.lp.y);
+    const float term3 = 1.f / (r.lp.z * r.lp.z);
+    const float j1 = -(e.gx1 * term1 + e.gy1 * term2) * term3;
+    const float j2 = -(e.gx2 * term1 + e.gy2 * term2) * term3;
+    constexpr float jd = -1.f;
+    const float w1 = DescWeight(e.r1), wr1 = w1 * e.r1;
+    const float w2 = DescWeight(e.r2), wr2 = w2 * e.r2;
+    q.H00 += w1 * j1 * j1 + w2 * j2 * j2;
+    q.H01 += w1 * j1 * jd;
+    q.H11 += w1 * jd * jd;
+    q.b0 += wr1 * j1 + wr2 * j2;
+    q.b1 += wr1 * jd;
+    q.H02 += w2 * j2 * jd;
+    q.H22 += w2 * jd * jd;
+    q.b2 += wr2 * jd;
+  }
+}
+template <bool USE_DESC>
+__device__ __forceinline__ void UpdatePosition(const GeometryArgs& a, uint32_t i, const Vec3& gp, const Vec3& nrm, float d1, float d2,
+                                               const PositionSums& q) {
+  if (!USE_DESC) {
+    if (q.H00 > 1e-6f) {
+      const float t = -1.f * q.b0 / q.H00;
+      StoreSurfelRow(a, kRowX, i, gp.x + t * nrm.x);
+      StoreSurfelRow(a, kRowY, i, gp.y + t * nrm.y);
+      StoreSurfelRow(a, kRowZ, i, gp.z + t * nrm.z);
+    }
+  } else {
+    constexpr float kEpsilon = 1e-6f;
+    constexpr float H12 = 0.f;
+    const float L00 = sqrtf(q.H00 + kEpsilon);
+    const float L01 = q.H01 / L00;
+    const float L11 = sqrtf((q.H11 + kEpsilon) - L01 * L01);
+    const float L02 = q.H02 / L00;
+    const float L12 = (H12 - L02 * L01) / L11;
+    const float L22 = sqrtf((q.H22 + kEpsilon) - L02 * L02 - L12 * L12);
+    const float y0 = q.b0 / L00;
+    const float y1 = (q.b1 - L01 * y0) / L11;
+    const float y2 = (q.b2 - L02 * y0 - L12 * y1) / L22;
+    const float x2 = y2 / L22;
+    const float x1 = (y1 - L12 * x2) / L11;
+    const float x0 = (y0 - L02 * x2 - L01 * x1) / L00;
+    if (x0 != 0) {
+      StoreSurfelRow(a, kRowX, i, gp.x - x0 * nrm.x);
+      StoreSurfelRow(a, kRowY, i, gp.y - x0 * nrm.y);
+      StoreSurfelRow(a, kRowZ, i, gp.z - x0 * nrm.z);
+    }
+    if (x1 != 0) StoreSurfelRow(a, kRowD1, i, fmaxf(-180.f, fminf(180.f, d1 - x1)));
+    if (x2 != 0) StoreSurfelRow(a, kRowD2, i, fmaxf(-180.f, fminf(180.f, d2 - x2)));
+  }
+}
+
 template <bool DETERMINE, bool NORMALS>
 __global__ void __launch_bounds__(kGeoThreads) ActivationNormalsKernel(const __grid_constant__ GeometryArgs a) {
   extern __shared__ __align__(16) unsigned char geo_smem[];
@@ -596,14 +682,9 @@
       const bool live = in_range && (DETERMINE || (flags & kSurfelActiveFlag));
       if (__ballot_sync(0xffffffffu, live) == 0) continue;
       bool act = !DETERMINE;
-      float s0 = 0.f, s1 = 0.f, s2 = 0.f, s3 = 0.f;
+      float ns[4] = {0.f, 0.f, 0.f, 0.f};
       if (!first && live) {
-        if (NORMALS) {
-          s0 = __ldcg(a.surfels + (kRowAccum0 + 0) * P + s);
-          s1 = __ldcg(a.surfels + (kRowAccum0 + 1) * P + s);
-          s2 = __ldcg(a.surfels + (kRowAccum0 + 2) * P + s);
-          s3 = __ldcg(a.surfels + (kRowAccum0 + 3) * P + s);
-        }
+        if (NORMALS) LoadParkedSums(a, s, ns);
         if (DETERMINE) act = __ldcg(a.surfels + (kRowAccum0 + 4) * P + s) != 0.f;
       }
       const bool walk = live && (NORMALS || !act);
@@ -619,13 +700,7 @@
         auto accumulate = [&](const KfRegs& K, const PixelLoads& l, Assoc& r) {
           if (Associate(a.cam, K.T, nrm, l, &r) != 3) return;
           if (K.activation == 0) act = true;
-          if (NORMALS) {
-            const Vec3 ln = U16ToImageSpaceNormal(r.kf_normal);
-            s0 += K.T[0] * ln.x + K.T[4] * ln.y + K.T[8] * ln.z;
-            s1 += K.T[1] * ln.x + K.T[5] * ln.y + K.T[9] * ln.z;
-            s2 += K.T[2] * ln.x + K.T[6] * ln.y + K.T[10] * ln.z;
-            s3 += 1.f;
-          }
+          if (NORMALS) AddPairNormal(K.T, r, ns);
         };
         for (int j = PopLowest(&vis); j >= 0; j = PopLowest(&vis)) {
           KfRegs K;
@@ -638,20 +713,12 @@
       }
       if (!live) continue;
       if (!last) {
-        if (NORMALS) {
-          __stcg(a.surfels + (kRowAccum0 + 0) * P + s, s0);
-          __stcg(a.surfels + (kRowAccum0 + 1) * P + s, s1);
-          __stcg(a.surfels + (kRowAccum0 + 2) * P + s, s2);
-          __stcg(a.surfels + (kRowAccum0 + 3) * P + s, s3);
-        }
+        if (NORMALS) StoreParkedSums(a, s, ns);
         if (DETERMINE) __stcg(a.surfels + (kRowAccum0 + 4) * P + s, act ? 1.f : 0.f);
       } else {
         const uint32_t i = GeoResultIndex(a, s);
         if (DETERMINE) StoreReplicas(a.active, a.peers.active, a.peers.count, i, act ? kSurfelActiveFlag : static_cast<uint8_t>(flags & ~kSurfelActiveFlag));
-        if (NORMALS && act && s3 >= 1.f) {
-          const float inv = 1.f / s3;
-          StoreSurfelRow(a, kRowNormal, i, __uint_as_float(PackNormal(V3(inv * s0, inv * s1, inv * s2))));
-        }
+        if (NORMALS && act && ns[3] >= 1.f) StoreSurfelRow(a, kRowNormal, i, __uint_as_float(PackedMeanNormal(ns)));
       }
     }
     RetireItem(a.tile_epoch, group, tile);
@@ -690,58 +757,22 @@
           d2 = a.stream[6 * F + s];
         }
       }
-      float H00 = 0.f, H01 = 0.f, H02 = 0.f, H11 = 0.f, H22 = 0.f, b0 = 0.f, b1 = 0.f, b2 = 0.f;
-      const float H12 = 0.f;
+      PositionSums q;
       if (!first && live) {
-        H00 = __ldcg(a.surfels + (kRowAccum0 + 0) * P + s);
-        b0 = __ldcg(a.surfels + (kRowAccum0 + 6) * P + s);
+        q.H00 = __ldcg(a.surfels + (kRowAccum0 + 0) * P + s);
+        q.b0 = __ldcg(a.surfels + (kRowAccum0 + 6) * P + s);
         if (USE_DESC) {
-          H01 = __ldcg(a.surfels + (kRowAccum0 + 1) * P + s);
-          H02 = __ldcg(a.surfels + (kRowAccum0 + 2) * P + s);
-          H11 = __ldcg(a.surfels + (kRowAccum0 + 3) * P + s);
-          H22 = __ldcg(a.surfels + (kRowAccum0 + 5) * P + s);
-          b1 = __ldcg(a.surfels + (kRowAccum0 + 7) * P + s);
-          b2 = __ldcg(a.surfels + (kRowAccum0 + 8) * P + s);
+          q.H01 = __ldcg(a.surfels + (kRowAccum0 + 1) * P + s);
+          q.H02 = __ldcg(a.surfels + (kRowAccum0 + 2) * P + s);
+          q.H11 = __ldcg(a.surfels + (kRowAccum0 + 3) * P + s);
+          q.H22 = __ldcg(a.surfels + (kRowAccum0 + 5) * P + s);
+          q.b1 = __ldcg(a.surfels + (kRowAccum0 + 7) * P + s);
+          q.b2 = __ldcg(a.surfels + (kRowAccum0 + 8) * P + s);
         }
       }
       float lo[3], hi[3];
       WarpBox(gp, live, lo, hi);
       unsigned vis = VisibleKeyframes<false>(a.cam, recs, j_end - j_begin, lo, hi, lane);
-      auto accumulate = [&](const Assoc& r, const DescEval& e, bool photo) {
-        if (USE_DEPTH) {
-          float inv_stddev;
-          Vec3 up;
-          const float raw = DepthResidual(a.cam, r, &inv_stddev, &up);
-          const float jac = -inv_stddev;
-          const float w = DepthWeight(raw);
-          if (USE_DESC) {
-            H00 += w * jac * jac;
-            b0 += w * raw * jac;
-          } else {
-            const float wj = w * jac;
-            H00 += wj * jac;
-            b0 += wj * raw;
-          }
-        }
-        if (USE_DESC && photo) {
-          const float term1 = -a.cam.cfx * (r.ln.x * r.lp.z - r.ln.z * r.lp.x);
-          const float term2 = -a.cam.cfy * (r.ln.y * r.lp.z - r.ln.z * r.lp.y);
-          const float term3 = 1.f / (r.lp.z * r.lp.z);
-          const float j1 = -(e.gx1 * term1 + e.gy1 * term2) * term3;
-          const float j2 = -(e.gx2 * term1 + e.gy2 * term2) * term3;
-          constexpr float jd = -1.f;
-          const float w1 = DescWeight(e.r1), wr1 = w1 * e.r1;
-          const float w2 = DescWeight(e.r2), wr2 = w2 * e.r2;
-          H00 += w1 * j1 * j1 + w2 * j2 * j2;
-          H01 += w1 * j1 * jd;
-          H11 += w1 * jd * jd;
-          b0 += wr1 * j1 + wr2 * j2;
-          b1 += wr1 * jd;
-          H02 += w2 * j2 * jd;
-          H22 += w2 * jd * jd;
-          b2 += wr2 * jd;
-        }
-      };
       for (int j = PopLowest(&vis); j >= 0; j = PopLowest(&vis)) {
         KfRegs K;
         LoadKfShared(recs + j, &K);
@@ -751,55 +782,123 @@
         PixelLoads l;
         DescEval e;
         bool photo = false;
-        if (EvalPair(a.cam, K, gp, nrm, radius_sq, d1, d2, USE_DESC, &r, &l, &e, &photo) == 3) accumulate(r, e, photo);
+        if (EvalPair(a.cam, K, gp, nrm, radius_sq, d1, d2, USE_DESC, &r, &l, &e, &photo) == 3)
+          AccumulatePosition<USE_DEPTH, USE_DESC>(a.cam, r, e, photo, q);
       }
 
       if (!live) continue;
       if (!last) {
-        __stcg(a.surfels + (kRowAccum0 + 0) * P + s, H00);
-        __stcg(a.surfels + (kRowAccum0 + 6) * P + s, b0);
+        __stcg(a.surfels + (kRowAccum0 + 0) * P + s, q.H00);
+        __stcg(a.surfels + (kRowAccum0 + 6) * P + s, q.b0);
         if (USE_DESC) {
-          __stcg(a.surfels + (kRowAccum0 + 1) * P + s, H01);
-          __stcg(a.surfels + (kRowAccum0 + 2) * P + s, H02);
-          __stcg(a.surfels + (kRowAccum0 + 3) * P + s, H11);
-          __stcg(a.surfels + (kRowAccum0 + 5) * P + s, H22);
-          __stcg(a.surfels + (kRowAccum0 + 7) * P + s, b1);
-          __stcg(a.surfels + (kRowAccum0 + 8) * P + s, b2);
+          __stcg(a.surfels + (kRowAccum0 + 1) * P + s, q.H01);
+          __stcg(a.surfels + (kRowAccum0 + 2) * P + s, q.H02);
+          __stcg(a.surfels + (kRowAccum0 + 3) * P + s, q.H11);
+          __stcg(a.surfels + (kRowAccum0 + 5) * P + s, q.H22);
+          __stcg(a.surfels + (kRowAccum0 + 7) * P + s, q.b1);
+          __stcg(a.surfels + (kRowAccum0 + 8) * P + s, q.b2);
         }
         continue;
       }
-      const uint32_t i = a.perm ? __ldg(a.perm + s) : s;
-      if (!USE_DESC) {
-        if (H00 > 1e-6f) {
-          const float t = -1.f * b0 / H00;
-          StoreSurfelRow(a, kRowX, i, gp.x + t * nrm.x);
-          StoreSurfelRow(a, kRowY, i, gp.y + t * nrm.y);
-          StoreSurfelRow(a, kRowZ, i, gp.z + t * nrm.z);
-        }
-      } else {
-        constexpr float kEpsilon = 1e-6f;
-        const float L00 = sqrtf(H00 + kEpsilon);
-        const float L01 = H01 / L00;
-        const float L11 = sqrtf((H11 + kEpsilon) - L01 * L01);
-        const float L02 = H02 / L00;
-        const float L12 = (H12 - L02 * L01) / L11;
-        const float L22 = sqrtf((H22 + kEpsilon) - L02 * L02 - L12 * L12);
-        const float y0 = b0 / L00;
-        const float y1 = (b1 - L01 * y0) / L11;
-        const float y2 = (b2 - L02 * y0 - L12 * y1) / L22;
-        const float x2 = y2 / L22;
-        const float x1 = (y1 - L12 * x2) / L11;
-        const float x0 = (y0 - L02 * x2 - L01 * x1) / L00;
-        if (x0 != 0) {
-          StoreSurfelRow(a, kRowX, i, gp.x - x0 * nrm.x);
-          StoreSurfelRow(a, kRowY, i, gp.y - x0 * nrm.y);
-          StoreSurfelRow(a, kRowZ, i, gp.z - x0 * nrm.z);
-        }
-        if (x1 != 0) StoreSurfelRow(a, kRowD1, i, fmaxf(-180.f, fminf(180.f, d1 - x1)));
-        if (x2 != 0) StoreSurfelRow(a, kRowD2, i, fmaxf(-180.f, fminf(180.f, d2 - x2)));
-      }
+      UpdatePosition<USE_DESC>(a, GeoResultIndex(a, s), gp, nrm, d1, d2, q);
     }
     RetireItem(a.tile_epoch, group, tile);
+  }
+}
+
+template <bool DETERMINE, bool USE_DEPTH, bool USE_DESC>
+__global__ void __launch_bounds__(kGeoThreads, 3) GeometryPassKernel(const __grid_constant__ GeometryArgs a) {
+  extern __shared__ __align__(16) unsigned char geo_smem[];
+  KfDevice* recs = reinterpret_cast<KfDevice*>(geo_smem);
+  const int n_kf = a.kf_count;
+  constexpr int kWords = sizeof(KfDevice) / 16;
+  for (int idx = threadIdx.x; idx < n_kf * kWords; idx += blockDim.x) {
+    const int rec = idx / kWords, part = idx - rec * kWords;
+    reinterpret_cast<uint4*>(recs + rec)[part] = __ldg(reinterpret_cast<const uint4*>(a.kfs + __ldg(a.kf_list + rec)) + part);
+  }
+  __syncthreads();
+  const uint32_t tile_len = 1u << a.tile_shift;
+  const uint32_t n_tiles = (a.end - a.begin + tile_len - 1) >> a.tile_shift;
+  const int n_words = (n_kf + 31) / 32;
+  const size_t F = a.stream_pitch;
+  const int lane = threadIdx.x & 31;
+  uint32_t unused, tile;
+  while (ClaimItem(a.queue, n_tiles, n_tiles, nullptr, &unused, &tile)) {
+    for (uint32_t sub = 0; sub < tile_len / 32; ++sub) {
+      uint32_t s;
+      const bool in_range = GeoStreamPosition(a, tile, sub, lane, &s);
+      const uint32_t flags = in_range ? __float_as_uint(a.stream[(kGeoStreamRows - 1) * F + s]) : 0u;
+      const bool live = in_range && (DETERMINE || (flags & kSurfelActiveFlag));
+      if (__ballot_sync(0xffffffffu, live) == 0) continue;
+      Vec3 gp = V3(0.f, 0.f, 0.f);
+      uint32_t packed = 0u;
+      if (live) {
+        gp = V3(a.stream[0 * F + s], a.stream[1 * F + s], a.stream[2 * F + s]);
+        packed = __float_as_uint(a.stream[3 * F + s]);
+      }
+      float lo[3], hi[3];
+      WarpBox(gp, live, lo, hi);
+      unsigned vis_word = 0u;
+      for (int g = 0; g < n_words; ++g) {
+        const unsigned v = VisibleKeyframes<false>(a.cam, recs + 32 * g, min(32, n_kf - 32 * g), lo, hi, lane);
+        if (lane == g) vis_word = v;
+      }
+
+      bool act = !DETERMINE;
+      float ns[4] = {0.f, 0.f, 0.f, 0.f};
+      {
+        const Vec3 nrm = UnpackNormal(packed);
+        for (int g = 0; g < n_words; ++g) {
+          unsigned vis = __shfl_sync(0xffffffffu, vis_word, g);
+          for (int j = PopLowest(&vis); j >= 0; j = PopLowest(&vis)) {
+            KfRegs K;
+            LoadKfShared(recs + 32 * g + j, &K);
+            Assoc r;
+            if (live && ProjectIntoImage(a.cam, K.T, gp, &r) &&
+                Associate(a.cam, K.T, nrm, LoadPixel(a.cam, K.depth, K.depth_pitch, K.normals, K.normals_pitch, r), &r) == 3) {
+              if (K.activation == 0) act = true;
+              AddPairNormal(K.T, r, ns);
+            }
+          }
+        }
+      }
+      uint32_t i = 0;
+      if (live) {
+        i = GeoResultIndex(a, s);
+        if (DETERMINE) StoreReplicas(a.active, a.peers.active, a.peers.count, i, act ? kSurfelActiveFlag : static_cast<uint8_t>(flags & ~kSurfelActiveFlag));
+        if (act && ns[3] >= 1.f) {
+          packed = PackedMeanNormal(ns);
+          StoreSurfelRow(a, kRowNormal, i, __uint_as_float(packed));
+        }
+      }
+
+      const bool update = live && act;
+      if (__ballot_sync(0xffffffffu, update) == 0) continue;
+      const Vec3 nrm = UnpackNormal(packed);
+      float radius_sq = 0.f, d1 = 0.f, d2 = 0.f;
+      if (USE_DESC && update) {
+        radius_sq = a.stream[4 * F + s];
+        d1 = a.stream[5 * F + s];
+        d2 = a.stream[6 * F + s];
+      }
+      PositionSums q;
+      for (int g = 0; g < n_words; ++g) {
+        unsigned vis = __shfl_sync(0xffffffffu, vis_word, g);
+        for (int j = PopLowest(&vis); j >= 0; j = PopLowest(&vis)) {
+          KfRegs K;
+          LoadKfShared(recs + 32 * g + j, &K);
+          K.tex = UniformTexture(K.tex);
+          Assoc r;
+          if (!update || !ProjectIntoImage(a.cam, K.T, gp, &r)) continue;
+          PixelLoads l;
+          DescEval e;
+          bool photo = false;
+          if (EvalPair(a.cam, K, gp, nrm, radius_sq, d1, d2, USE_DESC, &r, &l, &e, &photo) == 3)
+            AccumulatePosition<USE_DEPTH, USE_DESC>(a.cam, r, e, photo, q);
+        }
+      }
+      if (update) UpdatePosition<USE_DESC>(a, i, gp, nrm, d1, d2, q);
+    }
   }
 }
 
@@ -945,6 +1044,34 @@
   return LaunchGeo(PositionDescriptorKernel<true, false>, a, sm_count, false, stream);
 }
 
+template <bool DETERMINE, bool USE_DEPTH, bool USE_DESC>
+static LaunchResult LaunchGeometryPassT(GeometryArgs a, int sm_count, int tile_shift, cudaStream_t stream) {
+  const auto kernel = GeometryPassKernel<DETERMINE, USE_DEPTH, USE_DESC>;
+  const size_t smem = sizeof(KfDevice) * a.kf_count;
+  int per_sm = 0;
+  LaunchResult r{1, cudaOccupancyMaxActiveBlocksPerMultiprocessor(&per_sm, kernel, kGeoThreads, smem)};
+  const uint32_t grid = TileGrid(per_sm, sm_count, a.end - a.begin, tile_shift, &a.tile_shift);
+  r += cudaMemsetAsync(a.queue, 0, sizeof(unsigned int), stream);
+  kernel<<<grid, kGeoThreads, smem, stream>>>(a);
+  return r;
+}
+
+template <bool DETERMINE>
+static LaunchResult LaunchGeometryPassD(const GeometryArgs& a, int sm_count, int tile_shift, cudaStream_t stream) {
+  if (a.cam.use_desc) {
+    if (a.cam.use_depth) return LaunchGeometryPassT<DETERMINE, true, true>(a, sm_count, tile_shift, stream);
+    return LaunchGeometryPassT<DETERMINE, false, true>(a, sm_count, tile_shift, stream);
+  }
+  return LaunchGeometryPassT<DETERMINE, true, false>(a, sm_count, tile_shift, stream);
+}
+
+LaunchResult LaunchGeometryPass(const GeometryArgs& a, int sm_count, bool determine_activation, int tile_shift, cudaStream_t stream) {
+  if (a.end <= a.begin) return {};
+  if (!GeometryPassFits(a)) return {0, cudaErrorInvalidValue};
+  if (determine_activation) return LaunchGeometryPassD<true>(a, sm_count, tile_shift, stream);
+  return LaunchGeometryPassD<false>(a, sm_count, tile_shift, stream);
+}
+
 
 __global__ void __launch_bounds__(256) PackShardKernel(const float* __restrict__ surfels, uint32_t pitch,
                                                        const uint8_t* __restrict__ active, uint32_t n, ShardRows rows,
diff --git a/badslam_b200/csrc/kernels.cuh b/badslam_b200/csrc/kernels.cuh
--- a/badslam_b200/csrc/kernels.cuh
+++ b/badslam_b200/csrc/kernels.cuh
@@ -158,6 +158,9 @@
 LaunchResult LaunchActivationAndNormals(const GeometryArgs& args, int sm_count, bool determine_activation, bool update_normals,
                                         cudaStream_t stream);
 LaunchResult LaunchPositionAndDescriptor(const GeometryArgs& args, int sm_count, cudaStream_t stream);
+constexpr int kGeoPassMaxKeyframes = 512;
+inline bool GeometryPassFits(const GeometryArgs& args) { return args.kf_count > 0 && args.kf_count <= kGeoPassMaxKeyframes; }
+LaunchResult LaunchGeometryPass(const GeometryArgs& args, int sm_count, bool determine_activation, int tile_shift, cudaStream_t stream);
 
 struct KfChange {
   float D[12];
diff --git a/badslam_b200/csrc/persistent.cuh b/badslam_b200/csrc/persistent.cuh
--- a/badslam_b200/csrc/persistent.cuh
+++ b/badslam_b200/csrc/persistent.cuh
@@ -160,5 +160,11 @@
 inline uint32_t ItemGrid(int per_sm, int sm_count, uint64_t n_items) {
   return static_cast<uint32_t>(std::min<uint64_t>((n_items + 7) / 8, static_cast<uint64_t>(std::max(per_sm, 1)) * sm_count));
 }
+constexpr int kTileMajorShift = 5;
+inline uint32_t TileGrid(int per_sm, int sm_count, uint32_t n, int forced_shift, int* tile_shift) {
+  const int shift = forced_shift >= 5 && forced_shift <= 8 ? forced_shift : kTileMajorShift;
+  *tile_shift = shift;
+  return ItemGrid(per_sm, sm_count, (static_cast<uint64_t>(n) + (1u << shift) - 1) >> shift);
+}
 
 }
diff --git a/badslam_b200/direct_ba.py b/badslam_b200/direct_ba.py
--- a/badslam_b200/direct_ba.py
+++ b/badslam_b200/direct_ba.py
@@ -595,6 +595,9 @@
     def DebugSetPoseGroup(self, keyframes: int):
         self._check(self._lib.bba_debug_set_pose_group(self._h, int(keyframes)))
 
+    def DebugSetGeometryPass(self, pass_: int, tile_shift: int = 0):
+        self._check(self._lib.bba_debug_set_geometry_pass(self._h, int(pass_), int(tile_shift)))
+
     def EstimateFramePose(self, stream, global_T_frame_initial_estimate, keyframe_id: int):
         p = np.ascontiguousarray(global_T_frame_initial_estimate, np.float32)
         out = np.zeros(7, np.float32)
diff --git a/include/badba.h b/include/badba.h
--- a/include/badba.h
+++ b/include/badba.h
@@ -161,6 +161,8 @@
 bba_status bba_debug_pose_coeffs_batch(bba_handle h, int count, const int* keyframe_ids, const float* global_T_frame, int variant,
                                        int with_stats, double* H, double* b, uint64_t* counts, double* costs, void* stream);
 bba_status bba_debug_set_pose_group(bba_handle h, int keyframes);
+typedef enum { BBA_GEOMETRY_PASS_AUTO = 0, BBA_GEOMETRY_PASS_SPLIT = 1, BBA_GEOMETRY_PASS_ONE = 2 } bba_geometry_pass;
+bba_status bba_debug_set_geometry_pass(bba_handle h, int pass, int tile_shift);
 bba_status bba_estimate_frame_pose(bba_handle h, int keyframe_id, const float global_T_frame_initial[7],
                                    float global_T_frame_out[7], int* iterations, int* converged, void* stream);
 bba_status bba_estimate_frame_pose_for_frame(bba_handle h, const uint16_t* device_depth, size_t depth_pitch,
```

Measured after the change: 28.33 billion (median of 6 runs). 1.05x the previous value.
